# tudelft-iv/CCVPE

Measured on AMD Instinct MI355X. Metric: image-pairs/sec, higher is better.
Workload: dtype f32

## Files before the change

ccvpe_amd/_lib.py:

```python
import ctypes
import os
import subprocess

import torch

_HERE = os.path.dirname(os.path.abspath(__file__))
LIB_PATH = os.environ.get("CCVPE_LIB") or os.path.join(_HERE, "libccvpe_hip.so")
CSRC_DIR = os.path.join(_HERE, "csrc")

c_float_p = ctypes.c_void_p
c_int = ctypes.c_int
c_float = ctypes.c_float
c_void_p = ctypes.c_void_p


class ConvDesc(ctypes.Structure):
    _fields_ = [
        ("src0", c_void_p), ("src1", c_void_p), ("gate", c_void_p), ("w", c_void_p),
        ("scale", c_void_p), ("shift", c_void_p), ("residual", c_void_p), ("dst", c_void_p),
        ("c0", c_int), ("ld0", c_int), ("c1", c_int), ("ld1", c_int),
        ("batch", c_int), ("in_h", c_int), ("in_w", c_int),
        ("kh", c_int), ("kw", c_int), ("stride", c_int), ("pad", c_int),
        ("n", c_int), ("kpad", c_int), ("ldd", c_int), ("ldres", c_int),
        ("act", c_int), ("out_mode", c_int),
    ]


class UpconvDesc(ctypes.Structure):
    _fields_ = [
        ("src0", c_void_p), ("src1", c_void_p), ("w", c_void_p), ("shift9", c_void_p), ("dst", c_void_p),
        ("c0", c_int), ("ld0", c_int), ("c1", c_int), ("ld1", c_int),
        ("batch", c_int), ("h1", c_int), ("w1", c_int),
        ("n", c_int), ("kpad", c_int), ("ldd", c_int), ("act", c_int),
    ]


class TailDesc(ctypes.Structure):
    _fields_ = [
        ("x", c_void_p), ("w", c_void_p), ("shift9", c_void_p), ("w2", c_void_p), ("b2", c_void_p), ("out", c_void_p),
        ("batch", c_int), ("h1", c_int), ("w1", c_int),
        ("c0", c_int), ("ld0", c_int), ("kpad", c_int),
        ("cout", c_int), ("normalize", c_int), ("split", c_int), ("softmax_partial", c_void_p),
    ]


PROTOTYPES = {
    "ccvpe_last_error": (ctypes.c_char_p, []),
    "ccvpe_abi_version": (c_int, []),
    "ccvpe_multi_copy_f32": (c_int, [ctypes.POINTER(c_void_p), ctypes.POINTER(c_void_p), ctypes.POINTER(c_int), c_int, c_void_p]),
    "ccvpe_gather_repack_f32": (c_int, [c_void_p, c_void_p, c_void_p, c_void_p, c_void_p, c_int, c_void_p]),
    "ccvpe_gather_repack_chunk": (c_int, []),
    "ccvpe_ctx_create": (c_int, [c_void_p, ctypes.c_longlong, c_void_p, c_void_p, ctypes.POINTER(c_void_p)]),
    "ccvpe_ctx_destroy": (c_int, [c_void_p]),
    "ccvpe_ctx_info": (c_int, [c_void_p] + [ctypes.POINTER(ctypes.c_longlong)] * 4 + [ctypes.POINTER(c_int)] * 2),
    "ccvpe_ctx_output": (c_int, [c_void_p, c_int, ctypes.POINTER(c_void_p), ctypes.POINTER(ctypes.c_longlong),
                                  ctypes.POINTER(c_int), ctypes.POINTER(ctypes.c_longlong), ctypes.POINTER(ctypes.c_longlong)]),
    "ccvpe_forward": (c_int, [c_void_p, c_void_p, c_void_p, ctypes.POINTER(c_void_p), c_void_p]),
    "ccvpe_tail512_partials": (c_int, [ctypes.POINTER(TailDesc), c_int]),
    "ccvpe_softmax_apply_f32": (c_int, [c_void_p, c_void_p, c_int, c_void_p, c_int, c_int, c_void_p]),
    "ccvpe_tail512_f32": (c_int, [ctypes.POINTER(TailDesc), c_void_p]),
    "ccvpe_tail512_bf16": (c_int, [ctypes.POINTER(TailDesc), c_void_p]),
    "ccvpe_conv_igemm_f32": (c_int, [ctypes.POINTER(ConvDesc), c_void_p]),
    "ccvpe_conv_igemm_splitk_floats": (c_int, [ctypes.POINTER(ConvDesc), c_int]),
    "ccvpe_conv_igemm_route": (c_int, [ctypes.POINTER(ConvDesc), c_int, c_int]),
    "ccvpe_set_narrow_kernels": (c_int, [c_int]),
    "ccvpe_set_pw_ring_kernels": (c_int, [c_int]),
    "ccvpe_set_mbconv_plane_kernels": (c_int, [c_int]),
    "ccvpe_mbconv_front_route": (c_int, [c_int] * 8),
    "ccvpe_mbconv_band_plan": (c_int, [c_int] * 7),
    "ccvpe_conv3x3_variant": (c_int, [ctypes.POINTER(ConvDesc), c_int]),
    "ccvpe_set_match_mfma": (c_int, [c_int]),
    "ccvpe_match_route": (c_int, [c_int, c_int, ctypes.POINTER(c_int)] + [c_int] * 10 + [ctypes.POINTER(c_int)]),
    "ccvpe_set_pwn_kernels": (c_int, [c_int]),
    "ccvpe_conv3x3_wino_ok": (c_int, [ctypes.POINTER(ConvDesc)]),
    "ccvpe_conv3x3_wino_f32": (c_int, [ctypes.POINTER(ConvDesc), c_void_p]),
    "ccvpe_conv3x3_match1_ok": (c_int, [ctypes.POINTER(ConvDesc), c_int, c_int]),
    "ccvpe_conv3x3_match1_bf16": (c_int, [ctypes.POINTER(ConvDesc), c_int, c_void_p, c_int, c_int, c_int, c_int, c_int, c_void_p, c_void_p]),
    "ccvpe_conv_igemm_splitk_f32": (c_int, [ctypes.POINTER(ConvDesc), c_void_p, c_void_p]),
    "ccvpe_conv_igemm_splitk_bf16": (c_int, [ctypes.POINTER(ConvDesc), c_int, c_void_p, c_void_p]),
    "ccvpe_upconv3x3_f32": (c_int, [ctypes.POINTER(UpconvDesc), c_void_p]),
    "ccvpe_upconv3x3_bf16": (c_int, [ctypes.POINTER(UpconvDesc), c_void_p]),
    "ccvpe_upconv3x3_route": (c_int, [ctypes.POINTER(UpconvDesc), c_int]),
    "ccvpe_upconv3x3_s3_ok": (c_int, [ctypes.POINTER(UpconvDesc)]),
    "ccvpe_upconv3x3_s3_f32": (c_int, [ctypes.POINTER(UpconvDesc), c_void_p]),
    "ccvpe_upconv3x3_s3_form_ok": (c_int, [ctypes.POINTER(UpconvDesc), c_int]),
    "ccvpe_upconv3x3_s3_route": (c_int, [ctypes.POINTER(UpconvDesc), c_int]),
    "ccvpe_upconv3x3_s3_form_f32": (c_int, [ctypes.POINTER(UpconvDesc), c_int, c_void_p]),
    "ccvpe_set_s3_quad": (c_int, [c_int]),
    "ccvpe_pw_s3_ok": (c_int, [ctypes.POINTER(ConvDesc)]),
    "ccvpe_pw_s3_route": (c_int, [ctypes.POINTER(ConvDesc)]),
    "ccvpe_pw_s3_f32": (c_int, [ctypes.POINTER(ConvDesc), c_void_p]),
    "ccvpe_stem_conv_f32": (c_int, [c_void_p] * 5 + [c_int] * 4 + [c_void_p]),
    "ccvpe_dwconv_nblk": (c_int, [c_int] * 4),
    "ccvpe_dwconv_f32": (c_int, [c_void_p] * 6 + [c_int] * 7 + [c_void_p]),
    "ccvpe_mbconv_front_nblk": (c_int, [c_int] * 6),
    "ccvpe_stem_dw_nblk": (c_int, [c_int] * 3),
    "ccvpe_stem_dw_f32": (c_int, [c_void_p] * 9 + [c_int] * 4 + [c_void_p]),
    "ccvpe_stem_dw_bf16": (c_int, [c_void_p] * 9 + [c_int] * 4 + [c_void_p]),
    "ccvpe_mbconv_front_f32": (c_int, [c_void_p, c_void_p, c_int] + [c_void_p] * 7 + [c_int] * 8 + [c_void_p]),
    "ccvpe_se_gate_f32": (c_int, [c_void_p, c_int, c_float] + [c_void_p] * 5 + [c_int] * 3 + [c_void_p]),
    "ccvpe_ground_descriptor_f32": (c_int, [c_void_p, c_int, c_void_p, c_void_p, ctypes.POINTER(c_int),
                                            c_void_p, c_int, c_int, c_int, c_void_p]),
    "ccvpe_match_level_f32": (c_int, [c_void_p, c_int, c_void_p, c_int, c_int, ctypes.POINTER(c_int),
                                      c_int, c_int, c_int, c_int, c_int, c_void_p, c_void_p, c_int, c_int,
                                      c_int, c_int, c_void_p]),
    "ccvpe_head_conv3x3_f32": (c_int, [c_void_p] * 4 + [c_int] * 5 + [c_void_p]),
    "ccvpe_cast_bf16_f32": (c_int, [c_void_p, c_void_p, ctypes.c_long, c_void_p]),
    "ccvpe_softmax_rows_f32": (c_int, [c_void_p, c_void_p, c_int, c_int, c_void_p]),
    "ccvpe_eval_postprocess_f32": (c_int, [c_void_p, c_void_p, c_void_p, c_int, c_int, c_int, c_void_p]),
    "ccvpe_eval_metrics_f32": (c_int, [c_void_p] * 7 + [c_int, c_int, c_int, c_void_p]),
    "ccvpe_infonce_scratch_floats": (c_int, [c_int, c_int]),
    "ccvpe_infonce_loss_f32": (c_int, [c_void_p, c_void_p, c_float, c_void_p, c_void_p, c_void_p, c_int, c_int, c_void_p]),
    "ccvpe_cross_entropy_loss_f32": (c_int, [c_void_p] * 4 + [c_int, c_int, c_void_p]),
    "ccvpe_orientation_loss_f32": (c_int, [c_void_p] * 5 + [c_int, c_int, c_void_p]),
    "ccvpe_stem_conv_raw_f32": (c_int, [c_void_p] * 3 + [c_int] * 4 + [c_void_p]),
    "ccvpe_dwconv_raw_f32": (c_int, [c_void_p] * 3 + [c_int] * 7 + [c_void_p]),
    "ccvpe_bn_stats_nblk": (c_int, [c_int]),
    "ccvpe_bn_stats_f32": (c_int, [c_void_p, c_int, c_int] + [c_void_p] * 4 + [c_float, c_void_p, c_void_p]),
    "ccvpe_bn_act_nblk": (c_int, [c_int]),
    "ccvpe_bn_act_f32": (c_int, [c_void_p] * 5 + [c_float, c_int] + [c_void_p] * 4 + [c_int] * 3 + [c_void_p]),
    "ccvpe_conv_wgrad_tile": (c_int, [c_int, c_int]),
    "ccvpe_conv_wgrad_scratch_floats": (c_int, [c_int] * 9),
    "ccvpe_conv_wgrad_f32": (c_int, [c_void_p, c_int, c_int, c_void_p, c_int, c_int, c_void_p, c_int, c_void_p,
                                     c_void_p] + [c_int] * 8 + [c_void_p]),
    "ccvpe_conv_wgrad_gated_f32": (c_int, [c_void_p, c_int, c_int, c_void_p, c_void_p, c_int, c_void_p, c_void_p, c_int, c_int, c_int,
                                           c_int, c_void_p]),
    "ccvpe_conv_wgrad_bias_f32": (c_int, [c_void_p, c_int, c_int, c_void_p, c_int, c_int, c_void_p, c_int, c_void_p,
                                          c_void_p, c_void_p] + [c_int] * 8 + [c_void_p]),
    "ccvpe_colsum_f32": (c_int, [c_void_p, c_int, c_int, c_int, c_void_p, c_void_p, c_void_p]),
    "ccvpe_bn_bwd_nblk": (c_int, [c_int]),
    "ccvpe_bn_act_bwd_f32": (c_int, [c_void_p] * 9 + [c_float, c_int] + [c_void_p] * 4 + [c_int] * 3 + [c_void_p]),
    "ccvpe_bn_act_bwd_frozen_f32": (c_int, [c_void_p] * 9 + [c_float, c_int] + [c_void_p] * 4 + [c_int] * 3 + [c_void_p]),
    "ccvpe_se_bn_bwd_reduce_f32": (c_int, [c_void_p] * 6 + [c_float, c_int, c_void_p, c_void_p, c_int, c_int, c_int, c_void_p]),
    "ccvpe_se_bn_bwd_apply_f32": (c_int, [c_void_p] * 8 + [c_float, c_int, c_void_p, c_void_p, c_void_p, c_void_p, c_int, c_int, c_int,
                                          c_void_p]),
    "ccvpe_se_dgate_f32": (c_int, [c_void_p] * 6 + [c_float, c_int, c_void_p] + [c_int] * 3 + [c_void_p]),
    "ccvpe_se_bwd_f32": (c_int, [c_void_p, c_int, c_float, c_void_p, c_int] + [c_void_p] * 10 + [c_int] * 3 + [c_void_p]),
    "ccvpe_dwconv_dgrad_f32": (c_int, [c_void_p] * 3 + [c_int] * 7 + [c_void_p]),
    "ccvpe_dwconv_wgrad_nblk": (c_int, [c_int] * 4),
    "ccvpe_dwconv_wgrad_f32": (c_int, [c_void_p] * 4 + [c_int] * 7 + [c_void_p]),
    "ccvpe_relu_bwd_f32": (c_int, [c_void_p] * 3 + [c_int, c_void_p]),
    "ccvpe_gate_mul_f32": (c_int, [c_void_p] * 3 + [c_int] * 3 + [c_void_p]),
    "ccvpe_softmax_bwd_f32": (c_int, [c_void_p] * 4 + [c_int, c_int, c_void_p]),
    "ccvpe_l2norm2_bwd_f32": (c_int, [c_void_p] * 3 + [c_int, c_int, c_void_p]),
    "ccvpe_head_conv3x3_bwd_f32": (c_int, [c_void_p] * 7 + [c_int] * 5 + [c_void_p]),
    "ccvpe_ground_descriptor_bwd_f32": (c_int, [c_void_p, c_int, c_void_p, ctypes.POINTER(c_int)] + [c_void_p] * 4 +
                                        [c_int] * 3 + [c_void_p]),
    "ccvpe_add_cols_f32": (c_int, [c_void_p, c_int, c_int, c_void_p, c_int, c_int, c_int, c_int, c_void_p]),
    "ccvpe_stem_wgrad_nblk": (c_int, [c_int] * 3),
    "ccvpe_stem_conv_wgrad_f32": (c_int, [c_void_p] * 4 + [c_int] * 4 + [c_void_p]),
    "ccvpe_match_bwd_nblk": (c_int, [c_int, c_int, c_int]),
    "ccvpe_match_level_bwd_f32": (c_int, [c_void_p, c_int, c_void_p, c_int, c_int, ctypes.POINTER(c_int), c_int, c_int,
                                          c_int, c_int, c_int, c_void_p, c_void_p, c_void_p, c_int, c_void_p, c_int, c_void_p,
                                          c_int, c_void_p, c_int, c_int, c_int, c_void_p]),
    "ccvpe_infonce_loss_bwd_f32": (c_int, [c_void_p, c_void_p, c_float, c_void_p, c_void_p, c_void_p, c_int, c_int, c_void_p]),
    "ccvpe_cross_entropy_loss_bwd_f32": (c_int, [c_void_p] * 4 + [c_int, c_int, c_void_p]),
    "ccvpe_orientation_loss_bwd_f32": (c_int, [c_void_p] * 5 + [c_int, c_int, c_void_p]),
    "ccvpe_train_targets_nblk": (c_int, [c_int, c_int]),
    "ccvpe_train_targets_f32": (c_int, [c_void_p, c_void_p, c_int, c_float] + [c_void_p] * 10 + [c_int] * 3 + [c_void_p]),
    "ccvpe_train_targets_ordered_f32": (c_int, [c_void_p, c_void_p, c_int, c_int, c_float] + [c_void_p] * 10 + [c_int] * 3 + [c_void_p]),
    "ccvpe_adam_chunk_elems": (c_int, []),
    "ccvpe_adam_hyper_floats": (c_int, []),
    "ccvpe_adam_step_f32": (c_int, [c_void_p, c_void_p, c_void_p, c_void_p, c_int, c_float, c_void_p]),
    "ccvpe_adam_device_layout": (c_int, [c_int]),
    "ccvpe_grad_sqnorm_f32": (c_int, [c_void_p, c_void_p, c_void_p, c_int, c_float, c_void_p, c_void_p]),
    "ccvpe_adam_prepare_f32": (c_int, [c_void_p, c_void_p, c_void_p, c_void_p, c_int, c_void_p, c_int, c_float, c_void_p, c_void_p]),
    "ccvpe_adam_update_f32": (c_int, [c_void_p, c_void_p, c_void_p, c_void_p, c_int, c_float, c_void_p, c_void_p]),
    "ccvpe_preprocess_u8_f32": (c_int, [c_void_p, c_int, c_int, c_void_p, c_void_p, c_int, c_void_p, c_void_p, c_int, c_void_p,
                                        c_void_p, c_int, c_int, c_int, c_int, ctypes.POINTER(c_float), ctypes.POINTER(c_float),
                                        c_void_p]),
    "ccvpe_resize_u8": (c_int, [c_void_p, c_int, c_int, c_void_p, c_void_p, c_int, c_void_p, c_void_p, c_int, c_void_p, c_void_p,
                                c_int, c_int, c_void_p]),
    "ccvpe_gather_norm_u8_f32": (c_int, [c_void_p, c_void_p, c_int, c_int, c_int, c_int, ctypes.POINTER(c_float),
                                         ctypes.POINTER(c_float), c_void_p, c_void_p]),
    "ccvpe_window_resize_norm_u8_f32": (c_int, [c_void_p, c_int, c_int, c_void_p, c_int, c_int, c_int, c_void_p, c_void_p, c_int,
                                                c_void_p, c_void_p, c_int, ctypes.POINTER(c_float), ctypes.POINTER(c_float),
                                                c_void_p, c_int, c_int, c_void_p]),
    "ccvpe_kitti_align_u8": (c_int, [c_void_p, ctypes.c_long, c_void_p, c_void_p, c_int, c_void_p, c_int, c_int, c_void_p]),
    "ccvpe_kitti_align_norm_u8_f32": (c_int, [c_void_p, c_void_p, c_int, ctypes.POINTER(c_float), ctypes.POINTER(c_float),
                                              c_void_p, c_int, c_int, c_void_p]),
    "ccvpe_conv_igemm_bf16": (c_int, [ctypes.POINTER(ConvDesc), c_int, c_void_p]),
    "ccvpe_stem_conv_bf16": (c_int, [c_void_p] * 5 + [c_int] * 4 + [c_void_p]),
    "ccvpe_dwconv_bf16": (c_int, [c_void_p] * 6 + [c_int] * 7 + [c_void_p]),
    "ccvpe_mbconv_front_bf16": (c_int, [c_void_p, c_void_p, c_int] + [c_void_p] * 7 + [c_int] * 8 + [c_void_p]),
    "ccvpe_match_level_bf16": (c_int, [c_void_p, c_int, c_void_p, c_int, c_int, ctypes.POINTER(c_int),
                                       c_int, c_int, c_int, c_int, c_int, c_void_p, c_void_p, c_int, c_int,
                                       c_int, c_int, c_void_p]),
    "ccvpe_head_conv3x3_bf16": (c_int, [c_void_p] * 4 + [c_int] * 5 + [c_void_p]),
}

_lib = None
weights_epoch = 0


def build(verbose=False):
    cmd = ["make", "-C", CSRC_DIR, "-j8"]
    res = subprocess.run(cmd, capture_output=True, text=True)
    if verbose or res.returncode != 0:
        print(res.stdout)
        print(res.stderr)
    if res.returncode != 0:
        raise RuntimeError("building libccvpe_hip.so failed (see output above)")
    return LIB_PATH


def load():
    global _lib
    if _lib is not None:
        return _lib
    if not os.path.isfile(LIB_PATH):
        raise RuntimeError(
            "libccvpe_hip.so not found at %s — run `python -c 'import __graft_entry__ as g; g.build()'` "
            "(or `make -C ccvpe_amd/csrc`).  ccvpe_amd has no CPU fallback." % LIB_PATH)
    lib = ctypes.CDLL(LIB_PATH)
    lax = bool(os.environ.get("CCVPE_LIB")) and os.environ.get("CCVPE_LIB_ALLOW_MISSING") == "1"
    for name, (res, args) in PROTOTYPES.items():
        if lax and not hasattr(lib, name):
            continue
        fn = getattr(lib, name)
        fn.restype = res
        fn.argtypes = args
    if os.environ.get("CCVPE_NARROW") == "0" and hasattr(lib, "ccvpe_set_narrow_kernels"):
        lib.ccvpe_set_narrow_kernels(0)
    if os.environ.get("CCVPE_PW_RING") == "0" and hasattr(lib, "ccvpe_set_pw_ring_kernels"):
        lib.ccvpe_set_pw_ring_kernels(0)
    if os.environ.get("CCVPE_MATCH_MFMA") == "0" and hasattr(lib, "ccvpe_set_match_mfma"):
        lib.ccvpe_set_match_mfma(0)
    if os.environ.get("CCVPE_PWN") == "0" and hasattr(lib, "ccvpe_set_pwn_kernels"):
        lib.ccvpe_set_pwn_kernels(0)
    if os.environ.get("CCVPE_S3_QUAD") == "0" and hasattr(lib, "ccvpe_set_s3_quad"):
        lib.ccvpe_set_s3_quad(0)
    if os.environ.get("CCVPE_MBPLANE") is not None and hasattr(lib, "ccvpe_set_mbconv_plane_kernels"):
        lib.ccvpe_set_mbconv_plane_kernels(int(os.environ["CCVPE_MBPLANE"]))
    _lib = lib
    return lib


class CcvpeError(RuntimeError):
    pass


def check(status, what):
    if status != 0:
        msg = load().ccvpe_last_error()
        raise CcvpeError("%s failed (%d): %s" % (what, status, msg.decode() if msg else "?"))
```

ccvpe_amd/csrc/plan.hip:

```cpp
#include <cstring>
#include <string>
#include <unordered_map>
#include <utility>
#include <vector>

#include "common.h"

namespace ccvpe {

enum : uint32_t { K_INT = 0, K_FLT = 1, K_NULL = 2, K_WEIGHTS = 3, K_WORKSPACE = 4, K_GRD = 5, K_SAT = 6, K_STREAM = 7, K_BLOB = 8 };

template <typename A> struct FromSlot {
  static A get(uint64_t v) { return (A)(int64_t)v; }
};
template <typename P> struct FromSlot<P*> {
  static P* get(uint64_t v) { return reinterpret_cast<P*>((uintptr_t)v); }
};
template <> struct FromSlot<float> {
  static float get(uint64_t v) { uint32_t b = (uint32_t)v; float f; std::memcpy(&f, &b, 4); return f; }
};
template <typename... A, size_t... I>
static int invoke_seq(int (*f)(A...), const uint64_t* v, std::index_sequence<I...>) { return f(FromSlot<A>::get(v[I])...); }
template <typename... A>
static int invoke(int (*f)(A...), const uint64_t* v, int n) {
  if (n != (int)sizeof...(A)) return fail(CCVPE_EINVAL, "plan: call has %d arguments, the entry point takes %d", n, (int)sizeof...(A));
  return invoke_seq(f, v, std::index_sequence_for<A...>{});
}
typedef int (*Invoker)(const uint64_t*, int);

#define CCVPE_REG(fn) {#fn, [](const uint64_t* v, int n) -> int { return invoke(fn, v, n); }}
static const std::unordered_map<std::string, Invoker>& registry() {
  static const std::unordered_map<std::string, Invoker> r = {
      CCVPE_REG(ccvpe_conv_igemm_f32), CCVPE_REG(ccvpe_conv_igemm_bf16), CCVPE_REG(ccvpe_conv_igemm_splitk_f32),
      CCVPE_REG(ccvpe_conv_igemm_splitk_bf16), CCVPE_REG(ccvpe_conv3x3_match1_bf16), CCVPE_REG(ccvpe_conv3x3_wino_f32),
      CCVPE_REG(ccvpe_upconv3x3_f32), CCVPE_REG(ccvpe_upconv3x3_bf16), CCVPE_REG(ccvpe_upconv3x3_s3_f32), CCVPE_REG(ccvpe_pw_s3_f32),
      CCVPE_REG(ccvpe_tail512_f32), CCVPE_REG(ccvpe_tail512_bf16), CCVPE_REG(ccvpe_stem_conv_f32), CCVPE_REG(ccvpe_stem_conv_bf16),
      CCVPE_REG(ccvpe_stem_dw_f32), CCVPE_REG(ccvpe_stem_dw_bf16),
      CCVPE_REG(ccvpe_dwconv_f32), CCVPE_REG(ccvpe_dwconv_bf16), CCVPE_REG(ccvpe_mbconv_front_f32), CCVPE_REG(ccvpe_mbconv_front_bf16),
      CCVPE_REG(ccvpe_se_gate_f32), CCVPE_REG(ccvpe_ground_descriptor_f32), CCVPE_REG(ccvpe_match_level_f32),
      CCVPE_REG(ccvpe_match_level_bf16), CCVPE_REG(ccvpe_head_conv3x3_f32), CCVPE_REG(ccvpe_head_conv3x3_bf16),
      CCVPE_REG(ccvpe_softmax_rows_f32), CCVPE_REG(ccvpe_softmax_apply_f32), CCVPE_REG(ccvpe_cast_bf16_f32), CCVPE_REG(ccvpe_eval_postprocess_f32),
  };
  return r;
}
#undef CCVPE_REG

struct Patch { uint32_t call, arg, kind; uint64_t off; };
struct BlobPatch { uint32_t blob, field, kind; uint64_t off; };
struct Call { Invoker fn; std::string name; uint32_t first, nargs, sid; int wait_on; };
struct Output { uint64_t off, bytes; uint32_t dtype, ndim; long long dims[4], strides[4]; };

}

struct ccvpe_ctx {
  std::vector<ccvpe::Call> calls;
  std::vector<uint64_t> args;
  std::vector<std::vector<unsigned char>> blobs;
  std::vector<ccvpe::Patch> patches;
  std::vector<ccvpe::BlobPatch> blob_patches;
  std::vector<ccvpe::Output> outputs;
  uint64_t workspace_bytes = 0, weights_bytes = 0, grd_bytes = 0, sat_bytes = 0;
  char* weights = nullptr;
  char* workspace = nullptr;
  bool own_weights = false, own_workspace = false;
  hipStream_t side = nullptr;
  std::vector<hipEvent_t> events;
};

using namespace ccvpe;

namespace {
struct Reader {
  const unsigned char* p;
  const unsigned char* end;
  bool ok = true;
  template <typename T> T get() {
    T v{};
    if (sizeof(T) > (size_t)(end - p)) { ok = false; return v; }
    std::memcpy(&v, p, sizeof(T));
    p += sizeof(T);
    return v;
  }
  const unsigned char* bytes(size_t n) {
    if (n > (size_t)(end - p)) { ok = false; return nullptr; }
    const unsigned char* q = p;
    p += n;
    return q;
  }
};
}

extern "C" int ccvpe_ctx_create(const void* plan, long long n_bytes, void* weights_dev, void* workspace_dev, ccvpe_ctx** out) {
  if (!plan || n_bytes < 64 || !out) return fail(CCVPE_EINVAL, "ctx_create: null / short plan");
  Reader r{reinterpret_cast<const unsigned char*>(plan), reinterpret_cast<const unsigned char*>(plan) + n_bytes};
  const unsigned char* magic = r.bytes(8);
  if (!magic || std::memcmp(magic, "CCVPLAN1", 8)) return fail(CCVPE_EINVAL, "ctx_create: not a CCVPE plan (bad magic)");
  ccvpe_ctx* c = new ccvpe_ctx();
  auto bail = [&](int code, const char* msg) { delete c; return fail(code, "ctx_create: %s", msg); };
  const int abi = (int)r.get<uint32_t>();
  const uint32_t flags = r.get<uint32_t>();
  (void)flags;
  if (abi != ccvpe_abi_version()) {
    delete c;
    return fail(CCVPE_EINVAL, "ctx_create: the plan was recorded against ABI %d, this library is ABI %d", abi, ccvpe_abi_version());
  }
  c->workspace_bytes = r.get<uint64_t>();
  c->weights_bytes = r.get<uint64_t>();
  c->grd_bytes = r.get<uint64_t>();
  c->sat_bytes = r.get<uint64_t>();
  const uint32_t n_calls = r.get<uint32_t>(), n_blobs = r.get<uint32_t>(), n_out = r.get<uint32_t>();
  r.get<uint32_t>();
  if (!r.ok || n_calls > (1u << 20) || n_blobs > (1u << 20) || n_out > 64) return bail(CCVPE_EINVAL, "corrupt header");
  for (uint32_t i = 0; i < n_out; ++i) {
    Output o;
    o.off = r.get<uint64_t>(); o.bytes = r.get<uint64_t>(); o.dtype = r.get<uint32_t>(); o.ndim = r.get<uint32_t>();
    for (int k = 0; k < 4; ++k) o.dims[k] = (long long)r.get<uint64_t>();
    for (int k = 0; k < 4; ++k) o.strides[k] = (long long)r.get<uint64_t>();
    if (o.off > c->workspace_bytes || o.bytes > c->workspace_bytes - o.off) return bail(CCVPE_EINVAL, "output outside the workspace");
    c->outputs.push_back(o);
  }
  struct Reloc { uint32_t blob, field, kind; uint64_t value; };
  std::vector<Reloc> relocs;
  for (uint32_t i = 0; i < n_blobs && r.ok; ++i) {
    const uint32_t nb = r.get<uint32_t>(), nr = r.get<uint32_t>();
    for (uint32_t k = 0; k < nr; ++k) {
      Reloc q{i, r.get<uint32_t>(), r.get<uint32_t>(), r.get<uint64_t>()};
      if ((uint64_t)q.field + 8 > (uint64_t)nb) return bail(CCVPE_EINVAL, "relocation outside its blob");
      relocs.push_back(q);
    }
    const unsigned char* d = r.bytes((nb + 7) & ~7u);
    if (!d) return bail(CCVPE_EINVAL, "truncated blob");
    c->blobs.emplace_back(d, d + nb);
  }
  struct RawArg { uint32_t kind; uint64_t value; };
  std::vector<std::vector<RawArg>> raw(n_calls);
  for (uint32_t i = 0; i < n_calls && r.ok; ++i) {
    const unsigned char* nm = r.bytes(48);
    if (!nm) break;
    std::string name(reinterpret_cast<const char*>(nm), strnlen(reinterpret_cast<const char*>(nm), 48));
    const uint32_t na = r.get<uint32_t>();
    const uint32_t sid = r.get<uint32_t>() & 1u;
    if (na > 64) return bail(CCVPE_EINVAL, "call with more than 64 arguments");
    for (uint32_t k = 0; k < na; ++k) {
      RawArg a{r.get<uint32_t>(), 0};
      r.get<uint32_t>();
      a.value = r.get<uint64_t>();
      raw[i].push_back(a);
    }
    if (name == "@wait") {
      if (na != 2) return bail(CCVPE_EINVAL, "malformed stream wait");
      c->calls.push_back(Call{nullptr, name, 0, 0, (uint32_t)(raw[i][0].value & 1), (int)(raw[i][1].value & 1)});
      raw[i].clear();
      continue;
    }
    auto it = registry().find(name);
    if (it == registry().end()) {
      delete c;
      return fail(CCVPE_EINVAL, "ctx_create: the plan calls %s, which this library does not replay", name.c_str());
    }
    c->calls.push_back(Call{it->second, name, 0, na, sid, -1});
  }
  if (!r.ok) return bail(CCVPE_EINVAL, "truncated plan");
  size_t woff = (size_t)(r.p - reinterpret_cast<const unsigned char*>(plan));
  woff = (woff + 255) & ~(size_t)255;
  if (woff > (size_t)n_bytes || c->weights_bytes > (uint64_t)((size_t)n_bytes - woff)) return bail(CCVPE_EINVAL, "truncated weights");
  if (weights_dev) c->weights = reinterpret_cast<char*>(weights_dev);
  else {
    if (hipMalloc(reinterpret_cast<void**>(&c->weights), c->weights_bytes ? c->weights_bytes : 256) != hipSuccess) return bail(CCVPE_ELAUNCH, "hipMalloc(weights)");
    c->own_weights = true;
  }
  if (workspace_dev) c->workspace = reinterpret_cast<char*>(workspace_dev);
  else {
    if (hipMalloc(reinterpret_cast<void**>(&c->workspace), c->workspace_bytes ? c->workspace_bytes : 256) != hipSuccess) {
      if (c->own_weights) (void)hipFree(c->weights);
      return bail(CCVPE_ELAUNCH, "hipMalloc(workspace)");
    }
    c->own_workspace = true;
  }
  if (c->weights_bytes &&
      hipMemcpy(c->weights, reinterpret_cast<const unsigned char*>(plan) + woff, c->weights_bytes, hipMemcpyHostToDevice) != hipSuccess) {
    ccvpe_ctx_destroy(c);
    return fail(CCVPE_ELAUNCH, "ctx_create: weight upload failed");
  }
  auto resolve = [&](uint32_t kind, uint64_t v, bool& dynamic, bool& bad) -> uint64_t {
    dynamic = bad = false;
    switch (kind) {
      case K_INT: case K_FLT: return v;
      case K_NULL: return 0;
      case K_WEIGHTS: bad = v >= c->weights_bytes; return (uint64_t)(uintptr_t)(c->weights + v);
      case K_WORKSPACE: bad = v >= c->workspace_bytes; return (uint64_t)(uintptr_t)(c->workspace + v);
      case K_BLOB: bad = v >= c->blobs.size(); return bad ? 0 : (uint64_t)(uintptr_t)c->blobs[v].data();
      case K_GRD: bad = v >= c->grd_bytes; dynamic = true; return 0;
      case K_SAT: bad = v >= c->sat_bytes; dynamic = true; return 0;
      case K_STREAM: dynamic = true; return 0;
      default: bad = true; return 0;
    }
  };
  for (const Reloc& q : relocs) {
    bool dyn, bad;
    const uint64_t v = resolve(q.kind, q.value, dyn, bad);
    if (bad || q.kind == K_BLOB || q.kind == K_STREAM) { ccvpe_ctx_destroy(c); return fail(CCVPE_EINVAL, "ctx_create: bad relocation"); }
    if (dyn) c->blob_patches.push_back(BlobPatch{q.blob, q.field, q.kind, q.value});
    else std::memcpy(c->blobs[q.blob].data() + q.field, &v, 8);
  }
  for (uint32_t i = 0; i < n_calls; ++i) {
    c->calls[i].first = (uint32_t)c->args.size();
    for (uint32_t k = 0; k < raw[i].size(); ++k) {
      bool dyn, bad;
      const uint64_t v = resolve(raw[i][k].kind, raw[i][k].value, dyn, bad);
      if (bad) { ccvpe_ctx_destroy(c); return fail(CCVPE_EINVAL, "ctx_create: bad argument %u of call %u (%s)", k, i, c->calls[i].name.c_str()); }
      if (dyn) c->patches.push_back(Patch{i, k, raw[i][k].kind, raw[i][k].value});
      c->args.push_back(v);
    }
  }
  bool two_streams = false;
  for (const Call& k : c->calls) {
    two_streams = two_streams || k.sid == 1 || !k.fn;
    if (!k.fn) {
      hipEvent_t ev;
      if (hipEventCreateWithFlags(&ev, hipEventDisableTiming) != hipSuccess) { ccvpe_ctx_destroy(c); return fail(CCVPE_ELAUNCH, "ctx_create: hipEventCreate"); }
      c->events.push_back(ev);
    }
  }
  if (two_streams && hipStreamCreateWithFlags(&c->side, hipStreamNonBlocking) != hipSuccess) {
    ccvpe_ctx_destroy(c);
    return fail(CCVPE_ELAUNCH, "ctx_create: hipStreamCreate");
  }
  *out = c;
  return CCVPE_OK;
}

extern "C" int ccvpe_ctx_destroy(ccvpe_ctx* c) {
  if (!c) return CCVPE_OK;
  if (c->own_weights && c->weights) (void)hipFree(c->weights);
  if (c->own_workspace && c->workspace) (void)hipFree(c->workspace);
  for (hipEvent_t ev : c->events) (void)hipEventDestroy(ev);
  if (c->side) (void)hipStreamDestroy(c->side);
  delete c;
  return CCVPE_OK;
}

extern "C" int ccvpe_ctx_info(const ccvpe_ctx* c, long long* workspace_bytes, long long* weights_bytes, long long* grd_bytes,
                              long long* sat_bytes, int* n_outputs, int* n_calls) {
  if (!c) return fail(CCVPE_EINVAL, "ctx_info: null ctx");
  if (workspace_bytes) *workspace_bytes = (long long)c->workspace_bytes;
  if (weights_bytes) *weights_bytes = (long long)c->weights_bytes;
  if (grd_bytes) *grd_bytes = (long long)c->grd_bytes;
  if (sat_bytes) *sat_bytes = (long long)c->sat_bytes;
  if (n_outputs) *n_outputs = (int)c->outputs.size();
  if (n_calls) *n_calls = (int)c->calls.size();
  return CCVPE_OK;
}

extern "C" int ccvpe_ctx_output(const ccvpe_ctx* c, int i, void** dev_ptr, long long* bytes, int* ndim, long long* dims4,
                                long long* strides4) {
  if (!c || i < 0 || i >= (int)c->outputs.size()) return fail(CCVPE_EINVAL, "ctx_output: bad index");
  const Output& o = c->outputs[i];
  if (dev_ptr) *dev_ptr = c->workspace + o.off;
  if (bytes) *bytes = (long long)o.bytes;
  if (ndim) *ndim = (int)o.ndim;
  if (dims4) for (int k = 0; k < 4; ++k) dims4[k] = o.dims[k];
  if (strides4) for (int k = 0; k < 4; ++k) strides4[k] = o.strides[k];
  return CCVPE_OK;
}

extern "C" int ccvpe_forward(ccvpe_ctx* c, const void* grd, const void* sat, void** out, void* stream) {
  if (!c || !grd || !sat) return fail(CCVPE_EINVAL, "forward: null ctx / input");
  for (const Patch& q : c->patches) {
    uint64_t v = 0;
    if (q.kind == K_GRD) v = (uint64_t)(uintptr_t)(reinterpret_cast<const char*>(grd) + q.off);
    else if (q.kind == K_SAT) v = (uint64_t)(uintptr_t)(reinterpret_cast<const char*>(sat) + q.off);
    else v = (uint64_t)(uintptr_t)(c->calls[q.call].sid ? (void*)c->side : stream);
    c->args[c->calls[q.call].first + q.arg] = v;
  }
  for (const BlobPatch& q : c->blob_patches) {
    const uint64_t v = (uint64_t)(uintptr_t)(reinterpret_cast<const char*>(q.kind == K_GRD ? grd : sat) + q.off);
    std::memcpy(c->blobs[q.blob].data() + q.field, &v, 8);
  }
  size_t nev = 0;
  for (const Call& k : c->calls) {
    if (!k.fn) {
      hipStream_t waiter = k.sid ? c->side : (hipStream_t)stream, waitee = k.wait_on ? c->side : (hipStream_t)stream;
      hipEvent_t ev = c->events[nev++];
      if (hipEventRecord(ev, waitee) != hipSuccess || hipStreamWaitEvent(waiter, ev, 0) != hipSuccess)
        return fail(CCVPE_ELAUNCH, "forward: stream wait failed");
      continue;
    }
    const int rc = k.fn(c->args.data() + k.first, (int)k.nargs);
    if (rc != CCVPE_OK) return rc;
  }
  if (out) for (size_t i = 0; i < c->outputs.size(); ++i) out[i] = c->workspace + c->outputs[i].off;
  return CCVPE_OK;
}
```

ccvpe_amd/models.py:

```python
import torch
import torch.nn as nn

from . import ops
from .synth import B0_BLOCKS, MODEL_SPECS, state_dict_spec

BN_EPS = 1e-3
SKIP_BLOCKS = (15, 10, 4, 2, 0)
MATCH_STRIDES = {"vigor": (64, 32, 16, 8, 4, 2),
                 "kitti": (128, 64, 32, 16, 8, 8),
                 "oxford": (64, 32, 16, 8, 4, 2)}


def window_offset(kind, channels, length):
    return int(channels / 2 - length / 2) if kind == "oxford" else 0


def _round_up(v, m):
    return (v + m - 1) // m * m


class _Holder(nn.Module):

    def forward(self, *a, **k):
        raise RuntimeError("parameter holder is not callable; use the owning CVM_* module")


def _populate(root, kind, init):
    for key, shape, role in state_dict_spec(kind):
        parts = key.split(".")
        node = root
        for name in parts[:-1]:
            child = node._modules.get(name)
            if child is None:
                child = _Holder()
                node.add_module(name, child)
            node = child
        t = init[key].clone()
        if role in ("bn_m", "bn_v", "bn_n"):
            node.register_buffer(parts[-1], t)
        else:
            node.register_parameter(parts[-1], nn.Parameter(t))


def _pad2(w, dtype=torch.float32, n_mult=16):
    k_mult = 16 if dtype == torch.float32 else 32
    n, k = w.shape
    if n % n_mult == 0 and k % k_mult == 0:
        out = w.to(dtype).contiguous()
        return out.clone() if out.data_ptr() == w.data_ptr() else out
    out = w.new_zeros((_round_up(n, n_mult), _round_up(k, k_mult)))
    out[:n, :k] = w
    return out.to(dtype).contiguous()


def _pack_conv(w, dtype=torch.float32):
    o = w.shape[0]
    return _pad2(w.permute(0, 2, 3, 1).reshape(o, -1), dtype)


_WINO_G = ((1.0, 0.0, 0.0), (0.5, 0.5, 0.5), (0.5, -0.5, 0.5), (0.0, 0.0, 1.0))


def _pack_wino(w, dtype=torch.float32):
    if dtype != torch.float32:
        return None
    o, i = w.shape[0], w.shape[1]
    g = torch.tensor(_WINO_G, dtype=torch.float64, device=w.device)
    u = torch.einsum("ak,ockl,bl->oabc", g, w.to(torch.float64), g)
    out = torch.zeros((_round_up(o, 32), 4, 4, _round_up(i, 16)), dtype=torch.float64, device=w.device)
    out[:o, :, :, :i] = u
    return out.reshape(out.shape[0], -1).to(torch.float32).contiguous()


def _fold_bn(sd, p):
    scale = sd[p + ".weight"] / torch.sqrt(sd[p + ".running_var"] + BN_EPS)
    shift = sd[p + ".bias"] - sd[p + ".running_mean"] * scale
    return scale.contiguous(), shift.contiguous()


class _Obj(object):
    pass


def _pack_pw_s3(w):
    if w is None or w.dtype != torch.float32 or w.dim() != 2 or w.shape[1] % 16 or w.shape[0] % 16:
        return None
    npad, k = w.shape
    return torch.cat(_split3_bf16(w.reshape(npad, k // 16, 16).permute(1, 0, 2)), -1).contiguous()


def _unpack_pw_s3(w3):
    nst, npad, _ = w3.shape
    return tuple(w3[..., 16 * q:16 * q + 16].float().permute(1, 0, 2).reshape(npad, nst * 16) for q in range(3))


PW_S3_MIN_MID = 240


def _pack_encoder(sd, p, dtype=torch.float32, fold_bn=True, s3=False):
    fold = _fold_bn if fold_bn else (lambda _sd, _p: (None, None))
    e = _Obj()
    e.stem_w = sd[p + "._conv_stem.weight"].permute(2, 3, 1, 0).contiguous()
    e.stem_scale, e.stem_shift = fold(sd, p + "._bn0")
    e.blocks = []
    for i, (k, s, ex, cin, cout) in enumerate(B0_BLOCKS):
        b = _Obj()
        bp = "%s._blocks.%d" % (p, i)
        b.k, b.s, b.expand, b.cin, b.cout, b.mid = k, s, ex != 1, cin, cout, cin * ex
        if b.expand:
            b.w_exp = _pack_conv(sd[bp + "._expand_conv.weight"], dtype)
            b.s0, b.b0 = fold(sd, bp + "._bn0")
        b.w_dw = sd[bp + "._depthwise_conv.weight"].reshape(b.mid, k, k).permute(1, 2, 0).contiguous()
        b.s1, b.b1 = fold(sd, bp + "._bn1")
        b.se_w1 = sd[bp + "._se_reduce.weight"].reshape(-1, b.mid).contiguous()
        b.se_b1 = sd[bp + "._se_reduce.bias"].contiguous()
        b.se_w2 = sd[bp + "._se_expand.weight"].reshape(b.mid, -1).t().contiguous()
        b.se_b2 = sd[bp + "._se_expand.bias"].contiguous()
        b.w_proj = _pack_conv(sd[bp + "._project_conv.weight"], dtype)
        b.w_proj3 = _pack_pw_s3(b.w_proj) if s3 and b.mid >= PW_S3_MIN_MID else None
        b.s2, b.b2 = fold(sd, bp + "._bn2")
        b.skip = (s == 1 and cin == cout)
        e.blocks.append(b)
    e.w_head = _pack_conv(sd[p + "._conv_head.weight"], dtype)
    e.w_head3 = _pack_pw_s3(e.w_head) if s3 else None
    e.head_scale, e.head_shift = fold(sd, p + "._bn1")
    return e


def _pack_deconv(w, bias, col_map, ldo, dtype=torch.float32):
    cin, cout = w.shape[0], w.shape[1]
    wg = w.permute(2, 3, 1, 0).reshape(4 * cout, cin)
    out = w.new_zeros((4 * cout, ldo))
    for d0, s0, n in col_map:
        out[:, d0:d0 + n] = wg[:, s0:s0 + n]
    return _pad2(out, dtype), bias.repeat(4).contiguous()


_UP_S = {0: {0: ((0, 1),), 1: ((1, 0), (2, 1))}, 1: {0: ((0, 0), (1, 1)), 1: ((2, 0),)}}
_UP_R = {0: (1, 2), 1: (0, 1, 2), 2: (0, 1)}
_OVERLAP_ENV = __import__("os").environ.get("CCVPE_OVERLAP_DECODERS", "auto")


OVERLAP_DECODERS_MAX_BATCH = 128


def _overlap_decoders(precision, batch=1):
    return _OVERLAP_ENV == "1" or (_OVERLAP_ENV == "auto" and precision == "bf16" and batch <= OVERLAP_DECODERS_MAX_BATCH)
FOLD_LEVELS = tuple(int(c) for c in __import__("os").environ.get("CCVPE_FOLD_LEVELS", "012345"))
FOLD_MIN_PIXELS = int(__import__("os").environ.get("CCVPE_FOLD_MIN_PIXELS", "2048"))
FUSE_TAIL = __import__("os").environ.get("CCVPE_FUSE_TAIL", "1") != "0"
SPLIT_TAIL = __import__("os").environ.get("CCVPE_SPLIT_TAIL", "1") != "0"
WINO = __import__("os").environ.get("CCVPE_WINO", "1") != "0"
SPLIT3 = __import__("os").environ.get("CCVPE_SPLIT3", "1") != "0"
SPLIT3_TAIL = SPLIT3 and __import__("os").environ.get("CCVPE_SPLIT3_TAIL", "1") != "0"
SPLIT3_MIN_OK = 2
SPLIT3_PW = SPLIT3 and __import__("os").environ.get("CCVPE_SPLIT3_PW", "1") != "0"
SPLIT3_PW_MIN_OK = 2
PACK_GRAPH = __import__("os").environ.get("CCVPE_PACK_GRAPH", "1") != "0"
PACK_GATHER = __import__("os").environ.get("CCVPE_PACK_GATHER", "1") != "0"
FUSE_MATCH = __import__("os").environ.get("CCVPE_FUSE_MATCH", "1") != "0"
FUSE_STEM = __import__("os").environ.get("CCVPE_FUSE_STEM", "1") != "0"
EVAL_TWO_STREAMS = __import__("os").environ.get("CCVPE_EVAL_TWO_STREAMS", "1") != "0"


def _tail_split(precision, x, cout):
    if x.dtype != torch.float32:
        return 0
    if precision == "bf16":
        return 1 if SPLIT_TAIL and cout == 1 else 0
    return 2 if SPLIT3 and SPLIT3_TAIL else 0


def _pack_upconv(wd, bd, col_map, cp, w3, b3, dtype=torch.float32):
    cd, co = wd.shape[1], w3.shape[0]
    c1 = w3.shape[1] - cd
    wd_my = wd.new_zeros((cp, cd, 2, 2), dtype=torch.float64)
    for d0, s0, n in col_map:
        wd_my[d0:d0 + n] = wd[s0:s0 + n].double()
    w3d = w3[:, :cd].double()
    k = 4 * cp + 9 * c1
    kmult = 16 if dtype == torch.float32 else 32
    out = wd.new_zeros((4, _round_up(co, 16), _round_up(k, kmult)), dtype=torch.float64)
    for py in range(2):
        for px in range(2):
            par = py * 2 + px
            for du in range(2):
                for dv in range(2):
                    weff = wd.new_zeros((co, cp), dtype=torch.float64)
                    for ky, a in _UP_S[py][du]:
                        for kx, b in _UP_S[px][dv]:
                            weff += w3d[:, :, ky, kx] @ wd_my[:, :, a, b].t()
                    tap = du * 2 + dv
                    out[par, :co, tap * cp:(tap + 1) * cp] = weff
            if c1:
                out[par, :co, 4 * cp:k] = w3[:, cd:].double().permute(0, 2, 3, 1).reshape(co, 9 * c1)
    shift9 = wd.new_zeros((9, co), dtype=torch.float64)
    for rc in range(3):
        for cc in range(3):
            v = b3.double().clone()
            for ky in _UP_R[rc]:
                for kx in _UP_R[cc]:
                    v += w3d[:, :, ky, kx] @ bd.double()
            shift9[rc * 3 + cc] = v
    return out.to(dtype).contiguous(), shift9.float().contiguous()


def _split3_bf16(v):
    hi = v.to(torch.bfloat16)
    r = v - hi.float()
    mid = r.to(torch.bfloat16)
    lo = (r - mid.float()).to(torch.bfloat16)
    return hi, mid, lo


def _pack_upconv_s3(fw, cp, c1, dtype=torch.float32):
    if dtype != torch.float32 or fw is None or fw.dtype != torch.float32 or c1 <= 0:
        return None
    npad = fw.shape[1]
    nb0, nb1 = (cp + 15) // 16, (c1 + 15) // 16
    a = fw.new_zeros((4, npad, 4, nb0 * 16))
    a[..., :cp] = fw[:, :, :4 * cp].reshape(4, npad, 4, cp)
    a = a.reshape(4, npad, 4, nb0, 16).permute(0, 3, 2, 1, 4).reshape(4, 4 * nb0, npad, 16)
    s = fw.new_zeros((4, npad, 9, nb1 * 16))
    s[..., :c1] = fw[:, :, 4 * cp:4 * cp + 9 * c1].reshape(4, npad, 9, c1)
    s = s.reshape(4, npad, 9, nb1, 16).permute(0, 2, 3, 1, 4).reshape(4, 9 * nb1, npad, 16)
    return torch.cat(_split3_bf16(torch.cat([a, s], 1)), -1).contiguous()


def _pack_backward(sd, kind, pk):
    spec = MODEL_SPECS[kind]
    n_rot = spec["n_rot"]
    bwd = {}
    for enc in ("grd_efficientnet", "sat_efficientnet"):
        for i, (k, s_, ex, cin, cout) in enumerate(B0_BLOCKS):
            bp = "%s._blocks.%d" % (enc, i)
            if ex != 1:
                bwd[bp + "._expand_conv.weight"] = _pack_conv(sd[bp + "._expand_conv.weight"].permute(1, 0, 2, 3))
            bwd[bp + "._project_conv.weight"] = _pack_conv(sd[bp + "._project_conv.weight"].permute(1, 0, 2, 3))
            if s_ == 1:
                mid = cin * ex
                w_dw = sd[bp + "._depthwise_conv.weight"].reshape(mid, k * k).t()
                bwd[bp + "._depthwise_conv.weight"] = w_dw.flip(0).contiguous()
        bwd[enc + "._conv_head.weight"] = _pack_conv(sd[enc + "._conv_head.weight"].permute(1, 0, 2, 3))
    for j in range(6):
        lvl = 6 - j
        for branch, lv in (("", pk.loc[j]), ("_ori", pk.ori[j])):
            conv, deconv = "conv%d%s" % (lvl, branch), "deconv%d%s" % (lvl, branch)
            if lvl != 1:
                bwd[conv + ".2.weight"] = _pack_conv(sd[conv + ".2.weight"].flip(2, 3).permute(1, 0, 2, 3))
            bwd[conv + ".0.weight"] = _pack_conv(sd[conv + ".0.weight"].flip(2, 3).permute(1, 0, 2, 3))
            w_ref = sd[deconv + ".weight"]
            if branch == "":
                c = lv.c
                k_rows, cmap = lv.ldo, [(0, 1, c), (c, 0, 1)]
            elif j == 0:
                c6 = spec["ori"][0][0] - n_rot
                k_rows, cmap = lv.k, [(0, n_rot, c6), (c6 + 1, 0, n_rot)]
            else:
                k_rows, cmap = lv.k, [(0, 0, spec["ori"][j][0])]
            w_ours = w_ref.new_zeros((k_rows,) + tuple(w_ref.shape[1:]))
            for d0, s0, n in cmap:
                w_ours[d0:d0 + n] = w_ref[s0:s0 + n]
            bwd[deconv + ".weight"] = _pack_conv(w_ours)
    w = sd["sat_feature_to_descriptors.1.weight"]
    w4 = w.view(w.shape[0], 1280, 2, 2)
    bwd["sat_feature_to_descriptors.1.weight"] = _pack_deconv(w4, w4.new_zeros((1280,)), [(0, 0, w.shape[0])], w.shape[0])[0]
    wcat = torch.cat([sd["grd_feature_to_descriptor%d.0.weight" % l] for l in range(1, 7)], 0)
    ld = _round_up(pk.gd_n, 4)
    wpad = wcat.new_zeros((ld,) + tuple(wcat.shape[1:]))
    wpad[:pk.gd_n] = wcat
    bwd["grd_feature_to_descriptor.0.weight"] = _pack_conv(wpad.permute(1, 0, 2, 3))
    return bwd


def _pack_model(sd, kind, n_tail, dtype=torch.float32, fold=True, f32_tail=0):
    spec = MODEL_SPECS[kind]
    pk = _Obj()
    pk.dtype = dtype
    pk.f32_from = 6 - f32_tail if dtype != torch.float32 else 6
    base_dtype = dtype
    s3 = fold and dtype == torch.float32
    pk.grd = _pack_encoder(sd, "grd_efficientnet", dtype, fold_bn=fold, s3=s3)
    pk.sat = _pack_encoder(sd, "sat_efficientnet", dtype, fold_bn=fold, s3=s3)
    ws, bs, wh, bh = [], [], [], []
    for l in range(1, 7):
        p = "grd_feature_to_descriptor%d" % l
        ws.append(sd[p + ".0.weight"].reshape(-1, 1280))
        bs.append(sd[p + ".0.bias"])
        wh.append(sd[p + ".2.weight"].reshape(-1))
        bh.append(sd[p + ".2.bias"].reshape(-1))
    pk.gd_w = _pad2(torch.cat(ws, 0), dtype)
    pk.gd_w3 = _pack_pw_s3(pk.gd_w) if s3 else None
    pk.gd_bias = torch.cat(bs, 0).contiguous()
    pk.gd_n = pk.gd_bias.shape[0]
    pk.gd_wh = torch.stack(wh, 0).contiguous()
    pk.gd_bh = torch.cat(bh, 0).contiguous()
    w = sd["sat_feature_to_descriptors.1.weight"]
    pk.sd_w = _pack_conv(w.view(w.shape[0], 1280, 2, 2), dtype)
    pk.sd_w3 = _pack_pw_s3(pk.sd_w) if s3 else None
    pk.sd_bias = sd["sat_feature_to_descriptors.1.bias"].contiguous()
    pk.sd_n = w.shape[0]

    pk.loc, pk.ori = [], []
    n_rot = spec["n_rot"]
    for j in range(6):
        lvl = 6 - j
        dc_in, dc_out, c_in, c_out = spec["loc"][j]
        dtype = torch.float32 if j >= pk.f32_from else base_dtype
        c = dc_in - 1
        ldo = _round_up(c + 1 + (n_tail if j == 0 else 0), 8)
        lv = _Obj()
        lv.c, lv.ldo, lv.up_n = c, ldo, 4 * dc_out
        lv.up_w, lv.up_b = _pack_deconv(sd["deconv%d.weight" % lvl], sd["deconv%d.bias" % lvl],
                                        [(0, 1, c), (c, 0, 1)], ldo, dtype)
        lv.c0, lv.c1 = dc_out, c_in - dc_out
        lv.n_a = c_out
        if fold and j in FOLD_LEVELS:
            lv.fw, lv.fshift = _pack_upconv(sd["deconv%d.weight" % lvl], sd["deconv%d.bias" % lvl],
                                            [(0, 1, c), (c, 0, 1)], ldo, sd["conv%d.0.weight" % lvl],
                                            sd["conv%d.0.bias" % lvl], dtype)
            lv.fw3 = _pack_upconv_s3(lv.fw, ldo, lv.c1, dtype if base_dtype == torch.float32 else None)
        lv.w_a = _pack_conv(sd["conv%d.0.weight" % lvl], dtype)
        lv.b_a = sd["conv%d.0.bias" % lvl].contiguous()
        if lvl != 1:
            lv.w_b = _pack_conv(sd["conv%d.2.weight" % lvl], dtype)
            lv.u_b = _pack_wino(sd["conv%d.2.weight" % lvl], base_dtype) if fold else None
            lv.n_b = c_out
        else:
            lv.w_b = sd["conv1.2.weight"].permute(0, 2, 3, 1).contiguous()
        lv.b_b = sd["conv%d.2.bias" % lvl].contiguous()
        pk.loc.append(lv)
        dtype = base_dtype
        dc_in, dc_out, c_in, c_out = spec["ori"][j]
        ov = _Obj()
        if j == 0:
            c6 = dc_in - n_rot
            ov.k = pk.loc[0].ldo
            ov.k_algo = dc_in
            ov.up_w, ov.up_b = _pack_deconv(sd["deconv6_ori.weight"], sd["deconv6_ori.bias"],
                                            [(0, n_rot, c6), (c6 + 1, 0, n_rot)], pk.loc[0].ldo, dtype)
        else:
            ov.k = ov.k_algo = dc_in
            ov.up_w, ov.up_b = _pack_deconv(sd["deconv%d_ori.weight" % lvl], sd["deconv%d_ori.bias" % lvl],
                                            [(0, 0, dc_in)], dc_in, dtype)
        ov.up_n = 4 * dc_out
        ov.c0, ov.c1 = dc_out, c_in - dc_out
        if fold and j in FOLD_LEVELS:
            cmap = [(0, n_rot, c6), (c6 + 1, 0, n_rot)] if j == 0 else [(0, 0, dc_in)]
            ov.fw, ov.fshift = _pack_upconv(sd["deconv%d_ori.weight" % lvl], sd["deconv%d_ori.bias" % lvl], cmap,
                                            ov.k, sd["conv%d_ori.0.weight" % lvl], sd["conv%d_ori.0.bias" % lvl],
                                            dtype)
            ov.fw3 = _pack_upconv_s3(ov.fw, ov.k, ov.c1, dtype)
        ov.w_a = _pack_conv(sd["conv%d_ori.0.weight" % lvl], dtype)
        ov.b_a = sd["conv%d_ori.0.bias" % lvl].contiguous()
        ov.n_a = c_out
        if lvl != 1:
            ov.w_b = _pack_conv(sd["conv%d_ori.2.weight" % lvl], dtype)
            ov.u_b = _pack_wino(sd["conv%d_ori.2.weight" % lvl], dtype) if fold else None
            ov.n_b = c_out
        else:
            ov.w_b = sd["conv1_ori.2.weight"].permute(0, 2, 3, 1).contiguous()
        ov.b_b = sd["conv%d_ori.2.bias" % lvl].contiguous()
        pk.ori.append(ov)
    pk.bwd = _pack_backward(sd, kind, pk) if (not fold and base_dtype == torch.float32) else None
    return pk


def _pw(x, c0, w, w3, n, *, batch, in_h, in_w, two=False, gate=None, scale=None, shift=None, residual=None, act=ops.ACT_NONE,
        ldd=None, out_f32=False):
    if (SPLIT3 and SPLIT3_PW and w3 is not None and x.dtype == torch.float32 and
            ops.pw_s3_ok(x, c0, w3, n, batch=batch, in_h=in_h, in_w=in_w, two=two, gate=gate, residual=residual, act=act,
                         ldd=ldd) >= SPLIT3_PW_MIN_OK):
        return ops.pw_s3(x, c0, w3, n, batch=batch, in_h=in_h, in_w=in_w, two=two, gate=gate, scale=scale, shift=shift,
                         residual=residual, act=act, ldd=ldd)
    kk = dict(kh=2, kw=2, stride=2) if two else {}
    return ops.conv_igemm(x, c0, w, n, batch=batch, in_h=in_h, in_w=in_w, gate=gate, scale=scale, shift=shift, residual=residual,
                          act=act, ldd=ldd, out_f32=out_f32, **kk)


def _run_encoder(e, img, circular, multiscale, dtype=torch.float32):
    blk0 = e.blocks[0]
    stem_fused = (FUSE_STEM and not blk0.expand and blk0.k == 3 and blk0.s == 1 and blk0.mid == 32
                  and ops.stem_dw_supported(img.shape[2], img.shape[3], circular) > 0)
    x = None if stem_fused else ops.stem_conv(img, e.stem_w, e.stem_scale, e.stem_shift, circular, out_dtype=dtype)
    feats = []
    for blk in e.blocks:
        if x is not None:
            b, h, w, _ = x.shape
        if x is None:
            u, part = ops.stem_dw(img, e.stem_w, e.stem_scale, e.stem_shift, blk.w_dw, blk.s1, blk.b1, circular,
                                  out_dtype=dtype)
            b = u.shape[0]
        elif blk.expand and ops.mbconv_front_supported(h, w, blk.cin, blk.mid, blk.k, blk.s):
            u, part = ops.mbconv_front(x, blk.w_exp, blk.s0, blk.b0, blk.w_dw, blk.s1, blk.b1, blk.mid,
                                       blk.k, blk.s, circular)
        else:
            t = x
            if blk.expand:
                t = ops.conv_igemm(x, blk.cin, blk.w_exp, blk.mid, batch=b, in_h=h, in_w=w,
                                   scale=blk.s0, shift=blk.b0, act=ops.ACT_SWISH)
            u, part = ops.dwconv(t, blk.w_dw, blk.s1, blk.b1, blk.k, blk.s, circular)
        ho, wo = u.shape[1], u.shape[2]
        gate = ops.se_gate(part, ho * wo, blk.se_w1, blk.se_b1, blk.se_w2, blk.se_b2)
        x = _pw(u, blk.mid, blk.w_proj, getattr(blk, "w_proj3", None), blk.cout, batch=b, in_h=ho, in_w=wo, gate=gate,
                scale=blk.s2, shift=blk.b2, residual=x if blk.skip else None)
        if multiscale:
            feats.append(x)
    b, h, w, _ = x.shape
    f = _pw(x, 320, e.w_head, getattr(e, "w_head3", None), 1280, batch=b, in_h=h, in_w=w, scale=e.head_scale,
            shift=e.head_shift, act=ops.ACT_SWISH)
    return f, feats


def _double_conv(lv, up, skip, batch, hw):
    y = ops.conv_igemm(up, lv.c0, lv.w_a, lv.n_a, batch=batch, in_h=hw, in_w=hw, kh=3, kw=3, pad=1,
                       src1=skip, c1=lv.c1, shift=lv.b_a, act=ops.ACT_RELU)
    return y


def _conv_b(lv, y, batch, hw, out_f32=False):
    if (WINO and lv.u_b is not None and
            ops.conv3x3_wino_ok(y, lv.n_a, lv.u_b, lv.n_b, batch=batch, in_h=hw, in_w=hw)):
        return ops.conv3x3_wino(y, lv.n_a, lv.u_b, lv.n_b, batch=batch, in_h=hw, in_w=hw, shift=lv.b_b)
    return ops.conv_igemm(y, lv.n_a, lv.w_b, lv.n_b, batch=batch, in_h=hw, in_w=hw, kh=3, kw=3, pad=1, shift=lv.b_b,
                          out_f32=out_f32)


def _upconv_a(lv, x, k, batch, hw, skip):
    fw3 = getattr(lv, "fw3", None)
    if (SPLIT3 and fw3 is not None and
            ops.upconv3x3_s3_ok(x, k, fw3, lv.n_a, batch=batch, h1=hw, w1=hw, src1=skip, c1=lv.c1) >= SPLIT3_MIN_OK):
        return ops.upconv3x3_s3(x, k, fw3, lv.fshift, lv.n_a, batch=batch, h1=hw, w1=hw, src1=skip, c1=lv.c1, act=ops.ACT_RELU)
    return ops.upconv3x3(x, k, lv.fw, lv.fshift, lv.n_a, batch=batch, h1=hw, w1=hw, src1=skip, c1=lv.c1, act=ops.ACT_RELU)


class _CVMBase(nn.Module):
    kind = "vigor"

    def __init__(self, device, circular_padding, ori_noise=None, efficientnet_weights=None):
        super().__init__()
        self.device = device
        self.circular_padding = circular_padding
        self.ori_noise = ori_noise
        from . import init as _init
        _populate(self, self.kind, _init.reference_init_state_dict(self.kind))
        weights = efficientnet_weights if efficientnet_weights is not None else __import__("os").environ.get("CCVPE_EFFICIENTNET_B0")
        if weights:
            _init.load_efficientnet_b0(self, weights)
        self._pack_cache = None
        self._pack_key = None
        self.precision = "fp32"
        self.fp32_tail_levels = 1

    def set_precision(self, precision, fp32_tail_levels=1):
        if precision not in ("fp32", "bf16"):
            raise ValueError("precision must be 'fp32' or 'bf16'")
        if not 0 <= int(fp32_tail_levels) <= 5:
            raise ValueError("fp32_tail_levels must be in 0..5 (level 6 feeds the bf16 orientation decoder)")
        self.precision = precision
        self.fp32_tail_levels = int(fp32_tail_levels)
        return self

    def invalidate(self):
        self._pack_cache = None
        self._pack_key = None
        object.__setattr__(self, "_flat_tensors", None)
        return self

    def _weights_key(self):
        from . import _lib
        flat = getattr(self, "_flat_tensors", None)
        if flat is None:
            flat = list(self.parameters()) + list(self.buffers())
            object.__setattr__(self, "_flat_tensors", flat)
        return (_lib.weights_epoch,) + tuple((t.data_ptr(), t._version) for t in flat)

    def _packed(self):
        epoch = 0 if self.training else getattr(self, "_stats_epoch", 0)
        key = (self.precision, self.fp32_tail_levels, self.training, epoch) + self._weights_key()
        if self._pack_cache is not None and key == self._pack_key:
            return self._pack_cache
        dev = next(self.parameters()).device
        if dev.type != "cuda":
            raise RuntimeError("ccvpe_amd: move the model to the MI355X first (.to('cuda'))")
        sd = {k: v.detach() for k, v in self.state_dict().items()}
        n_tail = MODEL_SPECS[self.kind]["n_rot"]
        dtype = torch.float32 if self.precision == "fp32" else torch.bfloat16

        def pack(src=sd):
            with torch.no_grad():
                return _pack_model(src, self.kind, n_tail, dtype, fold=not self.training, f32_tail=self.fp32_tail_levels)

        if self.training and PACK_GATHER and dtype == torch.float32 and not getattr(self, "_pack_plan_failed", False):
            from . import repack
            where = tuple(t.data_ptr() for t in list(self.parameters()) + list(self.buffers()))
            gp = getattr(self, "_pack_plan", None)
            if gp is not None and gp[0] == where:
                self._pack_cache = gp[1].run()
            else:
                plan = repack.build(sd, pack)
                if plan is None:
                    self._pack_plan, self._pack_plan_failed = None, True
                    return self._packed()
                self._pack_plan = (where, plan)
                self._pack_cache = plan.pk
        elif self.training and PACK_GRAPH:
            where = (self.precision, self.fp32_tail_levels) + tuple(
                t.data_ptr() for t in list(self.parameters()) + list(self.buffers()))
            g = getattr(self, "_pack_graph", None)
            if g is not None and g[0] == where:
                g[1].replay()
                self._pack_cache = g[2]
            elif getattr(self, "_pack_where", None) == where and not getattr(self, "_pack_graph_failed", False):
                try:
                    graph = torch.cuda.CUDAGraph()
                    with torch.cuda.graph(graph, capture_error_mode="thread_local"):
                        pk = pack()
                    graph.replay()
                    self._pack_graph = (where, graph, pk)
                    self._pack_cache = pk
                except Exception:
                    self._pack_graph, self._pack_graph_failed = None, True
                    self._pack_cache = pack()
            else:
                self._pack_graph = None
                self._pack_where = where
                self._pack_cache = pack()
        else:
            self._pack_cache = pack()
        self._pack_key = key
        return self._pack_cache

    def _side_stream(self, which=1):
        dev = next(self.parameters()).device
        streams = self.__dict__.setdefault("_side_streams", {})
        st = streams.get(which)
        if st is None or st.device != dev:
            st = torch.cuda.Stream(device=dev)
            streams[which] = st
        return st

    def _ori_decoder(self, pk, cat6, sfeats, batch):
        xo = cat6
        normalize = not getattr(self, "ori_raw_output", False)
        for j in range(6):
            ov = pk.ori[j]
            hw = xo.shape[1]
            skip = sfeats[SKIP_BLOCKS[j]] if j < 5 else None
            if j == 5 and FUSE_TAIL and j in FOLD_LEVELS and ops.tail512_ok(hw, hw, ov.n_a):
                return ops.tail512(xo, ov.k, ov.fw, ov.fshift, ov.w_b, ov.b_b, 2, normalize, batch=batch, h1=hw, w1=hw,
                                   split=_tail_split(self.precision, xo, 2))
            if j in FOLD_LEVELS and batch * hw * hw >= FOLD_MIN_PIXELS:
                y = _upconv_a(ov, xo, ov.k, batch, hw, skip)
            else:
                up = ops.conv_igemm(xo, ov.k, ov.up_w, ov.up_n, batch=batch, in_h=hw, in_w=hw,
                                    shift=ov.up_b, out_mode=ops.OUT_DECONV2X, algo_k=ov.k_algo)
                y = _double_conv(ov, up, skip, batch, 2 * hw)
            if j < 5:
                xo = _conv_b(ov, y, batch, 2 * hw)
            else:
                return ops.head_conv3x3(y, ov.w_b, ov.b_b, 2, normalize)

    def _loc_shifts(self):
        n_rot = MODEL_SPECS[self.kind]["n_rot"]
        if self.ori_noise is None:
            return list(range(n_rot))
        k = int(self.ori_noise / 18)
        return list(range(-k, k + 1))

    drop_connect_rate = 0.2
    BN_MOMENTUM = 0.01

    bn_frozen = False

    def freeze_batchnorm(self, mode=True):
        self.bn_frozen = bool(mode)
        return self

    def forward(self, grd, sat, drop_masks=None):
        if self.training and self.precision != "fp32":
            raise NotImplementedError("ccvpe_amd: train mode is fp32 only")
        if not (grd.is_cuda and sat.is_cuda):
            raise RuntimeError("ccvpe_amd runs on the MI355X only: inputs must be device tensors")
        if self.training:
            from . import train
            if torch.is_grad_enabled() and any(p.requires_grad for p in self.parameters()):
                outs = train.apply(self, grd, sat, drop_masks)
            else:
                with torch.no_grad():
                    outs, _ = train.forward_train(self, grd, sat, drop_masks, rec=False)
            outs = list(outs)
            if self.ori_noise is not None:
                outs[3] = outs[3][:, len(self._loc_shifts()):]
            return tuple(outs)
        main = torch.cuda.current_stream()
        return self._forward_eval(grd, sat, main, self._side_stream() if EVAL_TWO_STREAMS else main)

    def _forward_eval(self, grd, sat, main, side):
        spec = MODEL_SPECS[self.kind]
        n_rot = spec["n_rot"]
        strides = MATCH_STRIDES[self.kind]
        circular = bool(self.circular_padding) and self.kind == "vigor"
        with torch.no_grad():
            pk = self._packed()
            grd = grd.contiguous().float()
            sat = sat.contiguous().float()
            batch = grd.shape[0]

            side.wait_stream(main)
            with torch.cuda.stream(side):
                gfeat, _ = _run_encoder(pk.grd, grd, circular, False, pk.dtype)
                _, gh, gw, _ = gfeat.shape
                if gh != spec["grd_h"]:
                    raise ValueError("ground feature height %d != %d expected by the descriptor heads"
                                     % (gh, spec["grd_h"]))
                y1 = _pw(gfeat, 1280, pk.gd_w, pk.gd_w3, pk.gd_n, batch=batch, in_h=gh, in_w=gw,
                         shift=pk.gd_bias, ldd=_round_up(pk.gd_n, 4), out_f32=True)
                gdesc = ops.ground_descriptor(y1, pk.gd_wh, pk.gd_bh, spec["cd"])
            svol, sfeats = _run_encoder(pk.sat, sat, False, True, pk.dtype)
            main.wait_stream(side)
            gdesc.record_stream(main)
            sdesc = _pw(svol, 1280, pk.sd_w, pk.sd_w3, pk.sd_n, batch=batch, in_h=svol.shape[1],
                        in_w=svol.shape[2], two=True, shift=pk.sd_bias)

            overlap = _overlap_decoders(self.precision, batch)
            loc_shifts = self._loc_shifts()
            fused = None
            scores_out = []
            smx = None
            x = sdesc
            cat6 = None
            goff = 0
            sfeats_loc = sfeats
            for j in range(6):
                lv = pk.loc[j]
                if j == pk.f32_from:
                    x = ops.cast_f32(x)
                    sfeats_loc = dict((SKIP_BLOCKS[q], ops.cast_f32(sfeats[SKIP_BLOCKS[q]])) for q in range(j, 5))
                hw = x.shape[1]
                cd = spec["cd"][j]
                L = gw * cd
                g = gdesc[:, goff:goff + L]
                goff += L
                if j == 0:
                    if self.ori_noise is None:
                        shifts, n_max = list(range(n_rot)), n_rot
                    else:
                        shifts, n_max = loc_shifts + list(range(n_rot)), len(loc_shifts)
                    n_tail = n_rot
                else:
                    shifts, n_max, n_tail = loc_shifts, len(loc_shifts), 0
                if fused is not None:
                    sc, cat = fused
                    fused = None
                else:
                    sc, cat = ops.match_level(x, g, L, shifts, n_max, n_tail, strides[j], lv.ldo, channels=lv.c,
                                              window_offset=window_offset(self.kind, lv.c, L))
                if j == 0:
                    cat6 = cat
                    scores_out.append(sc if self.ori_noise is None else sc[:, n_max:])
                    if overlap:
                        side.wait_stream(main)
                        with torch.cuda.stream(side):
                            x_ori = self._ori_decoder(pk, cat6, sfeats, batch)
                else:
                    scores_out.append(sc)
                skip = sfeats_loc[SKIP_BLOCKS[j]] if j < 5 else None
                if j == 5 and FUSE_TAIL and j in FOLD_LEVELS and ops.tail512_ok(hw, hw, lv.n_a):
                    logits_map, smx = ops.tail512(cat, lv.ldo, lv.fw, lv.fshift, lv.w_b, lv.b_b, 1, False, batch=batch, h1=hw, w1=hw,
                                                  split=_tail_split(self.precision, cat, 1),
                                                  want_softmax=True)
                    break
                if j in FOLD_LEVELS and batch * hw * hw >= FOLD_MIN_PIXELS:
                    y = _upconv_a(lv, cat, lv.ldo, batch, hw, skip)
                else:
                    up = ops.conv_igemm(cat, lv.ldo, lv.up_w, lv.up_n, batch=batch, in_h=hw, in_w=hw,
                                        shift=lv.up_b, out_mode=ops.OUT_DECONV2X, algo_k=lv.c + 1)
                    y = _double_conv(lv, up, skip, batch, 2 * hw)
                if j < 5:
                    to_f32 = j + 1 == pk.f32_from and y.dtype != torch.float32
                    nxt = pk.loc[j + 1]
                    L_n = gw * spec["cd"][j + 1]
                    if (FUSE_MATCH and len(loc_shifts) == 1 and
                            ops.conv3x3_match1(y, lv.n_a, lv.w_b, lv.n_b, None, L_n, loc_shifts[0], strides[j + 1], nxt.ldo, batch=batch,
                                               in_h=2 * hw, in_w=2 * hw, bias=lv.b_b, out_f32=to_f32, query_only=True)):
                        fused = ops.conv3x3_match1(y, lv.n_a, lv.w_b, lv.n_b, gdesc[:, goff:goff + L_n], L_n, loc_shifts[0],
                                                   strides[j + 1], nxt.ldo, batch=batch, in_h=2 * hw, in_w=2 * hw, bias=lv.b_b,
                                                   window_offset=window_offset(self.kind, nxt.c, L_n), out_f32=to_f32)
                        x = fused[1]
                    else:
                        x = _conv_b(lv, y, batch, 2 * hw, out_f32=to_f32)
                else:
                    logits_map = ops.head_conv3x3(y, lv.w_b, lv.b_b, 1, False)
            logits = logits_map.reshape(batch, -1)
            if smx is not None:
                heatmap = ops.softmax_apply(logits, smx).reshape(logits_map.shape)
            else:
                heatmap = ops.softmax_rows(logits).reshape(logits_map.shape)

            if overlap:
                main.wait_stream(side)
                x_ori.record_stream(main)
            else:
                x_ori = self._ori_decoder(pk, cat6, sfeats, batch)
        return (logits, heatmap, x_ori) + tuple(scores_out)


class CVM_VIGOR(_CVMBase):
    kind = "vigor"

    def __init__(self, device, circular_padding, efficientnet_weights=None):
        super().__init__(device, circular_padding, None, efficientnet_weights)


class CVM_VIGOR_ori_prior(_CVMBase):
    kind = "vigor"

    def __init__(self, device, ori_noise, circular_padding=True, efficientnet_weights=None):
        super().__init__(device, circular_padding, ori_noise, efficientnet_weights)


class CVM_OxfordRobotCar(_CVMBase):
    kind = "oxford"

    def __init__(self, device, efficientnet_weights=None):
        super().__init__(device, False, None, efficientnet_weights)


class CVM_KITTI(_CVMBase):
    kind = "kitti"

    def __init__(self, device, efficientnet_weights=None):
        super().__init__(device, False, None, efficientnet_weights)
```

ccvpe_amd/ops.py:

```python
import ctypes

import torch

from . import _lib
from ._lib import ConvDesc, check

ACT_NONE, ACT_RELU, ACT_SWISH, ACT_RELU_MASK = 0, 1, 2, 3
SPLIT_K_CALLS = 0
SPLIT_K = __import__("os").environ.get("CCVPE_SPLIT_K", "1") == "1"
OUT_NHWC, OUT_DECONV2X = 0, 1

_recorder = None


def set_recorder(rec):
    global _recorder
    _recorder = rec


class LaunchRecorder(object):

    def __init__(self):
        self.items = []

    def begin(self):
        ev = torch.cuda.Event(enable_timing=True)
        ev.record(torch.cuda.current_stream())
        return ev

    def end(self, name, tag, flops, nbytes, ev0):
        ev1 = torch.cuda.Event(enable_timing=True)
        ev1.record(torch.cuda.current_stream())
        self.items.append((name, tag, flops, nbytes, ev0, ev1))

    def summary(self):
        out = {}
        for name, tag, flops, nbytes, e0, e1 in self.items:
            d = out.setdefault(name, dict(calls=0, ms=0.0, flops=0.0, bytes=0.0))
            d["calls"] += 1
            d["ms"] += e0.elapsed_time(e1)
            d["flops"] += flops
            d["bytes"] += nbytes
        return out


def igemm_tile(n, is3x3=False):
    npad = (n + 15) // 16 * 16
    cfgs = [(4, 5, 2), (4, 4, 2), (4, 3, 2), (4, 2, 2), (4, 1, 2), (4, 5, 1), (4, 3, 1), (4, 1, 1), (2, 7, 1)]
    best, best_cost = None, None
    for mt, nt, wn in cfgs:
        bn = 16 * nt * wn
        tiles = (npad + bn - 1) // bn
        cost = tiles * bn * 1000 + (1000 - bn)
        if best_cost is None or cost < best_cost:
            best, best_cost = (mt, nt, wn), cost
    mt, nt, wn = best
    return "%s<%d,%d,%d>" % ("conv3x3_f32_kernel" if is3x3 else "igemm_f32_kernel", mt, nt, wn)


def _stream():
    return ctypes.c_void_p(torch.cuda.current_stream().cuda_stream)


ROUTE_FAMILIES = {0: "igemm", 1: "pw_gemm", 2: "conv3x3", 3: "c3n", 4: "pw_ring", 5: "pwn"}


def conv_route(desc, is_bf16, out_f32=False):
    r = _lib.load().ccvpe_conv_igemm_route(ctypes.byref(desc), int(bool(is_bf16)), int(bool(out_f32)))
    if r < 0:
        check(int(r), "ccvpe_conv_igemm_route")
    return ROUTE_FAMILIES[r & 0xff], (r >> 8) & 0xf, (r >> 12) & 0xf, (r >> 16) & 0xf


def conv3x3_variant(desc, is_bf16):
    r = _lib.load().ccvpe_conv3x3_variant(ctypes.byref(desc), int(bool(is_bf16)))
    if r < 0:
        check(int(r), "ccvpe_conv3x3_variant")
    return (r & 0xf, bool((r >> 4) & 1), (r >> 8) & 0xf) if r else None


UPROUTE_KERNELS = {0: "upconv_kernel", 1: "upconv_halo_kernel", 2: "upconv_dma_kernel", 3: "upconv_dma_kernel", 4: "up2_kernel"}


def upconv_route(desc, is_bf16):
    r = _lib.load().ccvpe_upconv3x3_route(ctypes.byref(desc), int(bool(is_bf16)))
    if r < 0:
        check(int(r), "ccvpe_upconv3x3_route")
    return UPROUTE_KERNELS[r & 0xff], (r >> 8) & 0xf, (r >> 12) & 0xf, (r >> 16) & 0xf, (r & 0xff) == 3


def upconv_route_name(desc, is_bf16):
    k, mt, nt, wn, pair = upconv_route(desc, is_bf16)
    ty = "bf16" if is_bf16 else "f32"
    if k == "up2_kernel":
        return "up2_kernel<bf16,%d,%d>" % (desc.c0, desc.n)
    return "%s<%s,%d,%d,%d%s>" % (k, ty, mt, nt, wn, ",pair" if pair else "")


def upconv_s3_route_name(desc, form=0):
    r = _lib.load().ccvpe_upconv3x3_s3_route(ctypes.byref(desc), form)
    if r <= 0:
        raise _lib.CcvpeError("ccvpe_upconv3x3_s3_route: form %d does not compute this layer" % form)
    mt, nt, wn = (r >> 8) & 0xf, (r >> 12) & 0xf, (r >> 16) & 0xf
    return "upconv_s3q_kernel<%d,%d>" % (mt, nt) if r & 0xf == 2 else "upconv_s3_kernel<%d,%d,%d%s>" % (mt, nt, wn, ",pair" if r & 16 else "")


def conv_route_name(desc, is_bf16, out_f32=False):
    fam, mt, nt, wn = conv_route(desc, is_bf16, out_f32)
    if fam == "c3n":
        return "c3n_kernel<bf16,%d>" % desc.n
    if is_bf16:
        return "%s_kernel<bf16,%d,%d,%d>" % (fam, mt, nt, wn)
    return "%s_f32_kernel<%d,%d,%d>" % (fam, mt, nt, wn)


_record = None


def _empty(shape, device=None, dtype=torch.float32):
    if _record is not None:
        return _record.empty(shape, dtype, device)
    return torch.empty(shape, device=device, dtype=dtype)


def _ptr(t):
    if t is None:
        return None
    if _record is not None:
        _record.note(t)
    return ctypes.c_void_p(t.data_ptr())


def _chk(t, name, dtype=torch.float32):
    if t is None:
        return
    if not t.is_cuda or t.dtype != dtype or not t.is_contiguous():
        raise ValueError("%s must be a contiguous %s device tensor (got %s %s contiguous=%s)" % (
            name, dtype, t.device, t.dtype, t.is_contiguous()))


def _act_dtype(t):
    if t.dtype not in (torch.float32, torch.bfloat16):
        raise ValueError("activations must be fp32 or bf16, got %s" % t.dtype)
    return t.dtype


def conv_igemm(src0, c0, w_packed, n, *, batch, in_h, in_w, kh=1, kw=1, stride=1, pad=0,
               src1=None, c1=0, gate=None, scale=None, shift=None, residual=None, act=ACT_NONE,
               out_mode=OUT_NHWC, dst=None, ldd=None, ld0=None, ld1=None, algo_k=None, out_f32=False, route_only=False,
               variant_only=False):
    lib = _lib.load()
    dt = _act_dtype(src0)
    odt = torch.float32 if (out_f32 or dt == torch.float32) else dt
    for t, nm in ((src0, "src0"), (src1, "src1"), (w_packed, "w"), (residual, "residual")):
        _chk(t, nm, dt)
    for t, nm in ((gate, "gate"), (scale, "scale"), (shift, "shift")):
        _chk(t, nm)
    _chk(dst, "dst", odt)
    ld0 = ld0 if ld0 is not None else src0.shape[-1]
    ld1 = ld1 if ld1 is not None else (src1.shape[-1] if src1 is not None else 0)
    ho = (in_h + 2 * pad - kh) // stride + 1
    wo = (in_w + 2 * pad - kw) // stride + 1
    if out_mode == OUT_DECONV2X:
        cout = n // 4
        oshape = (batch, 2 * ho, 2 * wo)
    else:
        cout = n
        oshape = (batch, ho, wo)
    if dst is None:
        ldd = ldd if ldd is not None else cout
        dst = _empty(oshape + (ldd,), device=src0.device, dtype=odt)
    elif ldd is None:
        ldd = dst.shape[-1]
    d = ConvDesc()
    d.src0, d.src1, d.gate, d.w = _ptr(src0), _ptr(src1), _ptr(gate), _ptr(w_packed)
    d.scale, d.shift, d.residual, d.dst = _ptr(scale), _ptr(shift), _ptr(residual), _ptr(dst)
    d.c0, d.ld0, d.c1, d.ld1 = c0, ld0, c1, ld1
    d.batch, d.in_h, d.in_w = batch, in_h, in_w
    d.kh, d.kw, d.stride, d.pad = kh, kw, stride, pad
    d.n, d.kpad = n, w_packed.shape[1]
    d.ldd = ldd
    d.ldres = residual.shape[-1] if residual is not None else 0
    d.act, d.out_mode = act, out_mode
    if route_only:
        return conv_route(d, dt != torch.float32, bool(out_f32))
    if variant_only:
        return conv3x3_variant(d, dt != torch.float32)
    rec = _recorder
    ev0 = rec.begin() if rec is not None else None
    want = lib.ccvpe_conv_igemm_splitk_floats(ctypes.byref(d), int(dt != torch.float32)) if SPLIT_K else 0
    if want < 0:
        check(int(want), "ccvpe_conv_igemm_splitk_floats")
    if want > 0:
        global SPLIT_K_CALLS
        SPLIT_K_CALLS += 1
        scratch = _empty((want,), device=src0.device, dtype=torch.float32)
        if dt == torch.float32:
            check(lib.ccvpe_conv_igemm_splitk_f32(ctypes.byref(d), _ptr(scratch), _stream()), "ccvpe_conv_igemm_splitk_f32")
        else:
            check(lib.ccvpe_conv_igemm_splitk_bf16(ctypes.byref(d), int(bool(out_f32)), _ptr(scratch), _stream()),
                  "ccvpe_conv_igemm_splitk_bf16")
    elif dt == torch.float32:
        check(lib.ccvpe_conv_igemm_f32(ctypes.byref(d), _stream()), "ccvpe_conv_igemm_f32")
    else:
        check(lib.ccvpe_conv_igemm_bf16(ctypes.byref(d), int(bool(out_f32)), _stream()), "ccvpe_conv_igemm_bf16")
    if rec is not None:
        m = batch * ho * wo
        k_alg = algo_k if algo_k is not None else kh * kw * (c0 + c1)
        flops = 2.0 * m * n * k_alg
        esz = 4.0 if dt == torch.float32 else 2.0
        nbytes = esz * (batch * in_h * in_w * (c0 + c1) + m * n + n * k_alg
                        + (m * n if residual is not None else 0))
        if want > 0:
            name = igemm_tile(n, False)
        else:
            name = conv_route_name(d, dt != torch.float32, bool(out_f32))
        if want > 0 and dt != torch.float32:
            name = name.replace("_f32_kernel<", "_kernel<bf16,")
        rec.end(name, "%dx%d s%d M%d N%d K%d" % (kh, kw, stride, m, n, k_alg), flops, nbytes, ev0)
    return dst


def _wino_desc(src0, c0, u_packed, n, batch, in_h, in_w, shift, dst, ldd, ld0):
    d = ConvDesc()
    d.src0, d.src1, d.gate, d.w = _ptr(src0), None, None, _ptr(u_packed)
    d.scale, d.shift, d.residual, d.dst = None, _ptr(shift), None, _ptr(dst) if dst is not None else None
    d.c0, d.ld0, d.c1, d.ld1 = c0, ld0, 0, 0
    d.batch, d.in_h, d.in_w = batch, in_h, in_w
    d.kh, d.kw, d.stride, d.pad = 3, 3, 1, 1
    d.n, d.kpad = n, u_packed.shape[1]
    d.ldd, d.ldres = ldd, 0
    d.act, d.out_mode = ACT_NONE, OUT_NHWC
    return d


def conv3x3_wino_ok(src0, c0, u_packed, n, *, batch, in_h, in_w, ldd=None, ld0=None):
    if src0.dtype != torch.float32 or u_packed is None:
        return False
    ld0 = ld0 if ld0 is not None else src0.shape[-1]
    d = _wino_desc(src0, c0, u_packed, n, batch, in_h, in_w, None, None, ldd if ldd is not None else n, ld0)
    return bool(_lib.load().ccvpe_conv3x3_wino_ok(ctypes.byref(d)))


def conv3x3_wino(src0, c0, u_packed, n, *, batch, in_h, in_w, shift=None, dst=None, ldd=None, ld0=None):
    lib = _lib.load()
    for t, nm in ((src0, "src0"), (u_packed, "w"), (shift, "shift"), (dst, "dst")):
        _chk(t, nm)
    ld0 = ld0 if ld0 is not None else src0.shape[-1]
    if dst is None:
        ldd = ldd if ldd is not None else n
        dst = _empty((batch, in_h, in_w, ldd), device=src0.device)
    elif ldd is None:
        ldd = dst.shape[-1]
    d = _wino_desc(src0, c0, u_packed, n, batch, in_h, in_w, shift, dst, ldd, ld0)
    rec = _recorder
    ev0 = rec.begin() if rec is not None else None
    check(lib.ccvpe_conv3x3_wino_f32(ctypes.byref(d), _stream()), "ccvpe_conv3x3_wino_f32")
    if rec is not None:
        m = batch * in_h * in_w
        flops = 2.0 * m * n * 9 * c0
        nbytes = 4.0 * (m * c0 + m * n + n * 9 * c0)
        rec.end("conv3x3_wino_f32_kernel<16x16,32>", "3x3 s1 M%d N%d K%d" % (m, n, 9 * c0), flops, nbytes, ev0)
    return dst


def upconv3x3(src0, c0, w_packed, shift9, n, *, batch, h1, w1, src1=None, c1=0, act=ACT_NONE, algo_flops=None, route_only=False):
    lib = _lib.load()
    dt = _act_dtype(src0)
    for t, nm in ((src0, "src0"), (src1, "src1"), (w_packed, "w")):
        _chk(t, nm, dt)
    _chk(shift9, "shift9")
    dst = _empty((batch, 2 * h1, 2 * w1, n), device=src0.device, dtype=dt)
    d = _lib.UpconvDesc()
    d.src0, d.src1, d.w, d.shift9, d.dst = _ptr(src0), _ptr(src1), _ptr(w_packed), _ptr(shift9), _ptr(dst)
    d.c0, d.ld0, d.c1, d.ld1 = c0, src0.shape[-1], c1, (src1.shape[-1] if src1 is not None else 0)
    d.batch, d.h1, d.w1 = batch, h1, w1
    d.n, d.kpad, d.ldd, d.act = n, w_packed.shape[-1], n, act
    if route_only:
        return upconv_route(d, dt != torch.float32)
    rec = _recorder
    ev0 = rec.begin() if rec is not None else None
    fn = lib.ccvpe_upconv3x3_f32 if dt == torch.float32 else lib.ccvpe_upconv3x3_bf16
    check(fn(ctypes.byref(d), _stream()), "ccvpe_upconv3x3")
    if rec is not None:
        m = batch * h1 * w1 * 4
        k_eff = 4 * c0 + 9 * c1
        flops = algo_flops if algo_flops is not None else 2.0 * m * n * k_eff
        esz = 4.0 if dt == torch.float32 else 2.0
        nbytes = esz * (batch * h1 * w1 * c0 + m * c1 + m * n + 4 * n * k_eff)
        name = upconv_route_name(d, dt != torch.float32)
        rec.end(name, "up3x3 M%d N%d Keff%d" % (m, n, k_eff), flops, nbytes, ev0)
    return dst


def _s3_desc(src0, c0, w3_packed, shift9, n, batch, h1, w1, src1, c1, act, dst, ldd, ld0, ld1):
    d = _lib.UpconvDesc()
    d.src0, d.src1, d.w, d.shift9 = _ptr(src0), _ptr(src1), _ptr(w3_packed), _ptr(shift9)
    d.dst = _ptr(dst) if dst is not None else None
    d.c0, d.ld0, d.c1, d.ld1 = c0, ld0, c1, ld1
    d.batch, d.h1, d.w1 = batch, h1, w1
    d.n, d.kpad, d.ldd, d.act = n, w3_packed.shape[1] * w3_packed.shape[3], ldd, act
    return d


def upconv3x3_s3_ok(src0, c0, w3_packed, n, *, batch, h1, w1, src1=None, c1=0, ldd=None, ld0=None, ld1=None):
    if w3_packed is None or src0.dtype != torch.float32 or (src1 is not None and src1.dtype != torch.float32):
        return 0
    if w3_packed.dtype != torch.bfloat16 or w3_packed.dim() != 4:
        return 0
    ld0 = ld0 if ld0 is not None else src0.shape[-1]
    ld1 = ld1 if ld1 is not None else (src1.shape[-1] if src1 is not None else 0)
    d = _s3_desc(src0, c0, w3_packed, None, n, batch, h1, w1, src1, c1, ACT_NONE, None, ldd if ldd is not None else n, ld0, ld1)
    return int(_lib.load().ccvpe_upconv3x3_s3_ok(ctypes.byref(d)))


def upconv3x3_s3_form_ok(src0, c0, w3_packed, n, form, *, batch, h1, w1, src1=None, c1=0, ldd=None, ld0=None, ld1=None):
    if not upconv3x3_s3_ok(src0, c0, w3_packed, n, batch=batch, h1=h1, w1=w1, src1=src1, c1=c1, ldd=ldd, ld0=ld0, ld1=ld1):
        return 0
    ld0 = ld0 if ld0 is not None else src0.shape[-1]
    ld1 = ld1 if ld1 is not None else (src1.shape[-1] if src1 is not None else 0)
    d = _s3_desc(src0, c0, w3_packed, None, n, batch, h1, w1, src1, c1, ACT_NONE, None, ldd if ldd is not None else n, ld0, ld1)
    return int(_lib.load().ccvpe_upconv3x3_s3_form_ok(ctypes.byref(d), form))


def upconv3x3_s3(src0, c0, w3_packed, shift9, n, *, batch, h1, w1, src1=None, c1=0, act=ACT_NONE, dst=None, ldd=None, ld0=None,
                 ld1=None, form=None):
    lib = _lib.load()
    for t, nm in ((src0, "src0"), (src1, "src1"), (shift9, "shift9"), (dst, "dst")):
        _chk(t, nm)
    _chk(w3_packed, "w", torch.bfloat16)
    ld0 = ld0 if ld0 is not None else src0.shape[-1]
    ld1 = ld1 if ld1 is not None else (src1.shape[-1] if src1 is not None else 0)
    if dst is None:
        ldd = ldd if ldd is not None else n
        dst = _empty((batch, 2 * h1, 2 * w1, ldd), device=src0.device)
    elif ldd is None:
        ldd = dst.shape[-1]
    d = _s3_desc(src0, c0, w3_packed, shift9, n, batch, h1, w1, src1, c1, act, dst, ldd, ld0, ld1)
    rec = _recorder
    ev0 = rec.begin() if rec is not None else None
    if form is None:
        check(lib.ccvpe_upconv3x3_s3_f32(ctypes.byref(d), _stream()), "ccvpe_upconv3x3_s3_f32")
    else:
        check(lib.ccvpe_upconv3x3_s3_form_f32(ctypes.byref(d), form, _stream()), "ccvpe_upconv3x3_s3_form_f32")
    if rec is not None:
        m = batch * h1 * w1 * 4
        k_eff = 4 * c0 + 9 * c1
        flops = 2.0 * m * n * k_eff
        nbytes = 4.0 * (batch * h1 * w1 * c0 + m * c1 + m * n + 4 * n * k_eff)
        rec.end(upconv_s3_route_name(d, form or 0), "up3x3 M%d N%d Keff%d" % (m, n, k_eff), flops, nbytes, ev0)
    return dst


def _pw_s3_desc(src0, c0, w3_packed, n, batch, in_h, in_w, two, gate, scale, shift, residual, act, dst, ldd, ld0):
    d = ConvDesc()
    d.src0, d.src1, d.gate, d.w = _ptr(src0), None, _ptr(gate), _ptr(w3_packed)
    d.scale, d.shift, d.residual = _ptr(scale), _ptr(shift), _ptr(residual)
    d.dst = _ptr(dst) if dst is not None else None
    d.c0, d.ld0, d.c1, d.ld1 = c0, ld0, 0, 0
    d.batch, d.in_h, d.in_w = batch, in_h, in_w
    d.kh, d.kw, d.stride, d.pad = (2, 2, 2, 0) if two else (1, 1, 1, 0)
    d.n, d.kpad = n, w3_packed.shape[0] * w3_packed.shape[2]
    d.ldd = ldd
    d.ldres = residual.shape[-1] if residual is not None else 0
    d.act, d.out_mode = act, OUT_NHWC
    return d


def pw_s3_ok(src0, c0, w3_packed, n, *, batch, in_h, in_w, two=False, gate=None, residual=None, act=ACT_NONE, ldd=None, ld0=None):
    if w3_packed is None or src0.dtype != torch.float32 or (residual is not None and residual.dtype != torch.float32):
        return 0
    if w3_packed.dtype != torch.bfloat16 or w3_packed.dim() != 3 or w3_packed.shape[1] != (n + 15) // 16 * 16 or w3_packed.shape[2] != 48:
        return 0
    ld0 = ld0 if ld0 is not None else src0.shape[-1]
    d = _pw_s3_desc(src0, c0, w3_packed, n, batch, in_h, in_w, two, gate, None, None, residual, act, None, ldd if ldd is not None else n, ld0)
    return int(_lib.load().ccvpe_pw_s3_ok(ctypes.byref(d)))


def pw_s3_route_name(desc):
    r = _lib.load().ccvpe_pw_s3_route(ctypes.byref(desc))
    if r <= 0:
        raise _lib.CcvpeError("ccvpe_pw_s3_route: the kernel does not compute this layer")
    return "pw_s3_kernel<%d,%d,%d,%d>" % ((r >> 8) & 0xf, (r >> 12) & 0xf, (r >> 16) & 0xf, (r >> 20) & 0xf)


def pw_s3(src0, c0, w3_packed, n, *, batch, in_h, in_w, two=False, gate=None, scale=None, shift=None, residual=None, act=ACT_NONE,
          dst=None, ldd=None, ld0=None):
    lib = _lib.load()
    for t, nm in ((src0, "src0"), (gate, "gate"), (scale, "scale"), (shift, "shift"), (residual, "residual"), (dst, "dst")):
        _chk(t, nm)
    _chk(w3_packed, "w", torch.bfloat16)
    if w3_packed.dim() != 3 or w3_packed.shape[1] != (n + 15) // 16 * 16 or w3_packed.shape[2] != 48:
        raise ValueError("w is not the three-plane pack of models._pack_pw_s3 for n = %d" % n)
    ld0 = ld0 if ld0 is not None else src0.shape[-1]
    ho, wo = (in_h // 2, in_w // 2) if two else (in_h, in_w)
    if dst is None:
        ldd = ldd if ldd is not None else n
        dst = _empty((batch, ho, wo, ldd), device=src0.device)
    elif ldd is None:
        ldd = dst.shape[-1]
    d = _pw_s3_desc(src0, c0, w3_packed, n, batch, in_h, in_w, two, gate, scale, shift, residual, act, dst, ldd, ld0)
    rec = _recorder
    ev0 = rec.begin() if rec is not None else None
    check(lib.ccvpe_pw_s3_f32(ctypes.byref(d), _stream()), "ccvpe_pw_s3_f32")
    if rec is not None:
        m = batch * ho * wo
        k_alg = (4 if two else 1) * c0
        flops = 2.0 * m * n * k_alg
        nbytes = 4.0 * (batch * in_h * in_w * c0 + m * n + n * k_alg + (m * n if residual is not None else 0))
        rec.end(pw_s3_route_name(d), "%s M%d N%d K%d" % ("2x2 s2" if two else "1x1 s1", m, n, k_alg), flops, nbytes, ev0)
    return dst


def tail512(x, c0, w_packed, shift9, w2, b2, cout, normalize, *, batch, h1, w1, split=False, want_softmax=False):
    lib = _lib.load()
    dt = _act_dtype(x)
    _chk(x, "x", dt)
    _chk(w_packed, "w", dt)
    for t, nm in ((shift9, "shift9"), (w2, "w2"), (b2, "b2")):
        _chk(t, nm)
    if tuple(w2.shape) != (cout, 3, 3, 16) or tuple(shift9.shape) != (9, 16) or w_packed.shape[0] != 4 or w_packed.shape[1] != 16:
        raise ValueError("tail512: w [4,16,kpad], shift9 [9,16], w2 [cout,3,3,16] expected")
    out = _empty((batch, cout, 2 * h1, 2 * w1), device=x.device, dtype=torch.float32)
    d = _lib.TailDesc()
    d.x, d.w, d.shift9, d.w2, d.b2, d.out = _ptr(x), _ptr(w_packed), _ptr(shift9), _ptr(w2), _ptr(b2), _ptr(out)
    d.batch, d.h1, d.w1 = batch, h1, w1
    d.c0, d.ld0, d.kpad = c0, x.shape[-1], w_packed.shape[-1]
    split = int(split)
    d.cout, d.normalize, d.split = cout, int(bool(normalize)), split
    smx = None
    if want_softmax:
        npart = lib.ccvpe_tail512_partials(ctypes.byref(d), int(dt != torch.float32))
        if npart <= 0:
            check(int(npart) if npart < 0 else -1, "ccvpe_tail512_partials")
        smx = _empty((batch, npart, 2), device=x.device, dtype=torch.float32)
        d.softmax_partial = _ptr(smx)
    rec = _recorder
    ev0 = rec.begin() if rec is not None else None
    fn = lib.ccvpe_tail512_f32 if dt == torch.float32 else lib.ccvpe_tail512_bf16
    check(fn(ctypes.byref(d), _stream()), "ccvpe_tail512")
    if rec is not None:
        m = batch * h1 * w1 * 4
        esz = 4.0 if dt == torch.float32 else 2.0
        rec.end("tail512_kernel<%s,%d>" % (("f32", "f32 as bf16 hi+lo", "f32 as bf16 hi+mid+lo")[split] if dt == torch.float32 else "bf16", cout), "tail M%d Keff%d" % (m, 4 * c0),
                2.0 * m * 16 * (4 * c0 + 9 * cout), esz * batch * h1 * w1 * c0 + 4.0 * m * cout, ev0)
    return (out, smx) if want_softmax else out


def softmax_apply(logits, partials):
    lib = _lib.load()
    _chk(logits, "logits")
    _chk(partials, "partials")
    rows, n = logits.shape
    out = _empty(logits.shape, device=logits.device, dtype=logits.dtype)
    check(lib.ccvpe_softmax_apply_f32(_ptr(logits), _ptr(partials), partials.shape[1], _ptr(out), rows, n, _stream()),
          "ccvpe_softmax_apply_f32")
    return out


def tail512_ok(h1, w1, n_a):
    return n_a == 16 and h1 % 16 == 0 and w1 % 16 == 0


def stem_conv(x_nchw, w, scale, shift, circular, out_dtype=torch.float32):
    lib = _lib.load()
    for t, nm in ((x_nchw, "x"), (w, "w"), (scale, "scale"), (shift, "shift")):
        _chk(t, nm)
    b, c, h, wd = x_nchw.shape
    if c != 3:
        raise ValueError("stem expects 3 input channels")
    ho, wo = (h + 1 - 3) // 2 + 1, (wd + 1 - 3) // 2 + 1
    y = _empty((b, ho, wo, 32), device=x_nchw.device, dtype=out_dtype)
    fn = lib.ccvpe_stem_conv_f32 if out_dtype == torch.float32 else lib.ccvpe_stem_conv_bf16
    check(fn(_ptr(x_nchw), _ptr(w), _ptr(scale), _ptr(shift), _ptr(y), b, h, wd, int(bool(circular)), _stream()),
          "ccvpe_stem_conv")
    return y


def stem_dw_supported(in_h, in_w, circular):
    return _lib.load().ccvpe_stem_dw_nblk(in_h, in_w, int(bool(circular)))


def stem_dw(x_nchw, w, s0, b0, w_dw, s1, b1, circular, out_dtype=torch.float32):
    lib = _lib.load()
    for t, nm in ((x_nchw, "x"), (w, "w"), (s0, "s0"), (b0, "b0"), (w_dw, "w_dw"), (s1, "s1"), (b1, "b1")):
        _chk(t, nm)
    b, c, h, wd = x_nchw.shape
    if c != 3 or w_dw.numel() != 9 * 32:
        raise ValueError("stem_dw expects 3 input channels and a 3x3x32 depthwise weight")
    nblk = stem_dw_supported(h, wd, circular)
    if nblk <= 0:
        raise _lib.CcvpeError("stem_dw: unsupported shape %s" % (tuple(x_nchw.shape),))
    ho, wo = (h + 1 - 3) // 2 + 1, (wd + 1 - 3) // 2 + 1
    y = _empty((b, ho, wo, 32), device=x_nchw.device, dtype=out_dtype)
    part = _empty((b, nblk, 32), device=x_nchw.device, dtype=torch.float32)
    rec = _recorder
    ev0 = rec.begin() if rec is not None else None
    fn = lib.ccvpe_stem_dw_f32 if out_dtype == torch.float32 else lib.ccvpe_stem_dw_bf16
    check(fn(_ptr(x_nchw), _ptr(w), _ptr(s0), _ptr(b0), _ptr(w_dw), _ptr(s1), _ptr(b1), _ptr(y), _ptr(part), b, h, wd,
             int(bool(circular)), _stream()), "ccvpe_stem_dw")
    if rec is not None:
        flops = 2.0 * b * ho * wo * 32 * (27 + 9)
        nbytes = 4.0 * b * 3 * h * wd + (4.0 if out_dtype == torch.float32 else 2.0) * b * ho * wo * 32
        rec.end("stem_dw_kernel", "in %dx%dx3" % (h, wd), flops, nbytes, ev0)
    return y, part


def dwconv(x, w, scale, shift, k, stride, circular):
    lib = _lib.load()
    dt = _act_dtype(x)
    _chk(x, "x", dt)
    for t, nm in ((w, "w"), (scale, "scale"), (shift, "shift")):
        _chk(t, nm)
    b, h, wd, c = x.shape
    tot = (k - 1) if stride == 1 else (k - 2)
    ho, wo = (h + tot - k) // stride + 1, (wd + tot - k) // stride + 1
    nblk = lib.ccvpe_dwconv_nblk(h, wd, c, stride)
    if nblk <= 0:
        raise _lib.CcvpeError("ccvpe_dwconv_nblk rejected shape %s" % (tuple(x.shape),))
    y = _empty((b, ho, wo, c), device=x.device, dtype=dt)
    part = _empty((b, nblk, c), device=x.device, dtype=torch.float32)
    fn = lib.ccvpe_dwconv_f32 if dt == torch.float32 else lib.ccvpe_dwconv_bf16
    check(fn(_ptr(x), _ptr(w), _ptr(scale), _ptr(shift), _ptr(y), _ptr(part), b, h, wd, c, k, stride,
             int(bool(circular)), _stream()), "ccvpe_dwconv")
    return y, part


def mbconv_front_supported(in_h, in_w, cin, mid, k, stride):
    n = _lib.load().ccvpe_mbconv_front_nblk(in_h, in_w, cin, mid, k, stride)
    if n < 0:
        raise _lib.CcvpeError("ccvpe_mbconv_front_nblk rejected k=%d stride=%d" % (k, stride))
    return n


def mbconv_band_plan(in_h, in_w, cin, mid, k, stride, batch):
    r = _lib.load().ccvpe_mbconv_band_plan(in_h, in_w, cin, mid, k, stride, batch)
    if r <= 0:
        return None
    return dict(nkk=r & 0xf, tpw=(r >> 4) & 0xf, ry=(r >> 8) & 0xf, cpg=(r >> 12) & 0xff, ngrp=(r >> 20) & 0xff)


def mbconv_front(x, w_exp, s0, b0, w_dw, s1, b1, mid, k, stride, circular):
    lib = _lib.load()
    dt = _act_dtype(x)
    _chk(x, "x", dt)
    _chk(w_exp, "w_exp", dt)
    for t, nm in ((s0, "s0"), (b0, "b0"), (w_dw, "w_dw"), (s1, "s1"), (b1, "b1")):
        _chk(t, nm)
    b, h, wd, cin = x.shape
    nblk = mbconv_front_supported(h, wd, cin, mid, k, stride)
    if nblk == 0:
        raise _lib.CcvpeError("mbconv_front: unsupported shape %s" % (tuple(x.shape),))
    tot = (k - 1) if stride == 1 else (k - 2)
    ho, wo = (h + tot - k) // stride + 1, (wd + tot - k) // stride + 1
    y = _empty((b, ho, wo, mid), device=x.device, dtype=dt)
    part = _empty((b, nblk, mid), device=x.device, dtype=torch.float32)
    rec = _recorder
    ev0 = rec.begin() if rec is not None else None
    fn = lib.ccvpe_mbconv_front_f32 if dt == torch.float32 else lib.ccvpe_mbconv_front_bf16
    check(fn(_ptr(x), _ptr(w_exp), w_exp.shape[1], _ptr(s0), _ptr(b0), _ptr(w_dw), _ptr(s1), _ptr(b1), _ptr(y),
             _ptr(part), b, h, wd, cin, mid, k, stride, int(bool(circular)), _stream()), "ccvpe_mbconv_front")
    if rec is not None:
        flops = 2.0 * b * h * wd * cin * mid + 2.0 * b * ho * wo * mid * k * k
        nbytes = (4.0 if dt == torch.float32 else 2.0) * (b * h * wd * cin + b * ho * wo * mid)
        route = lib.ccvpe_mbconv_front_route(h, wd, cin, mid, k, stride, int(dt != torch.float32), b)
        kname = {1: "mbconv_front_kernel", 2: "mbconv_plane_kernel", 3: "mbconv_band_kernel"}.get(route, "mbconv_front_kernel")
        rec.end("%s<%d,%d>" % (kname, k, stride), "in %dx%dx%d mid %d" % (h, wd, cin, mid), flops, nbytes, ev0)
    return y, part


def se_gate(part, hw, w1, b1, w2, b2):
    lib = _lib.load()
    for t, nm in ((part, "part"), (w1, "w1"), (b1, "b1"), (w2, "w2"), (b2, "b2")):
        _chk(t, nm)
    b, nblk, c = part.shape
    cs = w1.shape[0]
    gate = _empty((b, c), device=part.device, dtype=torch.float32)
    check(lib.ccvpe_se_gate_f32(_ptr(part), nblk, 1.0 / float(hw), _ptr(w1), _ptr(b1), _ptr(w2), _ptr(b2),
                                _ptr(gate), b, c, cs, _stream()), "ccvpe_se_gate_f32")
    return gate


def ground_descriptor(y1, wh, bh, cd):
    lib = _lib.load()
    for t, nm in ((y1, "y1"), (wh, "wh"), (bh, "bh")):
        _chk(t, nm)
    b, h, w, ld = y1.shape
    cd_arr = (ctypes.c_int * 6)(*cd)
    out = _empty((b, w * sum(cd)), device=y1.device, dtype=torch.float32)
    check(lib.ccvpe_ground_descriptor_f32(_ptr(y1), ld, _ptr(wh), _ptr(bh), cd_arr, _ptr(out), b, h, w,
                                          _stream()), "ccvpe_ground_descriptor_f32")
    return out


def conv3x3_match1(src0, c0, w_packed, n, g, L, shift, stride, ldo, *, batch, in_h, in_w, bias, window_offset=0, out_f32=False,
                   query_only=False):
    lib = _lib.load()
    dt = _act_dtype(src0)
    if dt != torch.bfloat16:
        if query_only:
            return False
        raise ValueError("conv3x3_match1: bf16 storage only")
    _chk(src0, "src0", dt)
    _chk(w_packed, "w", dt)
    _chk(bias, "bias")
    d = ConvDesc()
    d.src0, d.src1, d.gate, d.w = _ptr(src0), None, None, _ptr(w_packed)
    d.scale, d.shift, d.residual = None, _ptr(bias), None
    d.c0, d.ld0, d.c1, d.ld1 = c0, src0.shape[-1], 0, 0
    d.batch, d.in_h, d.in_w = batch, in_h, in_w
    d.kh, d.kw, d.stride, d.pad = 3, 3, 1, 1
    d.n, d.kpad, d.ldd, d.ldres = n, w_packed.shape[1], ldo, 0
    d.act, d.out_mode = ACT_NONE, OUT_NHWC
    if query_only:
        return lib.ccvpe_conv3x3_match1_ok(ctypes.byref(d), int(bool(out_f32)), L) == 1
    if not g.is_cuda or g.dtype != torch.float32 or g.stride(-1) != 1:
        raise ValueError("g must be an fp32 device tensor with unit inner stride")
    scores = _empty((batch, 1, in_h, in_w), device=src0.device, dtype=torch.float32)
    cat = _empty((batch, in_h, in_w, ldo), device=src0.device, dtype=torch.float32 if out_f32 else dt)
    d.dst = _ptr(cat)
    rec = _recorder
    ev0 = rec.begin() if rec is not None else None
    check(lib.ccvpe_conv3x3_match1_bf16(ctypes.byref(d), int(bool(out_f32)), _ptr(g), g.stride(0), L, int(shift), int(stride),
                                        int(window_offset), _ptr(scores), _stream()), "ccvpe_conv3x3_match1_bf16")
    if rec is not None:
        m = batch * in_h * in_w
        rec.end("c3n_kernel<bf16,%d,match>" % n, "3x3+match M%d N%d K%d" % (m, n, 9 * c0), 2.0 * m * n * 9 * c0,
                2.0 * m * c0 + (4.0 if out_f32 else 2.0) * m * ldo + 4.0 * m + 2.0 * n * 9 * c0, ev0)
    return scores, cat


def match_level(x, g, L, shifts, n_max, n_tail, stride, ldo, channels=None, window_offset=0):
    lib = _lib.load()
    dt = _act_dtype(x)
    _chk(x, "x", dt)
    if not g.is_cuda or g.dtype != torch.float32 or g.stride(-1) != 1:
        raise ValueError("g must be an fp32 device tensor with unit inner stride")
    b, h, w, ldx = x.shape
    c = channels if channels is not None else ldx
    n = len(shifts)
    sh = (ctypes.c_int * n)(*shifts)
    scores = _empty((b, n, h, w), device=x.device, dtype=torch.float32)
    dstx = _empty((b, h, w, ldo), device=x.device, dtype=dt)
    fn = lib.ccvpe_match_level_f32 if dt == torch.float32 else lib.ccvpe_match_level_bf16
    check(fn(_ptr(x), ldx, _ptr(g), g.stride(0), L, sh, n, n_max, n_tail, stride, window_offset, _ptr(scores), _ptr(dstx),
             ldo, b, h * w, c, _stream()), "ccvpe_match_level")
    return scores, dstx


def head_conv3x3(x, w, bias, cout, normalize):
    lib = _lib.load()
    dt = _act_dtype(x)
    _chk(x, "x", dt)
    for t, nm in ((w, "w"), (bias, "bias")):
        _chk(t, nm)
    b, h, wd, c = x.shape
    if c != 16:
        raise ValueError("head conv expects 16 input channels")
    out = _empty((b, cout, h, wd), device=x.device, dtype=torch.float32)
    fn = lib.ccvpe_head_conv3x3_f32 if dt == torch.float32 else lib.ccvpe_head_conv3x3_bf16
    check(fn(_ptr(x), _ptr(w), _ptr(bias), _ptr(out), b, h, wd, cout, int(bool(normalize)), _stream()),
          "ccvpe_head_conv3x3")
    return out


def cast_f32(x):
    if x.dtype == torch.float32:
        return x
    lib = _lib.load()
    _chk(x, "x", torch.bfloat16)
    out = _empty(x.shape, device=x.device, dtype=torch.float32)
    check(lib.ccvpe_cast_bf16_f32(_ptr(x), _ptr(out), x.numel(), _stream()), "ccvpe_cast_bf16_f32")
    return out


def softmax_rows(logits):
    lib = _lib.load()
    _chk(logits, "logits")
    rows, n = logits.shape
    out = _empty(logits.shape, device=logits.device, dtype=logits.dtype)
    check(lib.ccvpe_softmax_rows_f32(_ptr(logits), _ptr(out), rows, n, _stream()), "ccvpe_softmax_rows_f32")
    return out


def stem_conv_raw(x_nchw, w, circular):
    lib = _lib.load()
    _chk(x_nchw, "x")
    _chk(w, "w")
    b, c, h, wd = x_nchw.shape
    ho, wo = (h + 1 - 3) // 2 + 1, (wd + 1 - 3) // 2 + 1
    y = _empty((b, ho, wo, 32), device=x_nchw.device, dtype=torch.float32)
    check(lib.ccvpe_stem_conv_raw_f32(_ptr(x_nchw), _ptr(w), _ptr(y), b, h, wd, int(bool(circular)), _stream()),
          "ccvpe_stem_conv_raw_f32")
    return y


def dwconv_raw(x, w, k, stride, circular):
    lib = _lib.load()
    _chk(x, "x")
    _chk(w, "w")
    b, h, wd, c = x.shape
    tot = (k - 1) if stride == 1 else (k - 2)
    ho, wo = (h + tot - k) // stride + 1, (wd + tot - k) // stride + 1
    y = _empty((b, ho, wo, c), device=x.device, dtype=torch.float32)
    check(lib.ccvpe_dwconv_raw_f32(_ptr(x), _ptr(w), _ptr(y), b, h, wd, c, k, stride, int(bool(circular)), _stream()),
          "ccvpe_dwconv_raw_f32")
    return y


def bn_stats(x, run_mean=None, run_var=None, momentum=0.01):
    lib = _lib.load()
    _chk(x, "x")
    _chk(run_mean, "run_mean")
    _chk(run_var, "run_var")
    c = x.shape[-1]
    rows = x.numel() // c
    mean = _empty((c,), device=x.device, dtype=torch.float32)
    var = _empty((c,), device=x.device, dtype=torch.float32)
    scratch = _empty((lib.ccvpe_bn_stats_nblk(rows) * 3 * c,), device=x.device, dtype=torch.float32)
    check(lib.ccvpe_bn_stats_f32(_ptr(x), rows, c, _ptr(mean), _ptr(var), _ptr(run_mean), _ptr(run_var),
                                 float(momentum), _ptr(scratch), _stream()), "ccvpe_bn_stats_f32")
    return mean, var


def bn_act(x, mean, var, gamma, beta, eps, act, residual=None, dc_scale=None, want_se=False):
    lib = _lib.load()
    for t, nm in ((x, "x"), (mean, "mean"), (var, "var"), (gamma, "gamma"), (beta, "beta"), (residual, "residual"),
                  (dc_scale, "dc_scale")):
        _chk(t, nm)
    b, c = x.shape[0], x.shape[-1]
    rps = x.numel() // (b * c)
    y = _empty(x.shape, device=x.device, dtype=x.dtype)
    part = None
    if want_se:
        part = _empty((b, lib.ccvpe_bn_act_nblk(rps), c), device=x.device, dtype=torch.float32)
    check(lib.ccvpe_bn_act_f32(_ptr(x), _ptr(mean), _ptr(var), _ptr(gamma), _ptr(beta), float(eps), act, _ptr(residual),
                               _ptr(dc_scale), _ptr(y), _ptr(part), b, rps, c, _stream()), "ccvpe_bn_act_f32")
    return (y, part) if want_se else y


def eval_postprocess(heatmap, ori):
    lib = _lib.load()
    _chk(heatmap, "heatmap")
    _chk(ori, "ori")
    b, _, h, w = heatmap.shape
    out = _empty((b, 6), device=heatmap.device, dtype=torch.float32)
    check(lib.ccvpe_eval_postprocess_f32(_ptr(heatmap), _ptr(ori), _ptr(out), b, h, w, _stream()),
          "ccvpe_eval_postprocess_f32")
    return out


def eval_metrics(heatmap, ori, gt, gt_ori, heading_deg, metres_per_pixel, out=None):
    lib = _lib.load()
    for t, nm in ((heatmap, "heatmap"), (ori, "ori"), (gt, "gt"), (gt_ori, "gt_ori")):
        _chk(t, nm)
    for t, nm in ((heading_deg, "heading_deg"), (metres_per_pixel, "metres_per_pixel"), (out, "out")):
        _chk(t, nm, torch.float64)
    b, _, h, w = heatmap.shape
    if ori.shape != (b, 2, h, w) or gt.shape != heatmap.shape or gt_ori.shape != ori.shape:
        raise ValueError("eval_metrics: heatmap/gt [B,1,h,w] and ori/gt_ori [B,2,h,w] expected")
    if heading_deg.numel() != b or metres_per_pixel.numel() != b:
        raise ValueError("eval_metrics: heading_deg and metres_per_pixel must hold one value per sample")
    if out is None:
        out = _empty((b, 12), device=heatmap.device, dtype=torch.float64)
    elif tuple(out.shape) != (b, 12):
        raise ValueError("eval_metrics: out must be [%d,12], got %s" % (b, tuple(out.shape)))
    check(lib.ccvpe_eval_metrics_f32(_ptr(heatmap), _ptr(ori), _ptr(gt), _ptr(gt_ori), _ptr(heading_deg),
                                     _ptr(metres_per_pixel), _ptr(out), b, h, w, _stream()), "ccvpe_eval_metrics_f32")
    return out


def _loss_common(fn, name, tensors, extra):
    lib = _lib.load()
    for i, t in enumerate(tensors):
        _chk(t, "%s arg %d" % (name, i))
    b = tensors[0].shape[0]
    loss = _empty((1,), device=tensors[0].device, dtype=torch.float32)
    scratch = _empty((2 * b,), device=tensors[0].device, dtype=torch.float32)
    return lib, loss, scratch, b


def infonce_loss(scores, labels, temperature=0.1, want_den=False, want_rows=False):
    lib = _lib.load()
    _chk(scores, "infonce scores")
    _chk(labels, "infonce labels")
    b, n = scores.shape
    loss = _empty((1,), device=scores.device, dtype=torch.float32)
    rows = _empty((4 * b + 4,), device=scores.device, dtype=torch.float32)
    nfl = lib.ccvpe_infonce_scratch_floats(b, n)
    if nfl <= 0:
        raise _lib.CcvpeError("ccvpe_infonce_scratch_floats rejected [%d, %d]" % (b, n))
    scratch = _empty((nfl,), device=scores.device, dtype=torch.float32)
    check(lib.ccvpe_infonce_loss_f32(_ptr(scores), _ptr(labels), float(temperature), _ptr(loss), _ptr(rows), _ptr(scratch),
                                     b, n, _stream()), "ccvpe_infonce_loss_f32")
    out = (loss[0],)
    if want_den:
        out = out + (rows[4 * b],)
    if want_rows:
        out = out + (rows,)
    return out if len(out) > 1 else out[0]


def cross_entropy_loss(logits, labels):
    lib, loss, scratch, b = _loss_common(None, "ce", (logits, labels), None)
    check(lib.ccvpe_cross_entropy_loss_f32(_ptr(logits), _ptr(labels), _ptr(loss), _ptr(scratch), b,
                                           logits.shape[1], _stream()), "ccvpe_cross_entropy_loss_f32")
    return loss[0]


def orientation_loss(ori, gt_orientation, gt):
    lib, loss, scratch, b = _loss_common(None, "ori", (ori, gt_orientation, gt), None)
    hw = ori.shape[2] * ori.shape[3]
    check(lib.ccvpe_orientation_loss_f32(_ptr(ori), _ptr(gt_orientation), _ptr(gt), _ptr(loss), _ptr(scratch),
                                         b, hw, _stream()), "ccvpe_orientation_loss_f32")
    return loss[0]
```

ccvpe_amd/plan.py:

```python
import ctypes
import struct
import weakref

import torch

from . import _lib, ops

K_INT, K_FLT, K_NULL, K_WEIGHTS, K_WORKSPACE, K_GRD, K_SAT, K_STREAM, K_BLOB = range(9)
ALIGN = 256

LAUNCHES = ("ccvpe_conv_igemm_f32", "ccvpe_conv_igemm_bf16", "ccvpe_conv_igemm_splitk_f32", "ccvpe_conv_igemm_splitk_bf16",
            "ccvpe_conv3x3_match1_bf16", "ccvpe_conv3x3_wino_f32",
            "ccvpe_upconv3x3_f32", "ccvpe_upconv3x3_bf16", "ccvpe_upconv3x3_s3_f32", "ccvpe_pw_s3_f32", "ccvpe_tail512_f32", "ccvpe_tail512_bf16", "ccvpe_stem_conv_f32",
            "ccvpe_stem_conv_bf16", "ccvpe_stem_dw_f32", "ccvpe_stem_dw_bf16", "ccvpe_dwconv_f32", "ccvpe_dwconv_bf16", "ccvpe_mbconv_front_f32", "ccvpe_mbconv_front_bf16",
            "ccvpe_se_gate_f32", "ccvpe_ground_descriptor_f32", "ccvpe_match_level_f32", "ccvpe_match_level_bf16",
            "ccvpe_head_conv3x3_f32", "ccvpe_head_conv3x3_bf16", "ccvpe_softmax_rows_f32", "ccvpe_softmax_apply_f32", "ccvpe_cast_bf16_f32",
            "ccvpe_eval_postprocess_f32")
QUERIES = ("ccvpe_tail512_partials", "ccvpe_conv3x3_match1_ok", "ccvpe_conv3x3_wino_ok", "ccvpe_upconv3x3_s3_ok", "ccvpe_conv_igemm_splitk_floats", "ccvpe_conv_igemm_route", "ccvpe_conv3x3_variant", "ccvpe_upconv3x3_route", "ccvpe_upconv3x3_s3_route", "ccvpe_pw_s3_ok", "ccvpe_pw_s3_route", "ccvpe_dwconv_nblk", "ccvpe_mbconv_front_nblk", "ccvpe_mbconv_front_route", "ccvpe_mbconv_band_plan", "ccvpe_stem_dw_nblk",
           "ccvpe_last_error", "ccvpe_abi_version")


class _Arena(object):

    def __init__(self, size):
        self.size, self.free, self.peak = size, [(0, size)], 0

    def alloc(self, nbytes):
        n = max(ALIGN, (nbytes + ALIGN - 1) // ALIGN * ALIGN)
        for i, (off, sz) in enumerate(self.free):
            if sz >= n:
                if sz == n:
                    del self.free[i]
                else:
                    self.free[i] = (off + n, sz - n)
                self.peak = max(self.peak, off + n)
                return off, n
        raise MemoryError("plan arena exhausted")

    def release(self, off, n):
        fr = self.free
        lo, hi = 0, len(fr)
        while lo < hi:
            mid = (lo + hi) // 2
            if fr[mid][0] < off:
                lo = mid + 1
            else:
                hi = mid
        fr.insert(lo, (off, n))
        if lo + 1 < len(fr) and fr[lo][0] + fr[lo][1] == fr[lo + 1][0]:
            fr[lo] = (fr[lo][0], fr[lo][1] + fr[lo + 1][1])
            del fr[lo + 1]
        if lo > 0 and fr[lo - 1][0] + fr[lo - 1][1] == fr[lo][0]:
            fr[lo - 1] = (fr[lo - 1][0], fr[lo - 1][1] + fr[lo][1])
            del fr[lo]


def _tensor_ranges(obj, out=None, seen=None):
    out = [] if out is None else out
    seen = set() if seen is None else seen
    if id(obj) in seen:
        return out
    seen.add(id(obj))
    if isinstance(obj, torch.Tensor):
        if obj.is_cuda and obj.numel():
            st = obj.untyped_storage()
            out.append((st.data_ptr(), st.data_ptr() + st.nbytes()))
    elif isinstance(obj, dict):
        for v in obj.values():
            _tensor_ranges(v, out, seen)
    elif isinstance(obj, (list, tuple)):
        for v in obj:
            _tensor_ranges(v, out, seen)
    elif hasattr(obj, "__dict__"):
        _tensor_ranges(vars(obj), out, seen)
    return out


class _Recorder(object):
    def __init__(self, device, arena_bytes, grd, sat, side_fraction=0.45, constants=None):
        self.ws = torch.empty((arena_bytes,), dtype=torch.uint8, device=device)
        self.base = self.ws.data_ptr()
        self.split = int(arena_bytes * (1.0 - side_fraction)) // ALIGN * ALIGN
        self.arenas = (_Arena(self.split), _Arena(arena_bytes - self.split))
        self.size = arena_bytes
        self.grd, self.sat = grd, sat
        self.calls, self.blobs = [], []
        self.weights, self.weights_bytes = {}, 0
        self.seen = {}
        self.constants = sorted(constants) if constants is not None else None
        self.main = torch.cuda.current_stream().cuda_stream
        self.quarantine = []
        self.n_waits = 0

    def sid(self):
        return 0 if torch.cuda.current_stream().cuda_stream == self.main else 1

    @property
    def peak(self):
        return max(self.arenas[0].peak, self.split + self.arenas[1].peak if self.arenas[1].peak else 0)

    def empty(self, shape, dtype, device):
        shape = tuple(int(s) for s in shape)
        n = 1
        for s in shape:
            n *= s
        item = torch.empty((), dtype=dtype).element_size()
        region = self.sid()
        off, size = self.arenas[region].alloc(n * item)
        goff = off + (self.split if region else 0)
        t = torch.empty((0,), dtype=dtype, device=device).set_(self.ws.untyped_storage(), goff // item, shape)
        weakref.finalize(t, self._release, region, off, size)
        return t

    def _release(self, region, off, size):
        if self.sid() == region:
            self.arenas[region].release(off, size)
        else:
            self.quarantine.append((region, off, size))

    def wait(self, waiter, waitee):
        a = 0 if waiter.cuda_stream == self.main else 1
        b = 0 if waitee.cuda_stream == self.main else 1
        if a == b:
            return
        self.calls.append(("@wait", [(K_INT, a), (K_INT, b)], a))
        self.n_waits += 1
        if a == 0:
            for region, off, size in self.quarantine:
                self.arenas[region].release(off, size)
            self.quarantine = []

    def note(self, t):
        p = t.data_ptr()
        if not (self.base <= p < self.base + self.size):
            self._check_constant(p, t.numel() * t.element_size())
            self.seen[p] = t

    def _is_input(self, addr):
        for t in (self.grd, self.sat):
            p = t.data_ptr()
            if p <= addr < p + t.numel() * t.element_size():
                return True
        return False

    def _check_constant(self, addr, nbytes=1):
        if self.constants is None or self._is_input(addr):
            return
        import bisect
        i = bisect.bisect_right(self.constants, (addr, float("inf"))) - 1
        if i >= 0 and self.constants[i][0] <= addr and addr + max(nbytes, 1) <= self.constants[i][1]:
            return
        raise RuntimeError("plan: pointer 0x%x (%d bytes) is neither workspace, nor an input, nor part of the weights packed before "
                           "recording: an intermediate allocated outside ops._empty would be frozen as a constant" % (addr, nbytes))

    def classify(self, addr):
        if addr is None or addr == 0:
            return K_NULL, 0
        if self.base <= addr < self.base + self.size:
            return K_WORKSPACE, addr - self.base
        for kind, t in ((K_GRD, self.grd), (K_SAT, self.sat)):
            p = t.data_ptr()
            if p <= addr < p + t.numel() * t.element_size():
                return kind, addr - p
        return K_WEIGHTS, self._weight_offset(addr)

    def _weight_offset(self, addr):
        self._check_constant(addr)
        if addr in self.weights:
            return self.weights[addr][0]
        t = self.seen.get(addr)
        if t is None:
            for p, tt in self.seen.items():
                if p <= addr < p + tt.numel() * tt.element_size() and p in self.weights:
                    return self.weights[p][0] + (addr - p)
            raise RuntimeError("plan: pointer 0x%x is neither in the workspace, nor an input, nor a tensor passed through ops._ptr" % addr)
        if not t.is_contiguous():
            raise RuntimeError("plan: non-contiguous weight tensor")
        off = (self.weights_bytes + ALIGN - 1) // ALIGN * ALIGN
        self.weights[addr] = (off, t)
        self.weights_bytes = off + t.numel() * t.element_size()
        return off

    def log(self, name, argtypes, args):
        out = []
        for i, (ty, a) in enumerate(zip(argtypes, args)):
            if isinstance(a, ctypes.Array):
                self.blobs.append((bytes(a), []))
                out.append((K_BLOB, len(self.blobs) - 1))
            elif type(a).__name__ == "CArgObject":
                out.append((K_BLOB, self._struct_blob(a._obj)))
            elif ty is ctypes.c_void_p:
                v = a.value if isinstance(a, ctypes.c_void_p) else a
                if i == len(argtypes) - 1:
                    out.append((K_STREAM, 0))
                else:
                    out.append(self.classify(v))
            elif ty is ctypes.c_float:
                out.append((K_FLT, struct.unpack("<I", struct.pack("<f", float(a)))[0]))
            else:
                out.append((K_INT, int(a) & 0xffffffffffffffff))
        self.calls.append((name, out, self.sid()))

    def _struct_blob(self, obj):
        relocs = []
        for fname, ftype in obj._fields_:
            if ftype is ctypes.c_void_p:
                kind, off = self.classify(getattr(obj, fname))
                relocs.append((getattr(type(obj), fname).offset, kind, off))
        self.blobs.append((bytes(obj), relocs))
        return len(self.blobs) - 1


class _RecordingLib(object):

    def __init__(self, lib, rec):
        self._lib, self._rec = lib, rec

    def __getattr__(self, name):
        fn = getattr(self._lib, name)
        if name in QUERIES:
            return fn
        if name not in LAUNCHES:
            raise RuntimeError("plan: %s is not an entry point an eval forward may contain" % name)
        argtypes = _lib.PROTOTYPES[name][1]

        def call(*args):
            self._rec.log(name, argtypes, args)
            return fn(*args)
        return call


class Plan(object):

    def __init__(self, rec, outputs, grd, sat):
        main_peak = (rec.arenas[0].peak + ALIGN - 1) // ALIGN * ALIGN
        shift = rec.split - main_peak

        def fix(off):
            return off - shift if off >= rec.split else off
        self.calls = [(n, [(k, fix(v)) if k == K_WORKSPACE else (k, v) for k, v in a], sid) for n, a, sid in rec.calls]
        self.blobs = [(d, [(f, k, fix(v)) if k == K_WORKSPACE else (f, k, v) for f, k, v in r]) for d, r in rec.blobs]
        self.workspace_bytes = main_peak + (rec.arenas[1].peak + ALIGN - 1) // ALIGN * ALIGN
        self.n_waits = rec.n_waits
        self.weights_bytes = (rec.weights_bytes + ALIGN - 1) // ALIGN * ALIGN
        self.grd_shape, self.sat_shape = tuple(grd.shape), tuple(sat.shape)
        self.outputs = []
        for t in outputs:
            if t.dtype != torch.float32 or t.dim() > 4:
                raise RuntimeError("plan: outputs must be fp32 tensors of at most 4 dimensions")
            kind, off = rec.classify(t.data_ptr())
            if kind != K_WORKSPACE:
                raise RuntimeError("plan: an output lives outside the workspace")
            extent = 4 * (1 + sum((n - 1) * st for n, st in zip(t.shape, t.stride())))
            self.outputs.append((fix(off), extent, tuple(t.shape), tuple(t.stride())))
        blob = torch.zeros((max(self.weights_bytes, ALIGN),), dtype=torch.uint8, device=grd.device)
        for off, t in rec.weights.values():
            n = t.numel() * t.element_size()
            blob[off:off + n] = t.reshape(-1).view(torch.uint8)
        self.weights = blob

    def to_bytes(self):
        lib = _lib.load()
        head = [b"CCVPLAN1", struct.pack("<II", lib.ccvpe_abi_version(), 0),
                struct.pack("<QQQQ", self.workspace_bytes, self.weights_bytes,
                            4 * _numel(self.grd_shape), 4 * _numel(self.sat_shape)),
                struct.pack("<IIII", len(self.calls), len(self.blobs), len(self.outputs), 0)]
        for off, nbytes, shape, strides in self.outputs:
            dims = list(shape) + [1] * (4 - len(shape))
            strd = list(strides) + [0] * (4 - len(strides))
            head.append(struct.pack("<QQII4Q4Q", off, nbytes, 0, len(shape), *(dims + strd)))
        for data, relocs in self.blobs:
            head.append(struct.pack("<II", len(data), len(relocs)))
            for field, kind, value in relocs:
                head.append(struct.pack("<IIQ", field, kind, value))
            head.append(data + b"\0" * ((-len(data)) % 8))
        for name, args, sid in self.calls:
            head.append(name.encode().ljust(48, b"\0"))
            head.append(struct.pack("<II", len(args), sid))
            for kind, value in args:
                head.append(struct.pack("<IIQ", kind, 0, value))
        body = b"".join(head)
        body += b"\0" * ((-len(body)) % ALIGN)
        return body + bytes(self.weights[:self.weights_bytes].cpu().numpy().tobytes())

    def save(self, path):
        with open(path, "wb") as f:
            f.write(self.to_bytes())


def _numel(shape):
    n = 1
    for s in shape:
        n *= int(s)
    return n


def record(net, grd, sat, arena_bytes=None):
    if net.training:
        raise RuntimeError("plan.record: eval mode only (net.eval())")
    if not (grd.is_cuda and sat.is_cuda and grd.dtype == torch.float32 and sat.dtype == torch.float32
            and grd.is_contiguous() and sat.is_contiguous()):
        raise ValueError("plan.record: grd / sat must be contiguous fp32 device tensors")
    dev = grd.device
    with torch.no_grad():
        if arena_bytes is None:
            torch.cuda.synchronize(dev)
            torch.cuda.reset_peak_memory_stats(dev)
            before = torch.cuda.memory_allocated(dev)
            net(grd, sat)
            torch.cuda.synchronize(dev)
            arena_bytes = int(1.5 * (torch.cuda.max_memory_allocated(dev) - before)) + (64 << 20)
        constants = _tensor_ranges([net._packed(), net])
    lib = _lib.load()
    saved = (ops._record, _lib.load, torch.cuda.Stream.wait_stream)
    for attempt in range(4):
        rec = _Recorder(dev, arena_bytes, grd, sat, constants=constants)
        orig_wait = saved[2]

        def wait_stream(self, other, _rec=rec, _orig=orig_wait):
            _rec.wait(self, other)
            return _orig(self, other)
        try:
            ops._record = rec
            proxy = _RecordingLib(lib, rec)
            _lib.load = lambda: proxy
            torch.cuda.Stream.wait_stream = wait_stream
            with torch.no_grad():
                outs = net(grd, sat)
            break
        except MemoryError:
            arena_bytes = int(arena_bytes * 1.5)
            outs = None
        finally:
            ops._record, _lib.load, torch.cuda.Stream.wait_stream = saved
            torch.cuda.synchronize(dev)
    if outs is None:
        raise MemoryError("plan.record: workspace regions exhausted after growing the arena")
    torch.cuda.synchronize(dev)
    return Plan(rec, outs, grd, sat), outs


class PlannedForward(object):

    def __init__(self, net, grd, sat):
        self.plan, _ = record(net, grd, sat)
        lib = _lib.load()
        self._blob = self.plan.to_bytes()
        self.workspace = torch.empty((max(self.plan.workspace_bytes, ALIGN),), dtype=torch.uint8, device=grd.device)
        self.weights = torch.empty((max(self.plan.weights_bytes, ALIGN),), dtype=torch.uint8, device=grd.device)
        ctx = ctypes.c_void_p()
        host = ctypes.create_string_buffer(self._blob, len(self._blob))
        _lib.check(lib.ccvpe_ctx_create(ctypes.cast(host, ctypes.c_void_p), len(self._blob), ctypes.c_void_p(self.weights.data_ptr()),
                                        ctypes.c_void_p(self.workspace.data_ptr()), ctypes.byref(ctx)), "ccvpe_ctx_create")
        self._ctx = ctx
        self._lib = lib
        self._fin = weakref.finalize(self, lib.ccvpe_ctx_destroy, ctx)
        self.outputs = []
        for off, nbytes, shape, strides in self.plan.outputs:
            self.outputs.append(torch.as_strided(self.workspace[off:off + nbytes].view(torch.float32), shape, strides))
        self.grd_shape, self.sat_shape = self.plan.grd_shape, self.plan.sat_shape

    def __call__(self, grd, sat):
        if tuple(grd.shape) != self.grd_shape or tuple(sat.shape) != self.sat_shape:
            raise ValueError("PlannedForward was built for grd %s / sat %s" % (self.grd_shape, self.sat_shape))
        if not (grd.is_cuda and sat.is_cuda and grd.dtype == torch.float32 and sat.dtype == torch.float32
                and grd.is_contiguous() and sat.is_contiguous()):
            raise ValueError("PlannedForward: contiguous fp32 device inputs required")
        _lib.check(self._lib.ccvpe_forward(self._ctx, ctypes.c_void_p(grd.data_ptr()), ctypes.c_void_p(sat.data_ptr()), None,
                                           ctypes.c_void_p(torch.cuda.current_stream().cuda_stream)), "ccvpe_forward")
        return tuple(self.outputs)
```

include/ccvpe_hip.h:

```cpp
#ifndef CCVPE_HIP_H
#define CCVPE_HIP_H

#ifdef __cplusplus
extern "C" {
#endif

#define CCVPE_OK 0
#define CCVPE_EINVAL (-1)
#define CCVPE_ELAUNCH (-2)

#define CCVPE_ACT_NONE 0
#define CCVPE_ACT_RELU 1
#define CCVPE_ACT_SWISH 2
#define CCVPE_ACT_RELU_MASK 3

#define CCVPE_OUT_NHWC 0
#define CCVPE_OUT_DECONV2X 1

#define CCVPE_MAX_SHIFTS 48

const char* ccvpe_last_error(void);
int ccvpe_abi_version(void);

typedef struct ccvpe_conv_desc {
  const float* src0;
  const float* src1;
  const float* gate;
  const float* w;
  const float* scale;
  const float* shift;
  const float* residual;
  float* dst;
  int c0, ld0, c1, ld1;
  int batch, in_h, in_w;
  int kh, kw, stride, pad;
  int n;
  int kpad;
  int ldd, ldres;
  int act;
  int out_mode;
} ccvpe_conv_desc;

int ccvpe_conv_igemm_f32(const ccvpe_conv_desc* desc, void* stream);

int ccvpe_conv_igemm_splitk_floats(const ccvpe_conv_desc* desc, int is_bf16);
#define CCVPE_ROUTE_IGEMM 0
#define CCVPE_ROUTE_PW_GEMM 1
#define CCVPE_ROUTE_CONV3X3 2
#define CCVPE_ROUTE_C3N 3
#define CCVPE_ROUTE_PW_RING 4
#define CCVPE_ROUTE_PWN 5
int ccvpe_conv_igemm_route(const ccvpe_conv_desc* desc, int is_bf16, int out_f32);
int ccvpe_conv3x3_variant(const ccvpe_conv_desc* desc, int is_bf16);
int ccvpe_set_narrow_kernels(int on);
int ccvpe_set_pw_ring_kernels(int on);
int ccvpe_set_pwn_kernels(int on);
int ccvpe_set_mbconv_plane_kernels(int mode);
int ccvpe_conv3x3_wino_ok(const ccvpe_conv_desc* desc);
int ccvpe_conv3x3_wino_f32(const ccvpe_conv_desc* desc, void* stream);
int ccvpe_conv3x3_match1_ok(const ccvpe_conv_desc* desc, int out_f32, int L);
int ccvpe_conv3x3_match1_bf16(const ccvpe_conv_desc* desc, int out_f32, const float* g, int ldg, int L, int shift, int stride,
                              int window_offset, float* scores, void* stream);
int ccvpe_conv_igemm_splitk_f32(const ccvpe_conv_desc* desc, float* scratch, void* stream);

typedef struct ccvpe_upconv_desc {
  const void* src0;
  const void* src1;
  const void* w;
  const float* shift9;
  void* dst;
  int c0, ld0, c1, ld1;
  int batch, h1, w1;
  int n, kpad, ldd;
  int act;
} ccvpe_upconv_desc;

int ccvpe_upconv3x3_f32(const ccvpe_upconv_desc* desc, void* stream);
int ccvpe_upconv3x3_bf16(const ccvpe_upconv_desc* desc, void* stream);
#define CCVPE_UPROUTE_GATHER 0
#define CCVPE_UPROUTE_HALO 1
#define CCVPE_UPROUTE_DMA 2
#define CCVPE_UPROUTE_DMA_PAIR 3
#define CCVPE_UPROUTE_UP2 4
int ccvpe_upconv3x3_route(const ccvpe_upconv_desc* desc, int is_bf16);
int ccvpe_upconv3x3_s3_ok(const ccvpe_upconv_desc* desc);
int ccvpe_upconv3x3_s3_f32(const ccvpe_upconv_desc* desc, void* stream);
int ccvpe_upconv3x3_s3_form_ok(const ccvpe_upconv_desc* desc, int form);
int ccvpe_upconv3x3_s3_route(const ccvpe_upconv_desc* desc, int form);
int ccvpe_upconv3x3_s3_form_f32(const ccvpe_upconv_desc* desc, int form, void* stream);
int ccvpe_set_s3_quad(int on);
int ccvpe_pw_s3_ok(const ccvpe_conv_desc* desc);
int ccvpe_pw_s3_route(const ccvpe_conv_desc* desc);
int ccvpe_pw_s3_f32(const ccvpe_conv_desc* desc, void* stream);

typedef struct ccvpe_tail_desc {
  const void* x;
  const void* w;
  const float* shift9;
  const float* w2;
  const float* b2;
  float* out;
  int batch, h1, w1;
  int c0, ld0, kpad;
  int cout, normalize, split;
  float* softmax_partial;
} ccvpe_tail_desc;

int ccvpe_tail512_f32(const ccvpe_tail_desc* desc, void* stream);
int ccvpe_tail512_bf16(const ccvpe_tail_desc* desc, void* stream);
int ccvpe_tail512_partials(const ccvpe_tail_desc* desc, int is_bf16);
int ccvpe_softmax_apply_f32(const float* logits, const float* partials, int n_partials, float* out, int rows, int n,
                            void* stream);

typedef struct ccvpe_ctx ccvpe_ctx;
int ccvpe_ctx_create(const void* plan, long long n_bytes, void* weights_dev, void* workspace_dev, ccvpe_ctx** ctx);
int ccvpe_ctx_destroy(ccvpe_ctx* ctx);
int ccvpe_ctx_info(const ccvpe_ctx* ctx, long long* workspace_bytes, long long* weights_bytes, long long* grd_bytes,
                   long long* sat_bytes, int* n_outputs, int* n_calls);
int ccvpe_ctx_output(const ccvpe_ctx* ctx, int i, void** dev_ptr, long long* bytes, int* ndim, long long* dims4,
                     long long* strides4);
int ccvpe_forward(ccvpe_ctx* ctx, const void* grd, const void* sat, void** out, void* stream);

int ccvpe_stem_conv_f32(const float* x_nchw, const float* w, const float* scale, const float* shift,
                        float* y, int batch, int in_h, int in_w, int circular, void* stream);

int ccvpe_dwconv_nblk(int in_h, int in_w, int channels, int stride);
int ccvpe_dwconv_f32(const float* x, const float* w, const float* scale, const float* shift, float* y,
                     float* se_partial, int batch, int in_h, int in_w, int channels, int k, int stride,
                     int circular, void* stream);

int ccvpe_stem_dw_nblk(int in_h, int in_w, int circular);
int ccvpe_stem_dw_f32(const float* x_nchw, const float* w, const float* s0, const float* b0, const float* w_dw,
                      const float* s1, const float* b1, float* y, float* se_partial, int batch, int in_h,
                      int in_w, int circular, void* stream);
int ccvpe_stem_dw_bf16(const float* x_nchw, const float* w, const float* s0, const float* b0, const float* w_dw,
                       const float* s1, const float* b1, void* y, float* se_partial, int batch, int in_h,
                       int in_w, int circular, void* stream);

int ccvpe_mbconv_front_nblk(int in_h, int in_w, int cin, int mid, int k, int stride);
int ccvpe_mbconv_front_route(int in_h, int in_w, int cin, int mid, int k, int stride, int is_bf16, int batch);
int ccvpe_mbconv_band_plan(int in_h, int in_w, int cin, int mid, int k, int stride, int batch);
int ccvpe_mbconv_front_f32(const float* x, const float* w_exp, int kpad, const float* s0, const float* b0,
                           const float* w_dw, const float* s1, const float* b1, float* y, float* se_partial,
                           int batch, int in_h, int in_w, int cin, int mid, int k, int stride, int circular,
                           void* stream);

int ccvpe_se_gate_f32(const float* se_partial, int nblk, float inv_hw, const float* w1, const float* b1,
                      const float* w2, const float* b2, float* gate, int batch, int channels,
                      int squeezed, void* stream);

int ccvpe_ground_descriptor_f32(const float* y1, int ld, const float* wh, const float* bh, const int* cd,
                                float* out, int batch, int h, int w, void* stream);

int ccvpe_set_match_mfma(int on);
#define CCVPE_MATCH_ROUTE_INTS 10
int ccvpe_match_route(int elem_size, int L, const int* shifts, int n_shifts, int n_max, int n_tail, int stride,
                      int window_offset, int ldx, int ldo, int batch, int hw, int channels, int* out);
int ccvpe_match_level_f32(const float* x, int ldx, const float* g, int ldg, int L, const int* shifts,
                          int n_shifts, int n_max, int n_tail, int stride, int window_offset, float* scores,
                          float* dstx, int ldo, int batch, int hw, int channels, void* stream);

int ccvpe_head_conv3x3_f32(const float* x, const float* w, const float* bias, float* out_nchw, int batch,
                           int h, int w_, int cout, int normalize, void* stream);

int ccvpe_softmax_rows_f32(const float* logits, float* out, int rows, int n, void* stream);
int ccvpe_multi_copy_f32(const void* const* srcs, void* const* dsts, const int* counts, int n, void* stream);
int ccvpe_gather_repack_f32(void* const* dsts, const void* const* srcs, const long long* idx_off, const int* counts,
                            const int* idx, int n_chunks, void* stream);
int ccvpe_gather_repack_chunk(void);
int ccvpe_cast_bf16_f32(const void* src, float* dst, long n_elems, void* stream);

int ccvpe_eval_postprocess_f32(const float* heatmap, const float* ori, float* out, int batch, int h, int w,
                               void* stream);

int ccvpe_eval_metrics_f32(const float* heatmap, const float* ori, const float* gt, const float* gt_ori,
                           const double* heading_deg, const double* metres_per_pixel, double* rows, int batch, int h,
                           int w, void* stream);

int ccvpe_infonce_scratch_floats(int batch, int n);
int ccvpe_infonce_loss_f32(const float* scores, const float* labels, float temperature, float* loss,
                           float* rows, float* scratch, int batch, int n, void* stream);
int ccvpe_cross_entropy_loss_f32(const float* logits, const float* labels, float* loss, float* scratch,
                                 int batch, int n, void* stream);
int ccvpe_orientation_loss_f32(const float* ori, const float* gt_ori, const float* gt, float* loss,
                               float* scratch, int batch, int hw, void* stream);

int ccvpe_stem_conv_raw_f32(const float* x_nchw, const float* w, float* y, int batch, int in_h, int in_w,
                            int circular, void* stream);
int ccvpe_dwconv_raw_f32(const float* x, const float* w, float* y, int batch, int in_h, int in_w, int channels,
                         int k, int stride, int circular, void* stream);
int ccvpe_bn_stats_nblk(int rows);
int ccvpe_bn_stats_f32(const float* x, int rows, int channels, float* mean, float* var, float* run_mean,
                       float* run_var, float momentum, float* scratch, void* stream);
int ccvpe_bn_act_nblk(int rows_per_sample);
int ccvpe_bn_act_f32(const float* x, const float* mean, const float* var, const float* gamma, const float* beta,
                     float eps, int act, const float* residual, const float* dc_scale, float* y,
                     float* se_partial, int batch, int rows_per_sample, int channels, void* stream);

int ccvpe_conv_wgrad_tile(int n, int ncols);
int ccvpe_conv_wgrad_scratch_floats(int batch, int in_h, int in_w, int kh, int kw, int stride, int pad, int ctot,
                                    int n);
int ccvpe_conv_wgrad_f32(const float* src0, int c0, int ld0, const float* src1, int c1, int ld1, const float* dy,
                         int ldy, float* dw, float* scratch, int batch, int in_h, int in_w, int kh, int kw,
                         int stride, int pad, int n, void* stream);
int ccvpe_conv_wgrad_bias_f32(const float* src0, int c0, int ld0, const float* src1, int c1, int ld1, const float* dy,
                              int ldy, float* dw, float* dbias, float* scratch, int batch, int in_h, int in_w, int kh,
                              int kw, int stride, int pad, int n, void* stream);
int ccvpe_conv_wgrad_gated_f32(const float* x, int c, int ld, const float* gate, const float* dy, int ldy, float* dw,
                               float* scratch, int batch, int in_h, int in_w, int n, void* stream);
int ccvpe_colsum_f32(const float* x, int rows, int channels, int ld, float* out, float* scratch, void* stream);

int ccvpe_bn_bwd_nblk(int rows_per_sample);
int ccvpe_bn_act_bwd_f32(const float* x, const float* dv, const float* mean, const float* var, const float* gamma,
                         const float* beta, const float* gate, const float* dmean, const float* dc_scale, float eps,
                         int act, float* dx, float* dgamma, float* dbeta, float* scratch, int batch,
                         int rows_per_sample, int channels, void* stream);
int ccvpe_bn_act_bwd_frozen_f32(const float* x, const float* dv, const float* mean, const float* var, const float* gamma,
                                const float* beta, const float* gate, const float* dmean, const float* dc_scale, float eps,
                                int act, float* dx, float* dgamma, float* dbeta, float* scratch, int batch,
                                int rows_per_sample, int channels, void* stream);
int ccvpe_se_bn_bwd_reduce_f32(const float* x, const float* dv, const float* mean, const float* var, const float* gamma,
                               const float* beta, float eps, int act, float* A, float* scratch, int batch,
                               int rows_per_sample, int channels, void* stream);
int ccvpe_se_bn_bwd_apply_f32(const float* x, const float* dv, const float* mean, const float* var, const float* gamma,
                              const float* beta, const float* gate, const float* dmean, float eps, int act, const float* A,
                              float* dx, float* dgamma, float* dbeta, int batch, int rows_per_sample, int channels,
                              void* stream);
int ccvpe_se_dgate_f32(const float* x, const float* dv, const float* mean, const float* var, const float* gamma,
                       const float* beta, float eps, int act, float* part, int batch, int rows_per_sample,
                       int channels, void* stream);
int ccvpe_se_bwd_f32(const float* se_partial, int nblk, float inv_hw, const float* dgate_partial, int ndg,
                     const float* w1, const float* b1, const float* w2t, const float* b2, float* dmean, float* dw1,
                     float* db1, float* dw2, float* db2, float* scratch, int batch, int channels, int squeezed,
                     void* stream);
int ccvpe_dwconv_dgrad_f32(const float* dy, const float* w, float* dx, int batch, int in_h, int in_w, int channels,
                           int k, int stride, int circular, void* stream);
int ccvpe_dwconv_wgrad_nblk(int in_h, int in_w, int k, int stride);
int ccvpe_dwconv_wgrad_f32(const float* x, const float* dy, float* dw, float* scratch, int batch, int in_h, int in_w,
                           int channels, int k, int stride, int circular, void* stream);
int ccvpe_relu_bwd_f32(const float* y, const float* dy, float* dx, int n_elems, void* stream);
int ccvpe_gate_mul_f32(const float* u, const float* gate, float* v, int batch, int rows_per_sample, int channels,
                       void* stream);

#define CCVPE_HEAD_WGRAD_BLOCKS 1024
#define CCVPE_HEAD_BWD_SCRATCH ((CCVPE_HEAD_WGRAD_BLOCKS + 1) * 2 * 145)
int ccvpe_softmax_bwd_f32(const float* heatmap, const float* dheatmap, const float* dlogits_direct, float* dlogits,
                          int rows, int n, void* stream);
int ccvpe_l2norm2_bwd_f32(const float* raw, const float* dout, float* draw, int batch, int hw, void* stream);
int ccvpe_head_conv3x3_bwd_f32(const float* x, const float* w, const float* dout, float* dx, float* dw, float* dbias,
                               float* scratch, int batch, int h, int wd, int cout, int relu_mask_x, void* stream);
int ccvpe_ground_descriptor_bwd_f32(const float* y1, int ld, const float* wh, const int* cd, const float* dout,
                                    float* dy1, float* dwh, float* dbh, int batch, int h, int w, void* stream);
int ccvpe_add_cols_f32(const float* src, int ld_src, int col_off, float* dst, int ld_dst, int channels, int rows,
                       int accumulate, void* stream);
int ccvpe_stem_wgrad_nblk(int batch, int in_h, int in_w);
int ccvpe_stem_conv_wgrad_f32(const float* x_nchw, const float* dy, float* dw, float* scratch, int batch, int in_h,
                              int in_w, int circular, void* stream);
int ccvpe_match_bwd_nblk(int hw, int batch, int channels);
int ccvpe_match_level_bwd_f32(const float* x, int ldx, const float* g, int ldg, int L, const int* shifts, int n_shifts,
                              int n_max, int n_tail, int stride, int window_offset, const float* scores, const float* dscores,
                              const float* ddst, int ldo, float* dx, int lddx, float* dg, int ldg_out, float* scratch,
                              int batch, int hw, int channels, void* stream);

int ccvpe_infonce_loss_bwd_f32(const float* scores, const float* labels, float temperature, const float* dloss,
                               const float* rows, float* dscores, int batch, int n, void* stream);
int ccvpe_cross_entropy_loss_bwd_f32(const float* logits, const float* labels, const float* dloss, float* dlogits,
                                     int batch, int n, void* stream);
int ccvpe_orientation_loss_bwd_f32(const float* ori, const float* gt_ori, const float* gt, const float* dloss,
                                   float* dori, int batch, int hw, void* stream);

int ccvpe_train_targets_nblk(int h, int w);
int ccvpe_train_targets_f32(const float* center_xy, const float* angle_deg, int n_bins, float sigma, float* gt,
                            float* gt_norm, float* gt_ori, float* lab1, float* lab2, float* lab3, float* lab4,
                            float* lab5, float* lab6, float* scratch, int batch, int h, int w, void* stream);
int ccvpe_train_targets_ordered_f32(const float* center_xy, const float* angle_deg, int n_bins, int ascending, float sigma,
                                    float* gt, float* gt_norm, float* gt_ori, float* lab1, float* lab2, float* lab3,
                                    float* lab4, float* lab5, float* lab6, float* scratch, int batch, int h, int w,
                                    void* stream);
int ccvpe_adam_chunk_elems(void);
int ccvpe_adam_hyper_floats(void);
int ccvpe_adam_step_f32(const void* table, const float* hyper, const int* chunk_tensor, const int* chunk_off, int n_chunks,
                        float grad_scale, void* stream);

int ccvpe_adam_device_layout(int what);
int ccvpe_grad_sqnorm_f32(const void* table, const int* chunk_tensor, const int* chunk_off, int n_chunks, float grad_scale,
                          float* partials, void* stream);
int ccvpe_adam_prepare_f32(const void* table, const double* consts, float* steps, float* hyper, int n_tensors,
                           const float* partials, int n_partials, float max_norm, float* scalars, void* stream);
int ccvpe_adam_update_f32(const void* table, const float* hyper, const int* chunk_tensor, const int* chunk_off, int n_chunks,
                          float grad_scale, const float* scalars, void* stream);

int ccvpe_preprocess_u8_f32(const unsigned char* src, int in_h, int in_w, const int* xbounds, const int* xcoef,
                            int xksize, const int* ybounds, const int* ycoef, int yksize, unsigned char* tmp, float* dst,
                            int out_h, int out_w, int keep_w, int roll, const float* mean, const float* stdv,
                            void* stream);

int ccvpe_resize_u8(const unsigned char* src, int in_h, int in_w, const int* xbounds, const int* xcoef, int xksize,
                    const int* ybounds, const int* ycoef, int yksize, unsigned char* tmp, unsigned char* dst_u8,
                    int out_h, int out_w, void* stream);
int ccvpe_gather_norm_u8_f32(const long long* srcs, const int* rolls, int batch, int h, int w, int keep_w,
                             const float* mean, const float* stdv, float* dst, void* stream);

int ccvpe_window_resize_norm_u8_f32(const unsigned char* map, int map_h, int map_w, const int* origins, int batch, int box_h,
                                    int box_w, const int* xbounds, const int* xcoef, int xksize, const int* ybounds,
                                    const int* ycoef, int yksize, const float* mean, const float* stdv, float* dst, int out_h,
                                    int out_w, void* stream);

int ccvpe_kitti_align_u8(const unsigned char* src, long src_bytes, const long long* offsets, const long long* rows,
                         int batch, unsigned char* dst, int crop_h, int crop_w, void* stream);

int ccvpe_kitti_align_norm_u8_f32(const long long* srcs, const long long* rows, int batch, const float* mean,
                                  const float* stdv, float* dst, int crop_h, int crop_w, void* stream);

int ccvpe_conv_igemm_bf16(const ccvpe_conv_desc* desc, int out_f32, void* stream);
int ccvpe_conv_igemm_splitk_bf16(const ccvpe_conv_desc* desc, int out_f32, float* scratch, void* stream);
int ccvpe_stem_conv_bf16(const float* x_nchw, const float* w, const float* scale, const float* shift, void* y,
                         int batch, int in_h, int in_w, int circular, void* stream);
int ccvpe_dwconv_bf16(const void* x, const float* w, const float* scale, const float* shift, void* y,
                      float* se_partial, int batch, int in_h, int in_w, int channels, int k, int stride,
                      int circular, void* stream);
int ccvpe_mbconv_front_bf16(const void* x, const void* w_exp, int kpad, const float* s0, const float* b0,
                            const float* w_dw, const float* s1, const float* b1, void* y, float* se_partial,
                            int batch, int in_h, int in_w, int cin, int mid, int k, int stride, int circular,
                            void* stream);
int ccvpe_match_level_bf16(const void* x, int ldx, const float* g, int ldg, int L, const int* shifts,
                           int n_shifts, int n_max, int n_tail, int stride, int window_offset, float* scores, void* dstx, int ldo,
                           int batch, int hw, int channels, void* stream);
int ccvpe_head_conv3x3_bf16(const void* x, const float* w, const float* bias, float* out_nchw, int batch, int h,
                            int w_, int cout, int normalize, void* stream);

#ifdef __cplusplus
}
#endif
#endif
```

Baseline: 2852.

## Add split-three bf16 MFMA 3x3 conv kernel with fused matching epilogue for fp32

```diff
diff --git a/ccvpe_amd/_lib.py b/ccvpe_amd/_lib.py
--- a/ccvpe_amd/_lib.py
+++ b/ccvpe_amd/_lib.py
@@ -90,6 +90,10 @@
     "ccvpe_pw_s3_ok": (c_int, [ctypes.POINTER(ConvDesc)]),
     "ccvpe_pw_s3_route": (c_int, [ctypes.POINTER(ConvDesc)]),
     "ccvpe_pw_s3_f32": (c_int, [ctypes.POINTER(ConvDesc), c_void_p]),
+    "ccvpe_conv3x3_s3n_ok": (c_int, [ctypes.POINTER(ConvDesc), c_int]),
+    "ccvpe_conv3x3_s3n_route": (c_int, [ctypes.POINTER(ConvDesc), c_int]),
+    "ccvpe_conv3x3_s3n_f32": (c_int, [ctypes.POINTER(ConvDesc), c_void_p]),
+    "ccvpe_conv3x3_match1_s3n_f32": (c_int, [ctypes.POINTER(ConvDesc), c_int, c_void_p, c_int, c_int, c_int, c_int, c_int, c_void_p, c_void_p]),
     "ccvpe_stem_conv_f32": (c_int, [c_void_p] * 5 + [c_int] * 4 + [c_void_p]),
     "ccvpe_dwconv_nblk": (c_int, [c_int] * 4),
     "ccvpe_dwconv_f32": (c_int, [c_void_p] * 6 + [c_int] * 7 + [c_void_p]),
diff --git a/ccvpe_amd/csrc/conv3x3_s3n.hip b/ccvpe_amd/csrc/conv3x3_s3n.hip
--- /dev/null
+++ b/ccvpe_amd/csrc/conv3x3_s3n.hip
@@ -0,0 +1,438 @@
+#include "split3_impl.h"
+
+namespace ccvpe {
+
+struct S3nParams {
+  const float* src;
+  const void* w;
+  const float* bias;
+  float* dst;
+  int c0, ld0, H, W;
+  int N, nb, pitch;
+  int ldd;
+  int tiles_x, tiles_y, tiles_total;
+  int w_off;
+  const float* g;
+  float* scores;
+  int ldg, L, off;
+};
+
+#ifdef S3N_STAMPS
+__device__ unsigned long long s3n_dbg[8];
+#define S3N_STAMP_TILE() unsigned long long st_prev = __builtin_amdgcn_s_memtime(), st_w0 = 0; st_acc[7] += 1
+#define S3N_STAMP(k) do { const unsigned long long st_now = __builtin_amdgcn_s_memtime(); st_acc[k] += st_now - st_prev; st_prev = st_now; } while (0)
+#define S3N_STAMP_WAIT_BEGIN() st_w0 = __builtin_amdgcn_s_memtime()
+#define S3N_STAMP_WAIT_END() st_acc[6] += __builtin_amdgcn_s_memtime() - st_w0
+#else
+#define S3N_STAMP_TILE()
+#define S3N_STAMP(k)
+#define S3N_STAMP_WAIT_BEGIN()
+#define S3N_STAMP_WAIT_END()
+#endif
+
+constexpr int S3N_HC = 18;
+constexpr int S3N_GRP = 3;
+
+static inline int s3n_pitch(int nb) { return S3_ROW * nb + ((nb & 1) ? 0 : 8); }
+
+template <int NT>
+struct S3nGeom {
+  static constexpr int NW = 4;
+  static constexpr int RING = NT <= 3 ? 2 : 3;
+  static constexpr bool PIPE = NT >= 4;
+  static constexpr int TH = 2 * NW, HR = TH + 2, HPX = HR * S3N_HC;
+  static constexpr int NB_MAX = NT <= 3 ? 3 : 5;
+  static constexpr int W_EXACT = (S3N_GRP * 16 * NT * 6 + 63) / 64;
+  static constexpr int WQ = (W_EXACT + NW - 1) / NW;
+  static constexpr int W_INSTR = RING > 2 ? WQ * NW : W_EXACT;
+  static constexpr int WBUF_DW = W_INSTR * 256;
+  static constexpr int TAB_DW = 2 * 16 * NT;
+  static int lds_bytes(int nb) { return (HPX * s3n_pitch(nb) + RING * WBUF_DW + TAB_DW) * 4; }
+};
+
+template <int NT, bool MATCH>
+__global__ __launch_bounds__(64 * S3nGeom<NT>::NW) void conv3x3_s3n_kernel(const S3nParams p) {
+  using G = S3nGeom<NT>;
+  constexpr int MT = 2, ROW = S3_ROW, HC = S3N_HC, NW = G::NW, NTHR = 64 * NW, RING = G::RING, WQ = G::WQ;
+  constexpr int LIF = (G::HPX * 4 * G::NB_MAX + NTHR - 1) / NTHR;
+
+  extern __shared__ __attribute__((aligned(16))) float s3n_sm[];
+  float* Us = s3n_sm;
+  float* Ws = s3n_sm + p.w_off;
+  float* Tb = Ws + RING * G::WBUF_DW;
+
+  const int tid = threadIdx.x;
+  const int lane = tid & 63;
+  const int wave = sgpr(tid >> 6);
+  const int frow = lane & 15;
+  const int g4 = lane >> 4;
+
+  const int nb = sgpr(p.nb), pitch = sgpr(p.pitch), ld0s = sgpr(p.ld0), c0s = sgpr(p.c0);
+  constexpr int npad = 16 * NT;
+
+  unsigned wvoff[WQ];
+  {
+    const int valid = S3N_GRP * npad * 6;
+#pragma unroll
+    for (int q = 0; q < WQ; ++q) wvoff[q] = (unsigned)min((wave + NW * q) * 64 + lane, valid - 1) * 16u;
+  }
+  const unsigned ws_lds = (unsigned)(uintptr_t)(__attribute__((address_space(3))) float*)Ws;
+  const size_t group_bytes = (size_t)S3N_GRP * npad * (ROW * 4);
+  auto dma_w = [&](int grp, int dbuf) {
+    const char* sbase = reinterpret_cast<const char*>(p.w) + (size_t)grp * group_bytes;
+#pragma unroll
+    for (int q = 0; q < WQ; ++q) {
+      const int gq = wave + NW * q;
+      if (gq >= G::W_INSTR) continue;
+      const unsigned lds = __builtin_amdgcn_readfirstlane(ws_lds + (unsigned)((dbuf * G::WBUF_DW + gq * 256) * 4));
+      asm volatile("s_mov_b32 m0, %0\n\ts_nop 0\n\tglobal_load_lds_dwordx4 %1, %2" ::"s"(lds), "v"(wvoff[q]), "s"(sbase) : "memory", "m0");
+    }
+  };
+
+  const int ngrp = 3 * nb;
+
+  int h_dst[LIF], h_yx[LIF], h_ch[LIF];
+  {
+    const int nb4 = 4 * nb;
+    const unsigned dm = (65536u + (unsigned)nb4 - 1u) / (unsigned)nb4;
+    const int total = G::HPX * nb4;
+#pragma unroll
+    for (int u = 0; u < LIF; ++u) {
+      const int idx = min(tid + u * NTHR, total - 1);
+      const int pxl = (int)(((unsigned)idx * dm) >> 16);
+      const int piece = idx - pxl * nb4;
+      const int hy = pxl / HC, hx = pxl - hy * HC;
+      h_yx[u] = (hy << 8) | hx;
+      h_ch[u] = piece * 4 < c0s ? piece * 4 : -1;
+      h_dst[u] = tid + u * NTHR < total ? pxl * pitch + (piece >> 2) * ROW + (piece & 3) * 2 : -1;
+    }
+  }
+  f32x4 hv[LIF];
+  unsigned hkeep = 0;
+  float gpre[3] = {0.f, 0.f, 0.f};
+  const int gk = [&] { int k = min(tid, 16 * NT - 1) + p.off; return k >= p.N ? k - p.N : k; }();
+  const bool gin = tid < p.N && gk < p.L;
+  auto tile_decode3 = [&](int t, int& b, int& y0, int& x0) {
+    const int tx = t % p.tiles_x, r = t / p.tiles_x;
+    b = r / p.tiles_y;
+    y0 = (r - b * p.tiles_y) * G::TH;
+    x0 = tx * 16;
+  };
+  auto load_halo = [&](int t) {
+    int b, y0, x0;
+    tile_decode3(t, b, y0, x0);
+    hkeep = 0;
+#pragma unroll
+    for (int u = 0; u < LIF; ++u) {
+      const int iy = y0 - 1 + (h_yx[u] >> 8), ix = x0 - 1 + (h_yx[u] & 255);
+      const bool ok = (unsigned)iy < (unsigned)p.H && (unsigned)ix < (unsigned)p.W && h_ch[u] >= 0;
+      const unsigned off = ok ? ((unsigned)((b * p.H + iy) * p.W + ix) * (unsigned)ld0s + (unsigned)h_ch[u]) * 4u : 0u;
+      hv[u] = *reinterpret_cast<const f32x4*>(reinterpret_cast<const char*>(p.src) + off);
+      hkeep |= ok ? (1u << u) : 0u;
+    }
+    if constexpr (MATCH) {
+      const float* gb = p.g + (size_t)b * p.ldg;
+      gpre[0] = gb[gin ? gk : 0];
+      gpre[1] = gb[lane < p.L ? lane : 0];
+      gpre[2] = gb[lane + 64 < p.L ? lane + 64 : 0];
+    }
+  };
+  auto store_halo = [&]() {
+#pragma unroll
+    for (int u = 0; u < LIF; ++u)
+      if (h_dst[u] >= 0) store_planes(Us + h_dst[u], keep_if(hv[u], (hkeep >> u) & 1u));
+  };
+
+  f32x4 bq[NT];
+#pragma unroll
+  for (int j = 0; j < NT; ++j) {
+    const int n = 16 * j + 4 * g4;
+    const float* bp = p.bias + (n < p.N ? n : 0);
+    bq[j] = keep_if((f32x4){bp[0], bp[1], bp[2], bp[3]}, n < p.N);
+  }
+  const S3Frag fr(g4);
+  const int hfrag = (wave * MT * HC + frow) * pitch;
+  const int wfrag = frow * ROW;
+
+  int t = blockIdx.x;
+#ifdef S3N_STAMPS
+  unsigned long long st_acc[8] = {0, 0, 0, 0, 0, 0, 0, 0};
+#endif
+  load_halo(t);
+  while (true) {
+  S3N_STAMP_TILE();
+  int b, y0, x0;
+  tile_decode3(t, b, y0, x0);
+#pragma unroll
+  for (int r = 0; r < RING - 1; ++r)
+    if (r < ngrp) dma_w(r, r);
+
+  float gnorm = 1.f;
+  if constexpr (MATCH) {
+    if (tid < 16 * NT) {
+      Tb[tid] = gin ? gpre[0] : 0.f;
+      Tb[16 * NT + tid] = gin ? 1.f : 0.f;
+    }
+    float s = 0.f;
+#pragma unroll
+    for (int h = 0; h < 2; ++h) {
+      const float v = lane + 64 * h < p.L ? gpre[1 + h] : 0.f;
+      s = fmaf(v, v, s);
+    }
+    gnorm = sqrtf(wave_sum(s));
+  }
+
+  store_halo();
+  S3N_STAMP(0);
+  asm volatile("s_waitcnt vmcnt(0)" ::: "memory");
+  S3N_STAMP(1);
+  const int tnext = t + (int)gridDim.x;
+  const bool has_next = tnext < p.tiles_total;
+  if (has_next) load_halo(tnext);
+
+  f32x4 acc[MT][NT];
+#pragma unroll
+  for (int i = 0; i < MT; ++i)
+#pragma unroll
+    for (int j = 0; j < NT; ++j) acc[i][j] = (f32x4){0.f, 0.f, 0.f, 0.f};
+  struct Frags { f32x4 a1[MT], a2[MT], w1[NT], w2[NT], w3[NT]; };
+  auto load_frags = [&](Frags& f, const float* abase, int istride, const float* wb) {
+#pragma unroll
+    for (int i = 0; i < MT; ++i) {
+      f.a1[i] = *reinterpret_cast<const f32x4*>(abase + i * istride + fr.a1);
+      f.a2[i] = *reinterpret_cast<const f32x4*>(abase + i * istride + fr.a2);
+    }
+#pragma unroll
+    for (int j = 0; j < NT; ++j) {
+      f.w1[j] = *reinterpret_cast<const f32x4*>(wb + j * 16 * ROW + fr.w1);
+      f.w2[j] = *reinterpret_cast<const f32x4*>(wb + j * 16 * ROW + fr.w2);
+      f.w3[j] = *reinterpret_cast<const f32x4*>(wb + j * 16 * ROW + fr.w3);
+    }
+  };
+  auto mma = [&](const Frags& f) {
+#pragma unroll
+    for (int j = 0; j < NT; ++j)
+#pragma unroll
+      for (int i = 0; i < MT; ++i) acc[i][j] = mfma_stage<bf16_t>(f.w1[j], f.a1[i], acc[i][j]);
+#pragma unroll
+    for (int j = 0; j < NT; ++j)
+#pragma unroll
+      for (int i = 0; i < MT; ++i) acc[i][j] = mfma_stage<bf16_t>(f.w2[j], f.a1[i], acc[i][j]);
+#pragma unroll
+    for (int j = 0; j < NT; ++j)
+#pragma unroll
+      for (int i = 0; i < MT; ++i) acc[i][j] = mfma_stage<bf16_t>(f.w3[j], f.a2[i], acc[i][j]);
+  };
+
+  asm volatile("s_waitcnt lgkmcnt(0)\n\ts_barrier" ::: "memory");
+  S3N_STAMP(2);
+  {
+    int tap = 0, chunk = 0, slot = 0, nslot = RING - 1;
+    for (int grp = 0; grp < ngrp; ++grp) {
+      const bool ahead = grp + RING - 1 < ngrp;
+      if (ahead) dma_w(grp + RING - 1, nslot);
+      const float* wbuf = Ws + slot * G::WBUF_DW + wfrag;
+      const float* ab[S3N_GRP];
+#pragma unroll
+      for (int u = 0; u < S3N_GRP; ++u) {
+        const int ky = tap / 3, kx = tap - 3 * ky;
+        ab[u] = Us + hfrag + (ky * HC + kx) * pitch + chunk * ROW;
+        if (++chunk == nb) { chunk = 0; ++tap; }
+      }
+      Frags f[2];
+      load_frags(f[0], ab[0], HC * pitch, wbuf);
+#pragma unroll
+      for (int u = 0; u < S3N_GRP; ++u) {
+        if constexpr (G::PIPE) {
+          if (u + 1 < S3N_GRP) load_frags(f[(u + 1) & 1], ab[u + 1], HC * pitch, wbuf + (u + 1) * npad * ROW);
+          __builtin_amdgcn_sched_barrier(0);
+          mma(f[u & 1]);
+        } else {
+          if (u > 0) load_frags(f[0], ab[u], HC * pitch, wbuf + u * npad * ROW);
+          mma(f[0]);
+        }
+      }
+      S3N_STAMP_WAIT_BEGIN();
+      if (ahead) asm volatile("s_waitcnt vmcnt(%0) lgkmcnt(0)\n\ts_barrier" ::"n"((RING - 2) * WQ) : "memory");
+      else asm volatile("s_waitcnt vmcnt(0) lgkmcnt(0)\n\ts_barrier" ::: "memory");
+      S3N_STAMP_WAIT_END();
+      slot = slot + 1 == RING ? 0 : slot + 1;
+      nslot = nslot + 1 == RING ? 0 : nslot + 1;
+    }
+  }
+
+  S3N_STAMP(3);
+  const int x1 = x0 + frow;
+#pragma unroll
+  for (int i = 0; i < MT; ++i) {
+    const int y1 = y0 + wave * MT + i;
+    const size_t pix = (size_t)(b * p.H + y1) * p.W + x1;
+    f32x4 v[NT];
+#pragma unroll
+    for (int j = 0; j < NT; ++j) {
+      const int n = 16 * j + 4 * g4;
+      v[j] = acc[i][j] + bq[j];
+    }
+    if constexpr (!MATCH) {
+#pragma unroll
+      for (int j = 0; j < NT; ++j) {
+        const int n = 16 * j + 4 * g4;
+        if (n < p.N) *reinterpret_cast<f32x4*>(p.dst + pix * p.ldd + n) = v[j];
+      }
+    } else {
+      float s2 = 0.f, wn = 0.f, dt = 0.f;
+#pragma unroll
+      for (int j = 0; j < NT; ++j) {
+        const f32x4 gq = *reinterpret_cast<const f32x4*>(Tb + 16 * j + 4 * g4);
+        const f32x4 wq = *reinterpret_cast<const f32x4*>(Tb + 16 * NT + 16 * j + 4 * g4);
+#pragma unroll
+        for (int r = 0; r < 4; ++r) {
+          const float x2 = v[j][r] * v[j][r];
+          s2 += x2;
+          wn = fmaf(x2, wq[r], wn);
+          dt = fmaf(v[j][r], gq[r], dt);
+        }
+      }
+      s2 += __shfl_xor(s2, 16, 64); wn += __shfl_xor(wn, 16, 64); dt += __shfl_xor(dt, 16, 64);
+      s2 += __shfl_xor(s2, 32, 64); wn += __shfl_xor(wn, 32, 64); dt += __shfl_xor(dt, 32, 64);
+      const float inv = 1.0f / fmaxf(sqrtf(s2), 1e-12f);
+      const float score = dt / (sqrtf(wn) * gnorm);
+      float* drow = p.dst + pix * p.ldd;
+#pragma unroll
+      for (int j = 0; j < NT; ++j) {
+        const int n = 16 * j + 4 * g4;
+        if (n < p.N) *reinterpret_cast<f32x4*>(drow + n) = v[j] * inv;
+        else if (n < p.ldd) *reinterpret_cast<f32x4*>(drow + n) = (f32x4){n == p.N ? score : 0.f, 0.f, 0.f, 0.f};
+      }
+      for (int n = 16 * NT + 4 * g4; n < p.ldd; n += 16)
+        *reinterpret_cast<f32x4*>(drow + n) = (f32x4){n == p.N ? score : 0.f, 0.f, 0.f, 0.f};
+      if (g4 == 0) p.scores[pix] = score;
+    }
+  }
+  S3N_STAMP(4);
+  if (!has_next) break;
+  t = tnext;
+  asm volatile("s_waitcnt lgkmcnt(0)\n\ts_barrier" ::: "memory");
+  S3N_STAMP(5);
+  }
+#ifdef S3N_STAMPS
+  if (tid == 0)
+    for (int k = 0; k < 8; ++k) atomicAdd(&s3n_dbg[k], st_acc[k]);
+#endif
+}
+
+struct S3nRoute { int nt, nb, match, th, nw; long tiles_x, tiles_y, total; int lds; };
+
+static bool s3n_measured_size(const ccvpe_conv_desc* d, int match) {
+  const long m = (long)d->batch * d->in_h * d->in_w;
+  if (d->c0 != d->n) return false;
+  if (d->n == 40) return m >= 524288;
+  if (d->n == 80) return match && m >= 16384;
+  return false;
+}
+
+template <int NT> static int s3n_lds(int nb) { return S3nGeom<NT>::lds_bytes(nb); }
+
+static const char* s3n_pick(const ccvpe_conv_desc* d, int match, S3nRoute& r) {
+  r = S3nRoute{};
+  if (!d) return "null desc";
+  if (d->kh != 3 || d->kw != 3 || d->stride != 1 || d->pad != 1) return "not a 3x3 stride-1 pad-1 layer";
+  if (d->c1 != 0 || d->src1 || d->gate || d->scale || d->residual) return "one source, bias only";
+  if (d->act != CCVPE_ACT_NONE || d->out_mode != CCVPE_OUT_NHWC) return "no activation, NHWC store only";
+  if (d->c0 <= 0 || d->c0 % 8 || d->c0 > 80) return "c0 must be a positive multiple of 8, at most 80";
+  if (d->n <= 0 || d->n % 8 || d->n > 80) return "N must be a positive multiple of 8, at most 80";
+  if (d->batch <= 0 || d->in_h <= 0 || d->in_w <= 0) return "bad shape";
+  if (d->ld0 < d->c0 || d->ld0 % 4) return "bad strides";
+  if (d->ldd % 4 || d->ldd < (match ? d->n + 4 : d->n)) return "bad strides";
+  const int nb = (d->c0 + 15) / 16, npad = (d->n + 15) / 16 * 16;
+  if (d->kpad != 9 * nb * 48) return "kpad is not that of the three-plane pack (models._pack_conv_s3n)";
+  const double px = (double)d->batch * d->in_h * d->in_w;
+  if (px * d->ld0 * 4.0 >= 4294967296.0 || px >= 2147483648.0) return "tensor too large";
+  if ((d->src0 && !aligned16(d->src0)) || (d->w && !aligned16(d->w)) || (d->dst && !aligned16(d->dst)))
+    return "pointers must be 16-byte aligned";
+  r.nt = npad / 16;
+  r.nb = nb;
+  r.match = match ? 1 : 0;
+  int nb_max = 0;
+  switch (r.nt) {
+#define CCVPE_CASE(NT_) case NT_: r.lds = s3n_lds<NT_>(nb); r.th = S3nGeom<NT_>::TH; r.nw = S3nGeom<NT_>::NW; nb_max = S3nGeom<NT_>::NB_MAX; break;
+    CCVPE_CASE(1) CCVPE_CASE(2) CCVPE_CASE(3) CCVPE_CASE(4) CCVPE_CASE(5)
+#undef CCVPE_CASE
+    default: return "no instantiation";
+  }
+  if (nb > nb_max) return "c0 above 48 with N up to 48 is not served (no model has such a layer)";
+  if (r.lds > 160 * 1024) return "the halo does not fit the LDS";
+  if (d->in_h % r.th || d->in_w % 16) return "H must be a multiple of 8 and W of 16";
+  r.tiles_x = d->in_w / 16;
+  r.tiles_y = d->in_h / r.th;
+  r.total = r.tiles_x * r.tiles_y * d->batch;
+  if (r.total > 0x7fffffffL) return "grid too large";
+  return nullptr;
+}
+
+template <int NT, bool MATCH>
+static int launch_s3n(const S3nParams& p, const S3nRoute& r, hipStream_t stream) {
+  static DevCache lds_set;
+  if (int rc = ensure_dyn_lds(lds_set, conv3x3_s3n_kernel<NT, MATCH>, r.lds, "conv3x3_s3n_kernel")) return rc;
+  const long wgs = (long)(r.lds <= 80 * 1024 ? 2 : 1) * num_cus();
+  hipLaunchKernelGGL((conv3x3_s3n_kernel<NT, MATCH>), dim3((unsigned)(r.total < wgs ? r.total : wgs)), dim3(64 * S3nGeom<NT>::NW), r.lds, stream, p);
+  return check_launch("conv3x3_s3n_kernel");
+}
+
+static int s3n_run(const ccvpe_conv_desc* d, int match, const float* g, int ldg, int L, int off, float* scores, void* stream) {
+  S3nRoute r;
+  if (const char* why = s3n_pick(d, match, r)) return fail(CCVPE_EINVAL, "conv3x3_s3n: %s", why);
+  if (!d->src0 || !d->w || !d->shift || !d->dst) return fail(CCVPE_EINVAL, "conv3x3_s3n: null pointer (src0, w, shift and dst are required)");
+  S3nParams p{};
+  p.src = d->src0; p.w = d->w; p.bias = d->shift; p.dst = d->dst;
+  p.c0 = d->c0; p.ld0 = d->ld0; p.H = d->in_h; p.W = d->in_w;
+  p.N = d->n; p.nb = r.nb; p.pitch = s3n_pitch(r.nb);
+  p.ldd = d->ldd;
+  p.tiles_x = (int)r.tiles_x; p.tiles_y = (int)r.tiles_y; p.tiles_total = (int)r.total;
+  p.w_off = (r.th + 2) * S3N_HC * p.pitch;
+  p.g = g; p.scores = scores; p.ldg = ldg; p.L = L; p.off = off;
+  hipStream_t st = (hipStream_t)stream;
+#define CCVPE_CASE(NT_) \
+  if (r.nt == NT_) return match ? launch_s3n<NT_, true>(p, r, st) : launch_s3n<NT_, false>(p, r, st);
+  CCVPE_CASE(1) CCVPE_CASE(2) CCVPE_CASE(3) CCVPE_CASE(4) CCVPE_CASE(5)
+#undef CCVPE_CASE
+  return fail(CCVPE_EINVAL, "conv3x3_s3n: no instantiation");
+}
+
+}
+
+using namespace ccvpe;
+
+#ifdef S3N_STAMPS
+extern "C" int ccvpe_s3n_stamps(unsigned long long* out, int reset) {
+  if (hipDeviceSynchronize() != hipSuccess) return CCVPE_ELAUNCH;
+  if (out && hipMemcpyFromSymbol(out, HIP_SYMBOL(s3n_dbg), sizeof(s3n_dbg)) != hipSuccess) return CCVPE_ELAUNCH;
+  unsigned long long zero[8] = {0, 0, 0, 0, 0, 0, 0, 0};
+  if (reset && hipMemcpyToSymbol(HIP_SYMBOL(s3n_dbg), zero, sizeof(zero)) != hipSuccess) return CCVPE_ELAUNCH;
+  return CCVPE_OK;
+}
+#endif
+
+extern "C" int ccvpe_conv3x3_s3n_ok(const ccvpe_conv_desc* d, int match) {
+  S3nRoute r;
+  return s3n_pick(d, match, r) ? 0 : s3n_measured_size(d, match) ? 2 : 1;
+}
+
+extern "C" int ccvpe_conv3x3_s3n_route(const ccvpe_conv_desc* d, int match) {
+  S3nRoute r;
+  return s3n_pick(d, match, r) ? 0 : 1 | (r.match << 4) | (r.nt << 8) | (r.nb << 12) | (r.nw << 16);
+}
+
+extern "C" int ccvpe_conv3x3_s3n_f32(const ccvpe_conv_desc* d, void* stream) {
+  return s3n_run(d, 0, nullptr, 0, 0, 0, nullptr, stream);
+}
+
+extern "C" int ccvpe_conv3x3_match1_s3n_f32(const ccvpe_conv_desc* d, int out_f32, const float* g, int ldg, int L, int shift, int stride,
+                                            int window_offset, float* scores, void* stream) {
+  if (!d || !g || !scores) return fail(CCVPE_EINVAL, "conv3x3_match1_s3n: null pointer");
+  if (!out_f32) return fail(CCVPE_EINVAL, "conv3x3_match1_s3n: fp32 output only");
+  if (L <= 0 || L > ldg || L > d->n) return fail(CCVPE_EINVAL, "conv3x3_match1_s3n: the window length must be in 1 .. min(N, ldg)");
+  if ((reinterpret_cast<uintptr_t>(g) | reinterpret_cast<uintptr_t>(scores)) & 3) return fail(CCVPE_EINVAL, "conv3x3_match1_s3n: g and scores must be 4-byte aligned");
+  long o = d->n > 0 ? (-((long)shift * stride + window_offset)) % d->n : 0;
+  return s3n_run(d, 1, g, ldg, L, (int)(o < 0 ? o + d->n : o), scores, stream);
+}
diff --git a/ccvpe_amd/csrc/plan.hip b/ccvpe_amd/csrc/plan.hip
--- a/ccvpe_amd/csrc/plan.hip
+++ b/ccvpe_amd/csrc/plan.hip
@@ -34,6 +34,7 @@
       CCVPE_REG(ccvpe_conv_igemm_f32), CCVPE_REG(ccvpe_conv_igemm_bf16), CCVPE_REG(ccvpe_conv_igemm_splitk_f32),
       CCVPE_REG(ccvpe_conv_igemm_splitk_bf16), CCVPE_REG(ccvpe_conv3x3_match1_bf16), CCVPE_REG(ccvpe_conv3x3_wino_f32),
       CCVPE_REG(ccvpe_upconv3x3_f32), CCVPE_REG(ccvpe_upconv3x3_bf16), CCVPE_REG(ccvpe_upconv3x3_s3_f32), CCVPE_REG(ccvpe_pw_s3_f32),
+      CCVPE_REG(ccvpe_conv3x3_s3n_f32), CCVPE_REG(ccvpe_conv3x3_match1_s3n_f32),
       CCVPE_REG(ccvpe_tail512_f32), CCVPE_REG(ccvpe_tail512_bf16), CCVPE_REG(ccvpe_stem_conv_f32), CCVPE_REG(ccvpe_stem_conv_bf16),
       CCVPE_REG(ccvpe_stem_dw_f32), CCVPE_REG(ccvpe_stem_dw_bf16),
       CCVPE_REG(ccvpe_dwconv_f32), CCVPE_REG(ccvpe_dwconv_bf16), CCVPE_REG(ccvpe_mbconv_front_f32), CCVPE_REG(ccvpe_mbconv_front_bf16),
diff --git a/ccvpe_amd/models.py b/ccvpe_amd/models.py
--- a/ccvpe_amd/models.py
+++ b/ccvpe_amd/models.py
@@ -156,6 +156,8 @@
 SPLIT3_MIN_OK = 2
 SPLIT3_PW = SPLIT3 and __import__("os").environ.get("CCVPE_SPLIT3_PW", "1") != "0"
 SPLIT3_PW_MIN_OK = 2
+SPLIT3_CONV = SPLIT3 and __import__("os").environ.get("CCVPE_SPLIT3_CONV", "1") != "0"
+SPLIT3_CONV_MIN_OK = 2
 PACK_GRAPH = __import__("os").environ.get("CCVPE_PACK_GRAPH", "1") != "0"
 PACK_GATHER = __import__("os").environ.get("CCVPE_PACK_GATHER", "1") != "0"
 FUSE_MATCH = __import__("os").environ.get("CCVPE_FUSE_MATCH", "1") != "0"
@@ -211,6 +213,19 @@
     mid = r.to(torch.bfloat16)
     lo = (r - mid.float()).to(torch.bfloat16)
     return hi, mid, lo
+
+
+def _pack_conv_s3n(w):
+    if w is None or w.dtype != torch.float32 or w.dim() != 4 or tuple(w.shape[2:]) != (3, 3):
+        return None
+    o, i = w.shape[0], w.shape[1]
+    if o % 8 or i % 8 or o > 80 or i > 80:
+        return None
+    nb, npad = (i + 15) // 16, _round_up(o, 16)
+    t = w.new_zeros((9, npad, nb * 16))
+    t[:, :o, :i] = w.permute(2, 3, 0, 1).reshape(9, o, i)
+    t = t.reshape(9, npad, nb, 16).permute(0, 2, 1, 3)
+    return torch.cat(_split3_bf16(t), -1).contiguous()
 
 
 def _pack_upconv_s3(fw, cp, c1, dtype=torch.float32):
@@ -325,6 +340,7 @@
         if lvl != 1:
             lv.w_b = _pack_conv(sd["conv%d.2.weight" % lvl], dtype)
             lv.u_b = _pack_wino(sd["conv%d.2.weight" % lvl], base_dtype) if fold else None
+            lv.w_b3 = _pack_conv_s3n(sd["conv%d.2.weight" % lvl]) if s3 else None
             lv.n_b = c_out
         else:
             lv.w_b = sd["conv1.2.weight"].permute(0, 2, 3, 1).contiguous()
@@ -357,6 +373,7 @@
         if lvl != 1:
             ov.w_b = _pack_conv(sd["conv%d_ori.2.weight" % lvl], dtype)
             ov.u_b = _pack_wino(sd["conv%d_ori.2.weight" % lvl], dtype) if fold else None
+            ov.w_b3 = _pack_conv_s3n(sd["conv%d_ori.2.weight" % lvl]) if s3 else None
             ov.n_b = c_out
         else:
             ov.w_b = sd["conv1_ori.2.weight"].permute(0, 2, 3, 1).contiguous()
@@ -419,6 +436,10 @@
 
 
 def _conv_b(lv, y, batch, hw, out_f32=False):
+    w_b3 = getattr(lv, "w_b3", None)
+    if (SPLIT3_CONV and w_b3 is not None and y.dtype == torch.float32 and
+            ops.conv3x3_s3n_ok(y, lv.n_a, w_b3, lv.n_b, batch=batch, in_h=hw, in_w=hw) >= SPLIT3_CONV_MIN_OK):
+        return ops.conv3x3_s3n(y, lv.n_a, w_b3, lv.n_b, batch=batch, in_h=hw, in_w=hw, bias=lv.b_b)
     if (WINO and lv.u_b is not None and
             ops.conv3x3_wino_ok(y, lv.n_a, lv.u_b, lv.n_b, batch=batch, in_h=hw, in_w=hw)):
         return ops.conv3x3_wino(y, lv.n_a, lv.u_b, lv.n_b, batch=batch, in_h=hw, in_w=hw, shift=lv.b_b)
@@ -681,10 +702,13 @@
                     to_f32 = j + 1 == pk.f32_from and y.dtype != torch.float32
                     nxt = pk.loc[j + 1]
                     L_n = gw * spec["cd"][j + 1]
-                    if (FUSE_MATCH and len(loc_shifts) == 1 and
-                            ops.conv3x3_match1(y, lv.n_a, lv.w_b, lv.n_b, None, L_n, loc_shifts[0], strides[j + 1], nxt.ldo, batch=batch,
-                                               in_h=2 * hw, in_w=2 * hw, bias=lv.b_b, out_f32=to_f32, query_only=True)):
-                        fused = ops.conv3x3_match1(y, lv.n_a, lv.w_b, lv.n_b, gdesc[:, goff:goff + L_n], L_n, loc_shifts[0],
+                    f32y = y.dtype == torch.float32
+                    w_m = (getattr(lv, "w_b3", None) if SPLIT3_CONV else None) if f32y else lv.w_b
+                    if (FUSE_MATCH and len(loc_shifts) == 1 and w_m is not None and
+                            ops.conv3x3_match1(y, lv.n_a, w_m, lv.n_b, None, L_n, loc_shifts[0], strides[j + 1], nxt.ldo, batch=batch,
+                                               in_h=2 * hw, in_w=2 * hw, bias=lv.b_b, out_f32=to_f32, query_only=True,
+                                               min_ok=SPLIT3_CONV_MIN_OK)):
+                        fused = ops.conv3x3_match1(y, lv.n_a, w_m, lv.n_b, gdesc[:, goff:goff + L_n], L_n, loc_shifts[0],
                                                    strides[j + 1], nxt.ldo, batch=batch, in_h=2 * hw, in_w=2 * hw, bias=lv.b_b,
                                                    window_offset=window_offset(self.kind, nxt.c, L_n), out_f32=to_f32)
                         x = fused[1]
diff --git a/ccvpe_amd/ops.py b/ccvpe_amd/ops.py
--- a/ccvpe_amd/ops.py
+++ b/ccvpe_amd/ops.py
@@ -412,6 +412,65 @@
     return dst
 
 
+def _s3n_desc(src0, c0, w3_packed, n, batch, in_h, in_w, bias, dst, ldd, ld0):
+    d = ConvDesc()
+    d.src0, d.src1, d.gate, d.w = _ptr(src0), None, None, _ptr(w3_packed)
+    d.scale, d.shift, d.residual = None, _ptr(bias), None
+    d.dst = _ptr(dst) if dst is not None else None
+    d.c0, d.ld0, d.c1, d.ld1 = c0, ld0, 0, 0
+    d.batch, d.in_h, d.in_w = batch, in_h, in_w
+    d.kh, d.kw, d.stride, d.pad = 3, 3, 1, 1
+    d.n, d.kpad = n, w3_packed.shape[0] * w3_packed.shape[1] * w3_packed.shape[3]
+    d.ldd, d.ldres = ldd, 0
+    d.act, d.out_mode = ACT_NONE, OUT_NHWC
+    return d
+
+
+def _s3n_pack_ok(w3_packed, c0, n):
+    return (w3_packed is not None and w3_packed.dtype == torch.bfloat16 and w3_packed.dim() == 4 and
+            tuple(w3_packed.shape) == (9, (c0 + 15) // 16, (n + 15) // 16 * 16, 48))
+
+
+def conv3x3_s3n_ok(src0, c0, w3_packed, n, *, batch, in_h, in_w, match=False, ldd=None, ld0=None):
+    if src0.dtype != torch.float32 or not _s3n_pack_ok(w3_packed, c0, n):
+        return 0
+    ld0 = ld0 if ld0 is not None else src0.shape[-1]
+    ldd = ldd if ldd is not None else ((n + 8) // 8 * 8 if match else n)
+    d = _s3n_desc(src0, c0, w3_packed, n, batch, in_h, in_w, None, None, ldd, ld0)
+    return int(_lib.load().ccvpe_conv3x3_s3n_ok(ctypes.byref(d), int(bool(match))))
+
+
+def conv3x3_s3n_route_name(desc, match):
+    r = _lib.load().ccvpe_conv3x3_s3n_route(ctypes.byref(desc), int(bool(match)))
+    if r <= 0:
+        raise _lib.CcvpeError("ccvpe_conv3x3_s3n_route: the kernel does not compute this layer")
+    return "conv3x3_s3n_kernel<f32 as 3 bf16,%d%s>" % (desc.n, ",match" if match else "")
+
+
+def conv3x3_s3n(src0, c0, w3_packed, n, *, batch, in_h, in_w, bias, dst=None, ldd=None, ld0=None):
+    lib = _lib.load()
+    for t, nm in ((src0, "src0"), (bias, "bias"), (dst, "dst")):
+        _chk(t, nm)
+    _chk(w3_packed, "w", torch.bfloat16)
+    if not _s3n_pack_ok(w3_packed, c0, n):
+        raise ValueError("w is not the three-plane pack of models._pack_conv_s3n for c0 = %d, n = %d" % (c0, n))
+    ld0 = ld0 if ld0 is not None else src0.shape[-1]
+    if dst is None:
+        ldd = ldd if ldd is not None else n
+        dst = _empty((batch, in_h, in_w, ldd), device=src0.device)
+    elif ldd is None:
+        ldd = dst.shape[-1]
+    d = _s3n_desc(src0, c0, w3_packed, n, batch, in_h, in_w, bias, dst, ldd, ld0)
+    rec = _recorder
+    ev0 = rec.begin() if rec is not None else None
+    check(lib.ccvpe_conv3x3_s3n_f32(ctypes.byref(d), _stream()), "ccvpe_conv3x3_s3n_f32")
+    if rec is not None:
+        m = batch * in_h * in_w
+        rec.end(conv3x3_s3n_route_name(d, False), "3x3 s1 M%d N%d K%d" % (m, n, 9 * c0), 2.0 * m * n * 9 * c0,
+                4.0 * (m * c0 + m * n + n * 9 * c0), ev0)
+    return dst
+
+
 def tail512(x, c0, w_packed, shift9, w2, b2, cout, normalize, *, batch, h1, w1, split=False, want_softmax=False):
     lib = _lib.load()
     dt = _act_dtype(x)
@@ -594,13 +653,32 @@
 
 
 def conv3x3_match1(src0, c0, w_packed, n, g, L, shift, stride, ldo, *, batch, in_h, in_w, bias, window_offset=0, out_f32=False,
-                   query_only=False):
+                   query_only=False, min_ok=1, ld0=None):
     lib = _lib.load()
     dt = _act_dtype(src0)
     if dt != torch.bfloat16:
+        ok = 0 if not 1 <= L <= n else conv3x3_s3n_ok(src0, c0, w_packed, n, batch=batch, in_h=in_h, in_w=in_w, match=True, ldd=ldo, ld0=ld0)
         if query_only:
-            return False
-        raise ValueError("conv3x3_match1: bf16 storage only")
+            return ok >= min_ok
+        if not ok:
+            raise _lib.CcvpeError("conv3x3_match1: the fp32 three-plane kernel does not serve this layer (no fallback)")
+        _chk(src0, "src0")
+        _chk(w_packed, "w", torch.bfloat16)
+        _chk(bias, "bias")
+        if not g.is_cuda or g.dtype != torch.float32 or g.stride(-1) != 1:
+            raise ValueError("g must be an fp32 device tensor with unit inner stride")
+        scores = _empty((batch, 1, in_h, in_w), device=src0.device, dtype=torch.float32)
+        cat = _empty((batch, in_h, in_w, ldo), device=src0.device, dtype=torch.float32)
+        d = _s3n_desc(src0, c0, w_packed, n, batch, in_h, in_w, bias, cat, ldo, ld0 if ld0 is not None else src0.shape[-1])
+        rec = _recorder
+        ev0 = rec.begin() if rec is not None else None
+        check(lib.ccvpe_conv3x3_match1_s3n_f32(ctypes.byref(d), 1, _ptr(g), g.stride(0), L, int(shift), int(stride),
+                                               int(window_offset), _ptr(scores), _stream()), "ccvpe_conv3x3_match1_s3n_f32")
+        if rec is not None:
+            m = batch * in_h * in_w
+            rec.end(conv3x3_s3n_route_name(d, True), "3x3+match M%d N%d K%d" % (m, n, 9 * c0), 2.0 * m * n * 9 * c0,
+                    4.0 * m * c0 + 4.0 * m * ldo + 4.0 * m + 4.0 * n * 9 * c0, ev0)
+        return scores, cat
     _chk(src0, "src0", dt)
     _chk(w_packed, "w", dt)
     _chk(bias, "bias")
diff --git a/ccvpe_amd/plan.py b/ccvpe_amd/plan.py
--- a/ccvpe_amd/plan.py
+++ b/ccvpe_amd/plan.py
@@ -10,13 +10,13 @@
 ALIGN = 256
 
 LAUNCHES = ("ccvpe_conv_igemm_f32", "ccvpe_conv_igemm_bf16", "ccvpe_conv_igemm_splitk_f32", "ccvpe_conv_igemm_splitk_bf16",
-            "ccvpe_conv3x3_match1_bf16", "ccvpe_conv3x3_wino_f32",
+            "ccvpe_conv3x3_match1_bf16", "ccvpe_conv3x3_wino_f32", "ccvpe_conv3x3_s3n_f32", "ccvpe_conv3x3_match1_s3n_f32",
             "ccvpe_upconv3x3_f32", "ccvpe_upconv3x3_bf16", "ccvpe_upconv3x3_s3_f32", "ccvpe_pw_s3_f32", "ccvpe_tail512_f32", "ccvpe_tail512_bf16", "ccvpe_stem_conv_f32",
             "ccvpe_stem_conv_bf16", "ccvpe_stem_dw_f32", "ccvpe_stem_dw_bf16", "ccvpe_dwconv_f32", "ccvpe_dwconv_bf16", "ccvpe_mbconv_front_f32", "ccvpe_mbconv_front_bf16",
             "ccvpe_se_gate_f32", "ccvpe_ground_descriptor_f32", "ccvpe_match_level_f32", "ccvpe_match_level_bf16",
             "ccvpe_head_conv3x3_f32", "ccvpe_head_conv3x3_bf16", "ccvpe_softmax_rows_f32", "ccvpe_softmax_apply_f32", "ccvpe_cast_bf16_f32",
             "ccvpe_eval_postprocess_f32")
-QUERIES = ("ccvpe_tail512_partials", "ccvpe_conv3x3_match1_ok", "ccvpe_conv3x3_wino_ok", "ccvpe_upconv3x3_s3_ok", "ccvpe_conv_igemm_splitk_floats", "ccvpe_conv_igemm_route", "ccvpe_conv3x3_variant", "ccvpe_upconv3x3_route", "ccvpe_upconv3x3_s3_route", "ccvpe_pw_s3_ok", "ccvpe_pw_s3_route", "ccvpe_dwconv_nblk", "ccvpe_mbconv_front_nblk", "ccvpe_mbconv_front_route", "ccvpe_mbconv_band_plan", "ccvpe_stem_dw_nblk",
+QUERIES = ("ccvpe_tail512_partials", "ccvpe_conv3x3_match1_ok", "ccvpe_conv3x3_wino_ok", "ccvpe_upconv3x3_s3_ok", "ccvpe_conv_igemm_splitk_floats", "ccvpe_conv_igemm_route", "ccvpe_conv3x3_variant", "ccvpe_upconv3x3_route", "ccvpe_upconv3x3_s3_route", "ccvpe_pw_s3_ok", "ccvpe_pw_s3_route", "ccvpe_conv3x3_s3n_ok", "ccvpe_conv3x3_s3n_route", "ccvpe_dwconv_nblk", "ccvpe_mbconv_front_nblk", "ccvpe_mbconv_front_route", "ccvpe_mbconv_band_plan", "ccvpe_stem_dw_nblk",
            "ccvpe_last_error", "ccvpe_abi_version")
 
 
diff --git a/include/ccvpe_hip.h b/include/ccvpe_hip.h
--- a/include/ccvpe_hip.h
+++ b/include/ccvpe_hip.h
@@ -92,6 +92,12 @@
 int ccvpe_pw_s3_ok(const ccvpe_conv_desc* desc);
 int ccvpe_pw_s3_route(const ccvpe_conv_desc* desc);
 int ccvpe_pw_s3_f32(const ccvpe_conv_desc* desc, void* stream);
+
+int ccvpe_conv3x3_s3n_ok(const ccvpe_conv_desc* desc, int match);
+int ccvpe_conv3x3_s3n_route(const ccvpe_conv_desc* desc, int match);
+int ccvpe_conv3x3_s3n_f32(const ccvpe_conv_desc* desc, void* stream);
+int ccvpe_conv3x3_match1_s3n_f32(const ccvpe_conv_desc* desc, int out_f32, const float* g, int ldg, int L, int shift, int stride,
+                                 int window_offset, float* scores, void* stream);
 
 typedef struct ccvpe_tail_desc {
   const void* x;
```

Result: faster. 2908, median of 6 (+2.0%).
